# Vegeta2020/SE-SSD

Hardware: NVIDIA H100
Metric: frames_per_sec (higher is better)
Workload: dtype f32

## Files before the change

### include/sessd_b200.h

```cpp
#ifndef SESSD_B200_H
#define SESSD_B200_H

#include <stddef.h>
#include <stdint.h>

#ifdef __cplusplus
extern "C" {
#endif

#define SESSD_OK 0
#define SESSD_EINVAL (-1)
#define SESSD_ECAPACITY (-2)
#define SESSD_EWORKSPACE (-3)

const char *sessd_version(void);
long long sessd_launch_count(void);

typedef struct {
    float voxel_size[3];
    float range_min[3];
    float range_max[3];
    int grid[3];
    int max_points;
    int max_voxels;
    int num_feat;
} sessd_voxel_cfg;

size_t sessd_voxelize_workspace_bytes(int max_total_points, int batch, const sessd_voxel_cfg *cfg);

int sessd_voxelize(const float *d_points, const int *d_frame_off, int batch, int max_total_points,
                   const sessd_voxel_cfg *cfg, float *d_voxels, int *d_coors, int *d_num_points, float *d_mean,
                   int *d_num_voxels, void *workspace, size_t workspace_bytes, void *stream);

int sessd_voxelize_host(const float *h_points, int num_points, const sessd_voxel_cfg *cfg, float *h_voxels,
                        int *h_coors_zyx , int *h_num_points);

typedef struct {
    int batch;
    int shape[3];
} sessd_grid;

size_t sessd_hash_bytes(int max_rows, int *capacity_out);
int sessd_hash_build(const int *d_coors , const int *d_n, int max_rows, sessd_grid grid,
                     uint64_t *d_table, int capacity, void *stream);

size_t sessd_bitmap_words(sessd_grid grid);
size_t sessd_scan_scratch_bytes(size_t n_items);

int sessd_subm_rulebook(const int *d_coors, const int *d_n, int max_rows, sessd_grid grid, const int ksize[3],
                        int index_kind , const void *d_index, int hash_capacity,
                        int *d_nbr, void *stream);

int sessd_strided_rulebook(const int *d_in_coors, const int *d_n_in, int max_in, sessd_grid in_grid,
                           int in_index_kind, const void *d_in_index, int in_hash_capacity,
                           const int ksize[3], const int stride[3], const int padding[3],
                           sessd_grid out_grid, void *d_out_bitmap , void *d_scan_scratch,
                           int *d_out_coors, int *d_n_out, int max_out, int *d_nbr, int *d_status, void *stream);

int sessd_tile_list_stride(int kvol);
int sessd_rulebook_tile_lists(const int *d_nbr, int kvol, const int *d_n_out, int max_out, void *d_tiles, void *stream);

int sessd_spconv_forward(const float *d_in_feat, int cin, const int *d_nbr, int kvol, const int *d_n_out,
                         int max_out, const float *d_weight, int cout, const float *d_scale, const float *d_shift,
                         int relu, float *d_out_feat, void *stream);

int sessd_sparse_to_dense(const float *d_feat, const int *d_coors, const int *d_n, int max_rows, int channels,
                          sessd_grid grid, float *d_out, void *stream);
int sessd_sparse_to_dense_indexed(const float *d_feat, int max_rows, const void *d_bitmap_index, int channels, sessd_grid grid,
                                  float *d_out, void *stream);

int sessd_spconv_forward_rows(const float *d_in_feat, int cin, const int *d_nbr, int kvol, const int *d_n_out, int max_out,
                              const float *d_weight, int cout, const float *d_scale, const float *d_shift, int relu,
                              float *d_out_feat, float *d_amax_out, void *stream);
int sessd_spconv_forward_rows_planes(const float *d_in_feat, int cin, const int *d_nbr, int kvol, const int *d_n_out, int max_out,
                                     const float *d_weight, int cout, const float *d_scale, const float *d_shift, int relu,
                                     const float *d_amax_in, float gain, float shift_max, float *d_out_feat, void *d_out_planes, int cpo,
                                     float *d_out_info, void *stream);
int sessd_spconv_forward_cg(const void *d_in_planes, int cp, int plane_rows, const float *d_in_info, const void *d_tiles, int kvol,
                            const int *d_n_out, int max_out, const void *d_weight_h2, int cout, const float *d_scale, const float *d_shift,
                            int relu, float gain, float shift_max, float *d_out_f32, void *d_out_planes, float *d_out_info, void *stream);
void sessd_set_sp_cg_deep(int on);
int sessd_spconv_cg_blocks_per_sm(int cp, int cout, int deep);
int sessd_absmax_rows(const float *d_feat, const int *d_n, int max_rows, int channels, float *d_amax, void *stream);

int sessd_rulebook_transpose(const int *d_nbr, int kvol, const int *d_n_out, int max_out, int max_in, int *d_nbr_t, void *stream);
int sessd_sparse_split_planes(const float *d_x, const int *d_n, int max_rows, int channels, float *d_info, void *d_planes, int cp, void *stream);
int sessd_dense_grad_gather(const float *d_grad, const int *d_coors, const int *d_n, int max_rows, int channels, sessd_grid grid,
                            float *d_out, void *stream);
int sessd_spconv_wgrad_items(int max_out, int kvol);
size_t sessd_spconv_wgrad_workspace_bytes(int max_out, int kvol, int cin, int cout);
int sessd_spconv_wgrad_rows(const float *d_in_feat, int cin, const float *d_gout, int cout, const void *d_tiles, int kvol,
                            const int *d_n_out, int max_out, float *d_gw, void *d_ws, size_t ws_bytes, void *stream);
int sessd_spconv_wgrad_cg(const void *d_in_planes, int cp, const float *d_in_info, const void *d_g_planes, int cout, const float *d_g_info,
                          const void *d_tiles, int kvol, const int *d_n_out, int max_out, float *d_gw, void *d_ws, size_t ws_bytes,
                          void *stream);

typedef struct {
    int batch, in_h, in_w, cin;
    int out_h, out_w, cout;
    int grid_h, grid_w;
    int in_stride;
    int out_stride, out_off_y, out_off_x;
    int ntaps;
    int tap_dy[16], tap_dx[16];
    int relu;
} sessd_conv_desc;

int sessd_bev_conv_p2(const void *d_in_planes, const float *d_in_info, const void *d_weight_h2, int cout_pad, const float *d_scale,
                      const float *d_shift, const float *d_residual, const float *d_resid_info, float gain, float shift_max,
                      float *d_out_f32, void *d_out_planes, float *d_out_info, const sessd_conv_desc *desc, const int *d_items,
                      void *stream);
int sessd_bev_deconv_p2(const void *d_in_planes, const float *d_in_info, const void *d_weight_h2, int cout_pad, const float *d_scale,
                        const float *d_shift, const float *d_residual, const float *d_resid_info, float gain, float shift_max,
                        float *d_out_f32, void *d_out_planes, float *d_out_info, int batch, int in_h, int in_w, int cin, int cout,
                        int relu, const int *d_items, void *stream);
long long sessd_bev_skip_plan_words(int batch, int h, int w, int *offsets);
int sessd_bev_skip_plan(const void *d_bitmap_index, sessd_grid grid, int *d_plan, void *stream);
int sessd_bev_skip_fill(const int *d_record, float *d_out_f32, void *d_out_planes, int cout, void *stream);
int sessd_bev_wgrad_items(const sessd_conv_desc *desc);
size_t sessd_bev_wgrad_workspace_bytes(const sessd_conv_desc *desc);
int sessd_bev_wgrad(const void *d_in_planes, const float *d_in_info, const void *d_g_planes, const float *d_g_info,
                    const sessd_conv_desc *desc, float *d_gw, void *d_ws, size_t ws_bytes, void *stream);
int sessd_bev_split_planes(const float *d_x, long long n, float *d_info, void *d_planes, void *stream);
int sessd_sparse_to_dense_planes(const float *d_feat, int max_rows, const void *d_bitmap_index, int channels, sessd_grid grid,
                                 const float *d_amax, float *d_info, void *d_planes, void *stream);
int sessd_ssfa_fuse_planes(const float *d_x0, const float *d_x1, const float *d_w0, const float *d_w1, float s0, float t0, float s1,
                           float t1, int num_pixels, int channels, float *d_out, const float *d_info0, const float *d_info1,
                           float *d_out_info, void *d_planes, void *stream);

int sessd_absmax(const float *d_x, long long n, float *d_amax, void *stream);


typedef struct {
    float cnt_thresh;
    float dist_edge[4];
    float sigma2[3];
    float suppressed_thresh;
    float centerness_pow;
    int centerness;
} sessd_dinms_cfg;

#define SESSD_DINMS_MAX_PRE 4096

typedef struct {
    int batch;
    int num_anchors;
    int anchors_per_loc;
    int head_stride;
    float score_thresh;
    int nms_pre_max;
    int nms_post_max;
    float nms_iou_thresh;
    int nms_ge;
    float post_range[6];
    float direction_offset;
    int use_frustum;
    int nms_mode;
    sessd_dinms_cfg dinms;
} sessd_post_cfg;

size_t sessd_postprocess_workspace_bytes(const sessd_post_cfg *cfg);

int sessd_postprocess(const float *d_head, const float *d_anchors, const float *d_frustum,
                      const sessd_post_cfg *cfg, float *d_boxes, float *d_scores, int *d_labels, int *d_count,
                      int *d_aux, int *d_sel_anchor, void *workspace, size_t workspace_bytes, void *stream);

int sessd_postprocess_packed(const float *d_head, const float *d_anchors, const float *d_frustum,
                             const sessd_post_cfg *cfg, float *d_boxes, float *d_scores, int *d_labels, int *d_count,
                             int *d_aux, int *d_sel_anchor, float *d_packed, int *d_meta, const int *d_num_voxels,
                             const int *d_status, void *workspace, size_t workspace_bytes, void *stream);

size_t sessd_rotate_nms_workspace_bytes(int max_boxes, int pre_max);
int sessd_rotate_nms(const float *d_boxes5, const float *d_scores, const int *d_n, int max_boxes, int pre_max,
                     int post_max, float iou_thresh, int ge, int *d_keep, int *d_num_keep, void *workspace,
                     size_t workspace_bytes, void *stream);

size_t sessd_rotate_weighted_nms_workspace_bytes(int max_boxes, int pre_max);
int sessd_rotate_weighted_nms(const float *d_boxes7, const float *d_boxes5, const float *d_scores, const float *d_iou_preds,
                              const int *d_labels, const int *d_dirs, const float *d_anchors, const int *d_n, int max_boxes,
                              int pre_max, const sessd_dinms_cfg *cfg, float *d_out_boxes, float *d_out_scores, int *d_out_labels,
                              int *d_out_dirs, int *d_keep, int *d_selected, int *d_count, void *workspace, size_t workspace_bytes,
                              void *stream);

int sessd_boxes_overlap_bev(const float *d_a, int n, const float *d_b, int m, float *d_out, void *stream);
int sessd_boxes_aligned_overlap_bev(const float *d_a, const float *d_b, int n, float *d_out, void *stream);
int sessd_boxes_iou_bev(const float *d_a, int n, const float *d_b, int m, float *d_out, void *stream);
int sessd_boxes_iou3d(const float *d_a, int n, const float *d_b, int m, float *d_out, void *stream);
size_t sessd_nms_workspace_bytes(int n);
int sessd_nms_sorted(const float *d_boxes, int n, float thresh, int mode, long long *d_keep, int *d_num_keep,
                     void *workspace, size_t workspace_bytes, void *stream);

size_t sessd_assign_workspace_bytes(int num_anchors, int batch, int max_gt);
int sessd_assign_targets(const float *d_anchors, int num_anchors, const float *d_gt_boxes, const int *d_num_gt, int batch,
                         int max_gt, float matched_thr, float unmatched_thr, int *d_labels, float *d_bbox_targets,
                         float *d_bbox_outside_weights, int *d_pos_anchor, int *d_pos_gt_id, int *d_num_pos,
                         void *workspace, size_t workspace_bytes, void *stream);

#define SESSD_AUGMENT_MAX_GT 256
#define SESSD_AUGMENT_MAX_TRY 128
int sessd_box_collision(const double *d_boxes, int n, const double *d_qboxes, int k, uint8_t *d_out, void *stream);
int sessd_noise_per_box(const float *d_gt_boxes, const int *d_num_gt, const uint8_t *d_valid, int batch, int max_gt,
                        const double *d_loc_noise, const double *d_rot_noise, int num_try, double context, int *d_selected,
                        void *stream);
int sessd_points_in_boxes(const float *d_points, int n, int point_stride, const float *d_boxes, int m, double context, uint8_t *d_mask,
                          void *stream);
int sessd_augment_points(const float *d_points, const int *d_frame_off, int batch, int max_frame_points, const float *d_gt_boxes,
                         const int *d_num_gt, const uint8_t *d_valid, int max_gt, const double *d_loc_noise, const double *d_rot_noise,
                         int num_try, const int *d_selected, double context, const float *d_global, const int *d_perm,
                         const uint8_t *d_labeled, float *d_points_raw, float *d_points_out, void *stream);
int sessd_augment_boxes(const float *d_gt_boxes, const int *d_num_gt, const uint8_t *d_valid, const uint8_t *d_target, int batch,
                        int max_gt, const double *d_loc_noise, const double *d_rot_noise, int num_try, const int *d_selected,
                        const float *d_global, const float *range_bev, float *d_boxes_raw, int *d_num_raw, float *d_boxes_out,
                        int *d_num_out, float *d_boxes_global, int *d_num_global, void *stream);

int sessd_gtaug_select_host(const double *h_corners, int num_boxes, int num_cand, uint8_t *h_accepted);
size_t sessd_gtaug_paste_workspace_bytes(int batch, int num_points, int num_objects);
int sessd_gtaug_paste(const float *d_points, const int *d_frame_off, int batch, int num_points, const int *d_obj_off, const int *d_obj_ids,
                      int num_objects, int max_paste_points, const float *d_db_points, const int *d_db_off, const int *d_db_count,
                      const double *d_db_boxes, int db_size, void *d_workspace, size_t workspace_bytes, float *d_points_out, int capacity,
                      int *d_frame_off_out, void *stream);

#define SESSD_SADA_MAX_IDS (6 * SESSD_AUGMENT_MAX_GT)
int sessd_sada_pyramids(const float *d_boxes, int num_boxes, float *d_pyramids, float *d_planes, void *stream);
int sessd_sada_membership(const float *d_points, int n, const int *d_n, const float *d_planes, int num_pyramids, const int *d_ids, int num_ids,
                          uint32_t *d_bits, int *d_counts, void *stream);
size_t sessd_sada_compact_workspace_bytes(int n);
int sessd_sada_compact(const float *d_points, int n, const int *d_n, const uint32_t *d_bits, int num_ids, const int *d_counts, int min_count,
                       void *d_workspace, size_t workspace_bytes, float *d_out, int capacity, int *d_num_out, void *stream);
size_t sessd_sada_fps_workspace_bytes(int n, int num_ids);
int sessd_sada_fps(const float *d_points, int n, const int *d_n, const uint32_t *d_bits, int num_ids, const int *d_counts, int min_count, int k,
                   void *d_workspace, size_t workspace_bytes, float *d_out, int capacity, int *d_num, void *stream);
int sessd_sada_swap(const float *d_points, int n, const int *d_n, const uint32_t *d_bits, int num_pairs, const int *d_counts, const float *d_pyramids,
                    int num_pyramids, const int *d_ids, int max_swap_points, float *d_out, int capacity, const int *d_num_in,
                    int *d_num_out, void *stream);
int sessd_sada_shuffle(const float *d_points, const int *d_frame_off, int batch, int max_frame_points, const int *d_perm, float *d_out,
                       void *stream);

size_t sessd_prep_frustum_compact_workspace_bytes(int num_points);
int sessd_prep_frustum_compact(const float *d_points, const int *d_frame_off, int batch, int num_points, const double *d_planes,
                               void *d_workspace, size_t workspace_bytes, float *d_points_out, int capacity, int *d_frame_off_out, void *stream);
int sessd_prep_box_count(const float *d_points, const int *d_frame_off, int batch, int num_points, const double *d_box_planes,
                         const int *d_box_off, int num_boxes, int *d_counts, void *stream);
size_t sessd_prep_box_gather_workspace_bytes(int num_boxes);
int sessd_prep_box_gather(const float *d_points, const int *d_frame_off, int batch, int num_points, const double *d_box_planes,
                          const double *d_centres, const int *d_box_off, int num_boxes, const int *d_counts, int num_rows, void *d_workspace,
                          size_t workspace_bytes, float *d_rows_out, int capacity, int *d_obj_off, void *stream);

size_t sessd_head_loss_workspace_bytes(int batch);
size_t sessd_odiou_loss_workspace_bytes(int batch);
int sessd_odiou_loss(const float *d_head, const float *d_anchors, const int *d_labels, const float *d_reg_targets, int batch,
                     int num_anchors, int anchors_per_loc, int head_stride, float w_odiou, const float *d_losses, float *d_odiou_sum,
                     float *d_grad_head, void *workspace, size_t workspace_bytes, void *stream);
int sessd_odiou_pairs_host(const float *h_gboxes, const float *h_qboxes, int n, float *h_odiou, float *h_grad_q);
size_t sessd_iou_pred_loss_workspace_bytes(int batch);
int sessd_iou_pred_loss(const float *d_head, const float *d_anchors, const int *d_labels, const float *d_reg_targets, int batch,
                        int num_anchors, int anchors_per_loc, int head_stride, float sigma, float w_iou, float *d_losses,
                        float *d_grad_head, void *workspace, size_t workspace_bytes, void *stream);
int sessd_head_loss(const float *d_head, const float *d_anchors, const int *d_labels, const float *d_reg_targets, int batch,
                    int num_anchors, int anchors_per_loc, int head_stride, float alpha, float sigma, float dir_offset,
                    float pos_cls_weight, float neg_cls_weight, float w_cls, float w_loc, float w_dir, float *d_losses,
                    float *d_grad_head, void *workspace, size_t workspace_bytes, void *stream);

int sessd_axpby(float *d_y, const float *d_x, float a, float b, long long n, void *stream);
int sessd_adamw_step(float *d_param, const float *d_grad, float *d_exp_avg, float *d_exp_avg_sq, long long n, float lr, float beta1,
                     float beta2, float eps, float weight_decay, int step, void *stream);
size_t sessd_grad_sqnorm_workspace_bytes(long long n);
int sessd_grad_sqnorm(const float *d_x, long long n, float max_norm, float *d_out, void *d_workspace, void *stream);
int sessd_adamw_clip_ema_step(float *d_param, float *d_grad, float *d_exp_avg, float *d_exp_avg_sq, long long n, float lr, float beta1,
                              float beta2, float eps, float weight_decay, int step, const float *d_clip_coef, float *d_ema, double ema_alpha,
                              void *stream);

#define SESSD_KITTI_REC 13
#define SESSD_KITTI_PERSON_SITTING 11
#define SESSD_KITTI_VAN 12
typedef struct {
    int num_frames;
    const int *gt_off;
    const double *gt;
    const int *gt_code;
    const int *gt_occluded;
    const int *dc_off;
    const double *dc;
    const int *dt_off;
    const int *dt_cnt;
    const double *dt;
    const int *dt_code;
    const long long *ov_off;
} SessdKittiFrames;
size_t sessd_kitti_convert_workspace_bytes(long long capacity);
int sessd_kitti_convert_detections(const float *d_boxes7, const float *d_scores, const int *d_labels, const int *d_off, int num_frames,
                                   long long capacity, const double *d_calib, const int *d_image_hw, const int *d_label_code,
                                   int num_labels, double *d_rec, int *d_label, int *d_code, int *d_cnt, void *workspace,
                                   size_t workspace_bytes, void *stream);
int sessd_kitti_overlaps(const SessdKittiFrames *frames, int metric, int z_axis, double z_center, double *d_overlaps, void *stream);
size_t sessd_kitti_eval_workspace_bytes(int num_frames, long long total_gt, long long overlap_elems, int num_configs, int compute_aos);
int sessd_kitti_eval(const SessdKittiFrames *frames, int max_frame_dt, int metric, int z_axis, double z_center, int num_configs,
                     const int *d_cfg, const double *d_min_overlap, int compute_aos, long long total_gt, long long overlap_elems,
                     double *d_thresholds, int *d_num_thresholds, double *d_precision, double *d_aos, double *d_map, void *workspace,
                     size_t workspace_bytes, void *stream);

#ifdef __cplusplus
}
#endif
#endif
```

### include/sessd_b200_lab.h

```cpp
#ifndef SESSD_B200_LAB_H
#define SESSD_B200_LAB_H

#include "sessd_b200.h"

#ifdef __cplusplus
extern "C" {
#endif

int sessd_bev_conv_h2(const float *d_in, const void *d_weight_h2, int cout_pad, const float *d_scale,
                      const float *d_shift, const float *d_residual, float *d_out, const sessd_conv_desc *desc,
                      const float *d_amax_in, float *d_amax_out, void *stream);
int sessd_bev_deconv_h2(const float *d_in, const void *d_weight_h2, int cout_pad, const float *d_scale,
                        const float *d_shift, const float *d_residual, float *d_out, int batch, int in_h, int in_w,
                        int cin, int cout, int relu, const float *d_amax_in, float *d_amax_out, void *stream);

int sessd_bev_conv_p2_profile(const void *d_in_planes, const float *d_in_info, const void *d_weight_h2, int cout_pad,
                              const float *d_scale, const float *d_shift, const float *d_residual, const float *d_resid_info,
                              float gain, float shift_max, float *d_out_f32, void *d_out_planes, float *d_out_info,
                              const sessd_conv_desc *desc, const int *d_items, long long *d_prof, void *stream);
int sessd_bev_deconv_p2_profile(const void *d_in_planes, const float *d_in_info, const void *d_weight_h2, int cout_pad,
                                const float *d_scale, const float *d_shift, const float *d_residual, const float *d_resid_info,
                                float gain, float shift_max, float *d_out_f32, void *d_out_planes, float *d_out_info, int batch,
                                int in_h, int in_w, int cin, int cout, int relu, const int *d_items, long long *d_prof,
                                void *stream);

int sessd_bev_conv_p2_loads(const void *d_in_planes, const float *d_in_info, const void *d_weight_h2, int cout_pad,
                            const float *d_scale, const float *d_shift, const float *d_residual, const float *d_resid_info,
                            float gain, float shift_max, float *d_out_f32, void *d_out_planes, float *d_out_info,
                            const sessd_conv_desc *desc, const int *d_items, int smem_a, long long *d_prof, void *stream);

int sessd_bev_p2_plan(const sessd_conv_desc *desc, int deconv, int cout_pad, int split, int smem_a, int *plan);

#ifdef __cplusplus
}
#endif
#endif
```

### se-ssd_b200/csrc/bevconv_p2.cu

```cuda
#include "bevconv_p2.cuh"

namespace sessd {

__global__ void __launch_bounds__(256) bev_split_planes_kernel(const float4 *__restrict__ x, long long n4, float *__restrict__ info,
                                                               __half *__restrict__ planes, long long plane_stride) {
    const float s = pow2_scale_for_bound(__ldg(info));
    if (blockIdx.x == 0 && threadIdx.x == 0) info[1] = s;
    for (long long i = blockIdx.x * (long long)blockDim.x + threadIdx.x; i < n4; i += (long long)gridDim.x * blockDim.x) {
        const float4 v = __ldg(x + i);
        const float a[4] = {v.x * s, v.y * s, v.z * s, v.w * s};
        __align__(8) __half hi[4], lo[4];
#pragma unroll
        for (int t = 0; t < 4; ++t) {
            hi[t] = __float2half_rn(a[t]);
            lo[t] = __float2half_rn(a[t] - __half2float(hi[t]));
        }
        *reinterpret_cast<uint2 *>(planes + 4 * i) = *reinterpret_cast<const uint2 *>(hi);
        *reinterpret_cast<uint2 *>(planes + plane_stride + 4 * i) = *reinterpret_cast<const uint2 *>(lo);
    }
}

}

using namespace sessd;

extern "C" int sessd_bev_conv_p2(const void *d_in_planes, const float *d_in_info, const void *d_weight_h2, int cout_pad, const float *d_scale,
                                 const float *d_shift, const float *d_residual, const float *d_resid_info, float gain, float shift_max,
                                 float *d_out_f32, void *d_out_planes, float *d_out_info, const sessd_conv_desc *desc, const int *d_items,
                                 void *stream) {
    return p2_conv<kP2Planes>(d_in_planes, d_in_info, d_weight_h2, cout_pad, d_scale, d_shift, d_residual, d_resid_info, gain, shift_max,
                              d_out_f32, d_out_planes, d_out_info, desc, stream, d_items);
}

extern "C" int sessd_bev_deconv_p2(const void *d_in_planes, const float *d_in_info, const void *d_weight_h2, int cout_pad, const float *d_scale,
                                   const float *d_shift, const float *d_residual, const float *d_resid_info, float gain, float shift_max,
                                   float *d_out_f32, void *d_out_planes, float *d_out_info, int batch, int in_h, int in_w, int cin, int cout,
                                   int relu, const int *d_items, void *stream) {
    return p2_deconv<kP2Planes>(d_in_planes, d_in_info, d_weight_h2, cout_pad, d_scale, d_shift, d_residual, d_resid_info, gain, shift_max,
                                d_out_f32, d_out_planes, d_out_info, batch, in_h, in_w, cin, cout, relu, stream, d_items);
}

extern "C" int sessd_bev_split_planes(const float *d_x, long long n, float *d_info, void *d_planes, void *stream) {
    if (!d_x || !d_info || !d_planes || n < 4 || (n & 3) || ((uintptr_t)d_x & 15)) return SESSD_EINVAL;
    SESSD_LAUNCH(bev_split_planes_kernel, persistent_grid(n / 4, 256), 256, 0, stream, reinterpret_cast<const float4 *>(d_x), n / 4, d_info,
                 (__half *)d_planes, n);
    return last_error();
}
```

### se-ssd_b200/csrc/bevconv_p2.cuh

```cuda
#pragma once
#include <cuda_fp16.h>

#include "tc_common.cuh"

namespace sessd {

constexpr int kP2TileU = 8, kP2TileV = 16;
constexpr int kP2MaxCopies = 6, kP2MaxRowsV = 18;
constexpr int kP2BStages = 6, kP2MaxBStages = 12;
constexpr int kP2MmaWarps = 8;
constexpr int kP2PatchWarp = 8, kP2WeightWarp = 9;
constexpr int kP2Threads = 320;
constexpr int kP2ThreadsRegA = 384, kP2RegsConsumer = 232, kP2RegsProducer = 40;
static_assert(2 * (kP2RegsConsumer - 168) <= 168 - kP2RegsProducer, "the consumers take what the producers release");
constexpr int kP2MaxSmem = 227 * 1024;
constexpr int kP2Chunk = 32;
constexpr int kP2ItemsHeader = 32;
enum { kP2Planes = 0, kP2SplitF16 = 1 };
enum { kP2NoProbe = 0, kP2ProbeClocks = 1, kP2ProbeLoads = 2 };

struct P2Params {
    int batch, cin, cout;
    int in_stride;
    int out_h, out_w;
    int grid_u, grid_v;
    int u_is_x;
    int out_stride, nclass;
    int cls_ntaps[4], cls_off_u[4], cls_off_v[4];
    int tap_copy[4][9], tap_row[4][9], tap_w[4][9];
    int ncopies, rows_v, pitch_u;
    int copy_u[kP2MaxCopies], copy_v[kP2MaxCopies];
    int copy_bytes, patch_bytes, npatch;
    int load_bytes, staging_bytes;
    int bring_bytes;
    int out_info_scale;
    const float *in_amax;
    int relu, n_tile, nblocks;
    int bstages, bstage_bytes;
    int tiles_u, tiles_v, tiles, total;
    int cls_order[4];
    const float *in_info;
    const float *resid_info;
    float gain, shift_max;
    float *out_info;
    long long out_plane_stride;
    const int *items;
    long long *prof;
};

enum P2Prof {
    kProfCta,
    kProfItems,
    kProfSteps,
    kProfItemClk,
    kProfBFull,
    kProfPatchFull,
    kProfMmaWait,
    kProfEpilogue,
    kProfPatchEmpty,
    kProfPatchTotal,
    kProfBEmpty,
    kProfBTotal,
    kP2ProfWords = 16
};

__device__ __forceinline__ int p2_item_count(const P2Params &p) { return p.items ? __ldg(p.items) : p.total; }
__device__ __forceinline__ int p2_item(const P2Params &p, int k) { return p.items ? __ldg(p.items + kP2ItemsHeader + k) : k; }

struct P2ItemIndex { int rank, nb, t; };
__host__ __device__ __forceinline__ P2ItemIndex p2_item_index(int g, int nblocks, int tiles) {
    const int rank = g / (nblocks * tiles), rem = g - rank * (nblocks * tiles), nb = rem / tiles;
    return {rank, nb, rem - nb * tiles};
}

struct P2Item { int cls, n0, b, u0, v0, ntaps; };

__device__ __forceinline__ P2Item p2_decode(const P2Params &p, int g) {
    P2Item it;
    const P2ItemIndex ix = p2_item_index(g, p.nblocks, p.tiles);
    int t = ix.t;
    it.cls = p.cls_order[ix.rank];
    it.n0 = ix.nb * p.n_tile;
    const int tu = t % p.tiles_u; t /= p.tiles_u;
    const int tv = t % p.tiles_v;
    it.b = t / p.tiles_v;
    it.u0 = tu * kP2TileU; it.v0 = tv * kP2TileV;
    it.ntaps = p.cls_ntaps[it.cls];
    return it;
}

template <int N>
__device__ __forceinline__ void p2_wgmma(float *d, uint64_t da, uint64_t db, uint32_t accumulate) {
    if constexpr (N == 32) wgmma_f16_n32(d, da, db, accumulate);
    else if constexpr (N == 64) wgmma_f16_n64(d, da, db, accumulate);
    else if constexpr (N == 128) wgmma_f16_n128(d, da, db, accumulate);
    else wgmma_f16_n256(d, da, db, accumulate);
}

template <int N>
__device__ __forceinline__ void p2_wgmma_ra(float *d, const uint32_t *a, uint64_t db, uint32_t accumulate) {
    if constexpr (N == 32) wgmma_f16_ra_n32(d, a, db, accumulate);
    else if constexpr (N == 64) wgmma_f16_ra_n64(d, a, db, accumulate);
    else if constexpr (N == 128) wgmma_f16_ra_n128(d, a, db, accumulate);
    else wgmma_f16_ra_n256(d, a, db, accumulate);
}

template <bool PROFILE>
__device__ __forceinline__ long long p2_tick() {
    if constexpr (PROFILE) return clock64();
    return 0;
}
template <bool PROFILE>
__device__ __forceinline__ void p2_tock(long long &clk, long long t0) {
    if constexpr (PROFILE) clk += clock64() - t0;
}

__device__ __forceinline__ void p2_split_patch(const P2Params &p, const unsigned char *staging, unsigned char *planes, float s_in, int ctid) {
    const int rows = p.rows_v * kP2TileU;
    const int copy_in = p.staging_bytes / p.ncopies;
    const int items = p.ncopies * rows * 4;
    for (int i = ctid; i < items; i += kP2MmaWarps * 32) {
        const int j = i & 3, r = (i >> 2) % rows, c = (i >> 2) / rows;
        unsigned char *hi = planes + 2 * c * p.copy_bytes + r * 64 + ((j ^ ((r >> 1) & 3)) << 4);
        const float4 *src = reinterpret_cast<const float4 *>(staging + c * copy_in + r * 128 + j * 32);
        const float4 a = src[0], b = src[1];
        const float x[8] = {a.x * s_in, a.y * s_in, a.z * s_in, a.w * s_in, b.x * s_in, b.y * s_in, b.z * s_in, b.w * s_in};
        __align__(16) __half h[8], l[8];
#pragma unroll
        for (int t = 0; t < 8; ++t) { h[t] = __float2half_rn(x[t]); l[t] = __float2half_rn(x[t] - __half2float(h[t])); }
        *reinterpret_cast<uint4 *>(hi) = *reinterpret_cast<const uint4 *>(h);
        *reinterpret_cast<uint4 *>(hi + p.copy_bytes) = *reinterpret_cast<const uint4 *>(l);
    }
    asm volatile("fence.proxy.async.shared::cta;\n" ::: "memory");
    asm volatile("bar.sync 1, %0;\n" ::"n"(kP2MmaWarps * 32) : "memory");
}

template <int NT, int MODE, bool REGA = false, int PROBE = kP2NoProbe>
__global__ void __launch_bounds__(REGA ? kP2ThreadsRegA : kP2Threads, 1) bev_conv_p2_kernel(const __grid_constant__ CUtensorMap map_a,
                                                                   const __grid_constant__ CUtensorMap map_b,
                                                                   const float *__restrict__ scale, const float *__restrict__ shift,
                                                                   const float *__restrict__ resid, float *__restrict__ out_f32,
                                                                   __half *__restrict__ out_planes, P2Params p) {
    static_assert(!REGA || MODE == kP2Planes, "register-fed A reads the TMA-written planes");
    constexpr bool PROFILE = PROBE != kP2NoProbe, LOADS_ONLY = PROBE == kP2ProbeLoads;
    extern __shared__ unsigned char smem_raw[];
    unsigned char *tiles = (unsigned char *)(((uintptr_t)smem_raw + 1023) & ~(uintptr_t)1023);
    unsigned char *patches = tiles + p.bring_bytes;
    unsigned char *staging = patches + p.npatch * p.patch_bytes;
    uint64_t *bars = (uint64_t *)(staging + p.npatch * p.staging_bytes);
    uint64_t *patch_full = bars, *patch_empty = bars + 2, *b_full = bars + 4, *b_empty = bars + 4 + kP2MaxBStages;
    uint32_t *s_aoff = (uint32_t *)(b_empty + kP2MaxBStages);
    float *s_scale = (float *)(((uintptr_t)(s_aoff + 4 * 9) + 15) & ~(uintptr_t)15), *s_shift = s_scale + p.cout;

    const int warp = threadIdx.x >> 5, lane = threadIdx.x & 31;
    if (threadIdx.x == kP2PatchWarp * 32) prefetch_tensormap(&map_a);
    if (threadIdx.x == kP2WeightWarp * 32) prefetch_tensormap(&map_b);
    const int nchunks = p.cin / kP2Chunk;
    const int nitems = p2_item_count(p);
    const uint32_t b_plane_bytes = (uint32_t)p.n_tile * 64u;

    if (threadIdx.x == 0) {
        for (int s = 0; s < 2; ++s) { mbar_init(&patch_full[s], 1); mbar_init(&patch_empty[s], kP2MmaWarps); }
        for (int s = 0; s < p.bstages; ++s) { mbar_init(&b_full[s], 1); mbar_init(&b_empty[s], kP2MmaWarps); }
        asm volatile("fence.mbarrier_init.release.cluster;\n" ::: "memory");
    }
    for (int idx = threadIdx.x; idx < p.nclass * 9; idx += blockDim.x) {
        const int c = idx / 9, t = idx - c * 9;
        s_aoff[idx] = REGA ? (uint32_t)p.tap_row[c][t] : (uint32_t)((2 * p.tap_copy[c][t] * p.copy_bytes + p.tap_row[c][t] * 512) >> 4);
    }
    for (int n = threadIdx.x; n < p.cout; n += blockDim.x) {
        s_scale[n] = scale ? __ldg(scale + n) : 1.f;
        s_shift[n] = shift ? __ldg(shift + n) : 0.f;
    }
    __syncthreads();
    long long clk[kP2ProfWords] = {};
    const long long t_start = p2_tick<PROFILE>();
    long long *prof_rec = PROFILE ? p.prof + (size_t)blockIdx.x * kP2ProfWords : nullptr;

    if (warp >= kP2MmaWarps) {
        if constexpr (REGA) setmaxnreg_dec<kP2RegsProducer>();
        if (warp == kP2PatchWarp) {
            int pb = 0;
            uint32_t pph = 0;
            const uint32_t patches_u32 = smem_u32(patches);
            for (int k = blockIdx.x; k < nitems; k += gridDim.x) {
                const P2Item it = p2_decode(p, p2_item(p, k));
                const int bu = it.u0 * p.in_stride, bv = it.v0 * p.in_stride;
                for (int cc = 0; cc < nchunks; ++cc) {
                    { const long long t0 = p2_tick<PROFILE>(); mbar_wait<REGA>(&patch_empty[pb], pph ^ 1u); p2_tock<PROFILE>(clk[kProfPatchEmpty], t0); }
                    if (elect_one()) {
                        mbar_expect_tx(&patch_full[pb], (uint32_t)p.load_bytes);
                        if constexpr (MODE == kP2Planes) {
                            uint32_t dst = patches_u32 + (uint32_t)(pb * p.patch_bytes);
                            for (int c = 0; c < p.ncopies; ++c, dst += 2u * (uint32_t)p.copy_bytes) {
                                const int cu = bu + p.copy_u[c], cv = bv + p.copy_v[c];
                                tma_load_5d(dst, &map_a, &patch_full[pb], cc * kP2Chunk, cu, cv, it.b, 0);
                                tma_load_5d(dst + (uint32_t)p.copy_bytes, &map_a, &patch_full[pb], cc * kP2Chunk, cu, cv, it.b, 1);
                            }
                        } else {
                            const uint32_t copy_in = (uint32_t)(p.staging_bytes / p.ncopies);
                            uint32_t dst = smem_u32(staging) + (uint32_t)(pb * p.staging_bytes);
                            for (int c = 0; c < p.ncopies; ++c, dst += copy_in)
                                tma_load_5d(dst, &map_a, &patch_full[pb], cc * kP2Chunk, bu + p.copy_u[c], bv + p.copy_v[c], it.b, 0);
                        }
                    }
                    __syncwarp();
                    if (++pb == p.npatch) { pb = 0; pph ^= 1u; }
                }
            }
            if constexpr (PROFILE)
                if (lane == 0) {
                    prof_rec[kProfPatchEmpty] = clk[kProfPatchEmpty];
                    prof_rec[kProfPatchTotal] = clock64() - t_start;
                }
        } else if (warp == kP2WeightWarp) {
            int S = 0;
            uint32_t bph = 0;
            for (int k = blockIdx.x; k < nitems; k += gridDim.x) {
                const P2Item it = p2_decode(p, p2_item(p, k));
                for (int cc = 0; cc < nchunks; ++cc)
                    for (int tap = 0; tap < it.ntaps; ++tap) {
                        { const long long t0 = p2_tick<PROFILE>(); mbar_wait<REGA>(&b_empty[S], bph ^ 1u); p2_tock<PROFILE>(clk[kProfBEmpty], t0); }
                        if (elect_one()) {
                            unsigned char *st = tiles + S * p.bstage_bytes;
                            const int wtap = p.tap_w[it.cls][tap];
                            mbar_expect_tx(&b_full[S], 2 * b_plane_bytes);
                            tma_load_4d(st + b_plane_bytes, &map_b, &b_full[S], cc * kP2Chunk, it.n0, wtap, 0);
                            tma_load_4d(st, &map_b, &b_full[S], cc * kP2Chunk, it.n0, wtap, 1);
                        }
                        __syncwarp();
                        if (++S == p.bstages) { S = 0; bph ^= 1u; }
                    }
            }
            if constexpr (PROFILE)
                if (lane == 0) {
                    prof_rec[kProfBEmpty] = clk[kProfBEmpty];
                    prof_rec[kProfBTotal] = clock64() - t_start;
                }
        }
    } else {
        if constexpr (REGA) setmaxnreg_inc<kP2RegsConsumer>();
        const int wg = warp >> 2, wq = warp & 3;
        constexpr int kAcc = NT / 2;
        const uint32_t a_rows = (uint32_t)(wg * 64 * 64) >> 4;
        const uint32_t tiles_lo = desc_lo(smem_u32(tiles));
        const uint32_t patch_lo = desc_lo(smem_u32(patches)) + a_rows;
        const uint32_t plane_lo = b_plane_bytes >> 4;
        const uint32_t copy_lo = (uint32_t)(p.copy_bytes >> 4), patch_sz = (uint32_t)(p.patch_bytes >> 4);
        const uint32_t a_row = (uint32_t)((wg * 8 + wq * 2 + ((lane >> 3) & 1)) * p.pitch_u + (lane & 7)), a_chunk = (uint32_t)(lane >> 4);
        const uint32_t patches_u32 = smem_u32(patches);
        float amax_in = 0.f, s_in = 1.f;
        if constexpr (MODE == kP2Planes) { amax_in = __ldg(p.in_info); s_in = __ldg(p.in_info + 1); }
        if constexpr (MODE == kP2SplitF16) if (p.in_amax) { amax_in = __ldg(p.in_amax); s_in = pow2_scale_for_bound(amax_in); }
        const float inv_sa = 1.f / s_in;
        float bound = amax_in * p.gain + p.shift_max;
        if (p.resid_info) bound += __ldg(p.resid_info);
        const float s_out = pow2_scale_for_bound(bound);
        if (blockIdx.x == 0 && threadIdx.x == 0 && p.out_info && p.out_info_scale) p.out_info[1] = s_out;
        float vmax = 0.f;
        const int per_cls = p.nblocks * p.tiles;
        int S = 0, pb = 0;
        uint32_t bph = 0, pph = 0;
        for (int k = blockIdx.x; k < nitems; k += gridDim.x) {
            const long long t_item = p2_tick<PROFILE>();
            const int g = p2_item(p, k);
            const int cls = p.cls_order[g / per_cls];
            const int ntaps = p.cls_ntaps[cls];
            const uint32_t *aoff = s_aoff + cls * 9;
            float acc[NT];
#pragma unroll
            for (int i = 0; i < NT; ++i) acc[i] = 0.f;
            int prevS = -1, prev_pb = -1;
            bool first = true;
            if constexpr (REGA) {
                uint32_t frag[2][16];
                int tap = 0;
                uint32_t pbase = 0;
                auto load_frags = [&](uint32_t *fa) {
                    if (tap == 0) {
                        { const long long t0 = p2_tick<PROFILE>(); mbar_wait<REGA>(&patch_full[pb], pph); p2_tock<PROFILE>(clk[kProfPatchFull], t0); }
                        pbase = patches_u32 + (uint32_t)(pb * p.patch_bytes);
                    }
                    if constexpr (!LOADS_ONLY) {
                        const uint32_t r = a_row + aoff[tap];
                        const uint32_t a_hi = pbase + r * 64u + ((a_chunk ^ ((r >> 1) & 3u)) << 4), a_lo = a_hi + (uint32_t)p.copy_bytes;
                        ldsm_x4(fa, a_hi);
                        ldsm_x4(fa + 4, a_hi ^ 32u);
                        ldsm_x4(fa + 8, a_lo);
                        ldsm_x4(fa + 12, a_lo ^ 32u);
                    }
                };
                auto step_ra = [&](const uint32_t *fa, uint32_t *fn, bool more) {
                    { const long long t0 = p2_tick<PROFILE>(); mbar_wait<REGA>(&b_full[S], bph); p2_tock<PROFILE>(clk[kProfBFull], t0); }
                    const uint64_t db_lo = kDescSw64Hi | (uint64_t)(tiles_lo + (uint32_t)(S * (p.bstage_bytes >> 4)));
                    const uint64_t db_hi = db_lo + (uint64_t)plane_lo;
                    if constexpr (!LOADS_ONLY) {
                        wgmma_fence();
                        p2_wgmma_ra<2 * NT>(acc, fa, db_lo, first ? 0u : 1u);
                        p2_wgmma_ra<2 * NT>(acc, fa + 4, db_lo + 2, 1u);
                        wgmma_commit();
                    }
                    first = false;
                    if constexpr (PROFILE) ++clk[kProfSteps];
                    { const long long t0 = p2_tick<PROFILE>(); wgmma_wait<1>(); p2_tock<PROFILE>(clk[kProfMmaWait], t0); }
                    if (lane == 0 && prevS >= 0) mbar_arrive(&b_empty[prevS]);
                    prevS = S;
                    if (++S == p.bstages) { S = 0; bph ^= 1u; }
                    if (++tap == ntaps) {
                        tap = 0;
                        if (lane == 0) mbar_arrive(&patch_empty[pb]);
                        if (++pb == p.npatch) { pb = 0; pph ^= 1u; }
                    }
                    if (more) load_frags(fn);
                    if constexpr (!LOADS_ONLY) {
                        wgmma_fence();
                        p2_wgmma_ra<NT>(acc, fa + 8, db_hi, 1u);
                        p2_wgmma_ra<NT>(acc, fa + 12, db_hi + 2, 1u);
                        wgmma_commit();
                    }
                };
                const int nsteps = nchunks * ntaps;
                load_frags(frag[0]);
#pragma unroll 1
                for (int st = 0; st + 1 < nsteps; st += 2) { step_ra(frag[0], frag[1], true); step_ra(frag[1], frag[0], st + 2 < nsteps); }
                if (nsteps & 1) step_ra(frag[0], frag[1], false);
            } else {
                for (int cc = 0; cc < nchunks; ++cc) {
                    { const long long t0 = p2_tick<PROFILE>(); mbar_wait(&patch_full[pb], pph); p2_tock<PROFILE>(clk[kProfPatchFull], t0); }
                    if constexpr (MODE == kP2SplitF16)
                        p2_split_patch(p, staging + pb * p.staging_bytes, patches + pb * p.patch_bytes, s_in, threadIdx.x);
                    const uint32_t pbase = patch_lo + (uint32_t)pb * patch_sz;
#pragma unroll 1
                    for (int tap = 0; tap < ntaps; ++tap) {
                        { const long long t0 = p2_tick<PROFILE>(); mbar_wait(&b_full[S], bph); p2_tock<PROFILE>(clk[kProfBFull], t0); }
                        if constexpr (!LOADS_ONLY) {
                            const uint64_t da_hi = kDescSw64Hi | (uint64_t)(pbase + aoff[tap]);
                            const uint64_t da_lo = da_hi + (uint64_t)copy_lo;
                            const uint64_t db_lo = kDescSw64Hi | (uint64_t)(tiles_lo + (uint32_t)(S * (p.bstage_bytes >> 4)));
                            const uint64_t db_hi = db_lo + (uint64_t)plane_lo;
                            const uint32_t accum = first ? 0u : 1u;
                            wgmma_fence();
                            if constexpr (MODE == kP2Planes) {
                                p2_wgmma<2 * NT>(acc, da_hi, db_lo, accum);
                                p2_wgmma<2 * NT>(acc, da_hi + 2, db_lo + 2, 1u);
                            } else {
                                p2_wgmma<NT>(acc + kAcc, da_hi, db_hi, accum);
                                p2_wgmma<NT>(acc + kAcc, da_hi + 2, db_hi + 2, 1u);
                                p2_wgmma<NT>(acc, da_hi, db_lo, accum);
                                p2_wgmma<NT>(acc, da_hi + 2, db_lo + 2, 1u);
                            }
                            p2_wgmma<NT>(acc, da_lo, db_hi, 1u);
                            p2_wgmma<NT>(acc, da_lo + 2, db_hi + 2, 1u);
                            wgmma_commit();
                        }
                        first = false;
                        if constexpr (PROFILE) ++clk[kProfSteps];
                        { const long long t0 = p2_tick<PROFILE>(); wgmma_wait<1>(); p2_tock<PROFILE>(clk[kProfMmaWait], t0); }
                        if (lane == 0) {
                            if (prevS >= 0) mbar_arrive(&b_empty[prevS]);
                            if (prev_pb >= 0) mbar_arrive(&patch_empty[prev_pb]);
                        }
                        prevS = S;
                        prev_pb = (tap == ntaps - 1) ? pb : -1;
                        if (++S == p.bstages) { S = 0; bph ^= 1u; }
                    }
                    if (p.npatch == 1) {
                        { const long long t0 = p2_tick<PROFILE>(); wgmma_wait<0>(); p2_tock<PROFILE>(clk[kProfMmaWait], t0); }
                        if (lane == 0) {
                            mbar_arrive(&b_empty[prevS]);
                            mbar_arrive(&patch_empty[pb]);
                        }
                        prevS = prev_pb = -1;
                    }
                    if (++pb == p.npatch) { pb = 0; pph ^= 1u; }
                }
            }
            { const long long t0 = p2_tick<PROFILE>(); wgmma_wait<0>(); p2_tock<PROFILE>(clk[kProfMmaWait], t0); }
            const long long t_epi = p2_tick<PROFILE>();
            wgmma_fence_regs<NT>(acc);
            if (lane == 0) {
                if (prevS >= 0) mbar_arrive(&b_empty[prevS]);
                if (prev_pb >= 0) mbar_arrive(&patch_empty[prev_pb]);
            }
#pragma unroll
            for (int i = 0; i < kAcc; ++i) acc[i] = acc[kAcc + i] + acc[i];
            const P2Item it = p2_decode(p, g);
            const int q = lane & 3;
            const int r0 = wg * 64 + wq * 16 + (lane >> 2);
            bool rows_ok[2];
            size_t opixs[2];
#pragma unroll
            for (int h = 0; h < 2; ++h) {
                const int r = r0 + 8 * h;
                const int lv = r / kP2TileU, lu = r % kP2TileU;
                const int gu = it.u0 + lu, gv = it.v0 + lv;
                rows_ok[h] = it.b < p.batch && gu < p.grid_u && gv < p.grid_v;
                const int ou = gu * p.out_stride + p.cls_off_u[it.cls], ov = gv * p.out_stride + p.cls_off_v[it.cls];
                const int oy = p.u_is_x ? ov : ou, ox = p.u_is_x ? ou : ov;
                opixs[h] = ((size_t)it.b * p.out_h + (size_t)oy) * p.out_w + (size_t)ox;
            }
#pragma unroll
            for (int j = 0; j < (LOADS_ONLY ? 0 : NT / 32); ++j)
#pragma unroll
                for (int h = 0; h < 2; ++h) {
                    const bool row_ok = rows_ok[h];
                    const size_t opix = opixs[h];
                    float v[8], o[8] = {};
                    quad_transpose8(acc + 16 * j + 2 * h, q, v);
                    const int n = it.n0 + 32 * j + 8 * q;
                    const size_t off = opix * p.cout + n;
                    if (row_ok && n < p.cout) {
                        float sc[8], sh[8];
#pragma unroll
                        for (int t = 0; t < 8; t += 4) {
                            const float4 a = *reinterpret_cast<const float4 *>(s_scale + n + t);
                            const float4 b = *reinterpret_cast<const float4 *>(s_shift + n + t);
                            sc[t] = a.x; sc[t + 1] = a.y; sc[t + 2] = a.z; sc[t + 3] = a.w;
                            sh[t] = b.x; sh[t + 1] = b.y; sh[t + 2] = b.z; sh[t + 3] = b.w;
                        }
#pragma unroll
                        for (int t = 0; t < 8; ++t) {
                            o[t] = fmaf(v[t] * inv_sa, sc[t], sh[t]);
                            if (p.relu) o[t] = fmaxf(o[t], 0.f);
                        }
                        if (resid) {
#pragma unroll
                            for (int t = 0; t < 8; t += 4) {
                                const float4 rr = __ldg(reinterpret_cast<const float4 *>(resid + off + t));
                                o[t] += rr.x; o[t + 1] += rr.y; o[t + 2] += rr.z; o[t + 3] += rr.w;
                            }
                        }
#pragma unroll
                        for (int t = 0; t < 8; ++t) vmax = fmaxf(vmax, fabsf(o[t]));
                        if (out_planes) {
                            __align__(16) __half2 hi[4], lo[4];
#pragma unroll
                            for (int t = 0; t < 4; ++t) {
                                const float x0 = o[2 * t] * s_out, x1 = o[2 * t + 1] * s_out;
                                hi[t] = __floats2half2_rn(x0, x1);
                                const float2 f = __half22float2(hi[t]);
                                lo[t] = __floats2half2_rn(x0 - f.x, x1 - f.y);
                            }
                            *reinterpret_cast<uint4 *>(out_planes + off) = *reinterpret_cast<const uint4 *>(hi);
                            *reinterpret_cast<uint4 *>(out_planes + p.out_plane_stride + off) = *reinterpret_cast<const uint4 *>(lo);
                        }
                    }
                    if (out_f32) {
                        const bool up = q & 2;
                        float keep[4], recv[4];
#pragma unroll
                        for (int t = 0; t < 4; ++t) {
                            keep[t] = up ? o[4 + t] : o[t];
                            recv[t] = __shfl_xor_sync(0xFFFFFFFFu, up ? o[t] : o[4 + t], 2);
                        }
                        const int n_lo = it.n0 + 32 * j + 8 * (q & 1), c_lo = n_lo + 4 * (q >> 1);
                        const float4 w_lo = up ? make_float4(recv[0], recv[1], recv[2], recv[3]) : make_float4(keep[0], keep[1], keep[2], keep[3]);
                        const float4 w_hi = up ? make_float4(keep[0], keep[1], keep[2], keep[3]) : make_float4(recv[0], recv[1], recv[2], recv[3]);
                        if (row_ok && n_lo < p.cout) *reinterpret_cast<float4 *>(out_f32 + opix * p.cout + c_lo) = w_lo;
                        if (row_ok && n_lo + 16 < p.cout) *reinterpret_cast<float4 *>(out_f32 + opix * p.cout + c_lo + 16) = w_hi;
                    }
                }
            if constexpr (PROFILE) {
                const long long t_end = clock64();
                clk[kProfEpilogue] += t_end - t_epi;
                clk[kProfItemClk] += t_end - t_item;
                ++clk[kProfItems];
            }
        }
        if constexpr (PROFILE)
            if (threadIdx.x == 0) {
                clk[kProfCta] = clock64() - t_start;
                for (int w = kProfCta; w <= kProfEpilogue; ++w) prof_rec[w] = clk[w];
            }
        if (p.out_info) {
            const unsigned m = __reduce_max_sync(0xFFFFFFFFu, __float_as_uint(vmax));
            if (lane == 0 && m != 0u) atomicMax(reinterpret_cast<unsigned *>(p.out_info), m);
        }
    }
}

static int encode_map_nd(CUtensorMap *m, const void *base, int rank, const cuuint64_t *dims, const cuuint64_t *strides_bytes ,
                         const cuuint32_t *box, const cuuint32_t *estr, CUtensorMapSwizzle swz,
                         CUtensorMapDataType dtype = CU_TENSOR_MAP_DATA_TYPE_FLOAT16) {
    EncodeTiledFn enc = get_tensor_map_encoder();
    if (!enc) return SESSD_EINVAL;
    CUresult r = enc(m, dtype, (cuuint32_t)rank, const_cast<void *>(base), dims, strides_bytes, box, estr,
                     CU_TENSOR_MAP_INTERLEAVE_NONE, swz, CU_TENSOR_MAP_L2_PROMOTION_L2_256B, CU_TENSOR_MAP_FLOAT_OOB_FILL_NONE);
    return r == CUDA_SUCCESS ? 0 : 700 + (int)r;
}

struct P2Taps { int n, dy[9], dx[9], w[9], off_y, off_x; };

static void p2_deconv_classes(P2Taps cls[4]) {
    for (int c = 0; c < 4; ++c) {
        P2Taps &k = cls[c];
        k = {};
        k.off_y = c >> 1; k.off_x = c & 1;
        for (int dy = k.off_y; dy >= 0; --dy)
            for (int dx = k.off_x; dx >= 0; --dx, ++k.n) {
                k.dy[k.n] = dy; k.dx[k.n] = dx; k.w[k.n] = (k.off_y + 1 - 2 * dy) * 3 + (k.off_x + 1 - 2 * dx);
            }
    }
}

constexpr int p2_n_tile(int cout) { return cout <= 32 ? 32 : 128; }

struct P2Geometry {
    int u_is_x, grid_u, grid_v, tiles_u, tiles_v, tiles;
    int n_tile, nblocks, nclass, total;
    int ntaps[4], off_u[4], off_v[4], order[4];
};

static int p2_geometry(P2Geometry &g, int batch, int grid_h, int grid_w, int cout, int cout_pad, const P2Taps *cls, int nclass) {
    g = {};
    if (batch < 1 || grid_h < 1 || grid_w < 1 || cout < 8 || cout % 8) return SESSD_EINVAL;
    g.n_tile = p2_n_tile(cout);
    if (cout_pad % g.n_tile || cout_pad < cout) return SESSD_EINVAL;
    g.u_is_x = div_up(grid_w, kP2TileU) * div_up(grid_h, kP2TileV) <= div_up(grid_h, kP2TileU) * div_up(grid_w, kP2TileV);
    g.grid_u = g.u_is_x ? grid_w : grid_h; g.grid_v = g.u_is_x ? grid_h : grid_w;
    g.tiles_u = div_up(g.grid_u, kP2TileU); g.tiles_v = div_up(g.grid_v, kP2TileV);
    g.tiles = g.tiles_u * g.tiles_v * batch;
    g.nblocks = cout_pad / g.n_tile;
    g.nclass = nclass; g.total = nclass * g.nblocks * g.tiles;
    for (int c = 0; c < nclass; ++c) {
        g.ntaps[c] = cls[c].n;
        g.off_u[c] = g.u_is_x ? cls[c].off_x : cls[c].off_y;
        g.off_v[c] = g.u_is_x ? cls[c].off_y : cls[c].off_x;
        g.order[c] = c;
    }
    for (int i = 1; i < nclass; ++i)
        for (int k = i; k > 0 && g.ntaps[g.order[k]] > g.ntaps[g.order[k - 1]]; --k) {
            const int tmp = g.order[k]; g.order[k] = g.order[k - 1]; g.order[k - 1] = tmp;
        }
    return 0;
}

static int p2_plan(P2Params &p, const P2Taps *cls, int nclass, int grid_h, int grid_w, int cout_pad, int mode, bool reg_a, int *smem) {
    if (reg_a && (mode != kP2Planes || p.in_stride != 1)) return SESSD_EINVAL;
    if (p.cin < 64 || p.cin % 64) return SESSD_EINVAL;
    P2Geometry g;
    if (p2_geometry(g, p.batch, grid_h, grid_w, p.cout, cout_pad, cls, nclass)) return SESSD_EINVAL;
    p.u_is_x = g.u_is_x; p.grid_u = g.grid_u; p.grid_v = g.grid_v;
    p.tiles_u = g.tiles_u; p.tiles_v = g.tiles_v; p.tiles = g.tiles;
    p.n_tile = g.n_tile; p.nblocks = g.nblocks; p.nclass = g.nclass; p.total = g.total;
    for (int c = 0; c < 4; ++c) {
        p.cls_ntaps[c] = g.ntaps[c]; p.cls_off_u[c] = g.off_u[c]; p.cls_off_v[c] = g.off_v[c]; p.cls_order[c] = g.order[c];
    }
    const int s = p.in_stride;
    p.ncopies = 0;
    int key_u[kP2MaxCopies], key_vm[kP2MaxCopies], vmin[kP2MaxCopies], vmax[kP2MaxCopies];
    for (int c = 0; c < p.nclass; ++c)
        for (int t = 0; t < cls[c].n; ++t) {
            const int tu = p.u_is_x ? cls[c].dx[t] : cls[c].dy[t], tv = p.u_is_x ? cls[c].dy[t] : cls[c].dx[t];
            const int vm = ((tv % s) + s) % s;
            int k = 0;
            for (; k < p.ncopies; ++k)
                if (key_u[k] == tu && key_vm[k] == vm) break;
            if (k == p.ncopies) {
                if (p.ncopies == kP2MaxCopies) return SESSD_EINVAL;
                key_u[k] = tu; key_vm[k] = vm; vmin[k] = tv; vmax[k] = tv;
                ++p.ncopies;
            }
            vmin[k] = min(vmin[k], tv); vmax[k] = max(vmax[k], tv);
        }
    p.rows_v = 0;
    p.pitch_u = kP2TileU;
    for (int k = 0; k < p.ncopies; ++k) p.rows_v = max(p.rows_v, kP2TileV + (vmax[k] - vmin[k]) / s);
    if (p.rows_v > kP2MaxRowsV) return SESSD_EINVAL;
    for (int k = 0; k < p.ncopies; ++k) { p.copy_u[k] = key_u[k]; p.copy_v[k] = vmin[k]; }
    if (reg_a) {
        int umin = key_u[0], umax = key_u[0];
        for (int k = 1; k < p.ncopies; ++k) {
            umin = min(umin, key_u[k]); umax = max(umax, key_u[k]);
            vmin[0] = min(vmin[0], vmin[k]); vmax[0] = max(vmax[0], vmax[k]);
        }
        p.ncopies = 1;
        p.copy_u[0] = umin; p.copy_v[0] = vmin[0];
        p.pitch_u = kP2TileU + umax - umin; p.rows_v = kP2TileV + vmax[0] - vmin[0];
        if (p.pitch_u > 256 || p.rows_v > 256) return SESSD_EINVAL;
    }
    for (int c = 0; c < p.nclass; ++c) {
        for (int t = 0; t < cls[c].n; ++t) {
            const int tu = p.u_is_x ? cls[c].dx[t] : cls[c].dy[t], tv = p.u_is_x ? cls[c].dy[t] : cls[c].dx[t];
            const int vm = ((tv % s) + s) % s;
            int k = 0;
            for (; k < p.ncopies; ++k)
                if (key_u[k] == tu && key_vm[k] == vm) break;
            p.tap_copy[c][t] = reg_a ? 0 : k;
            p.tap_row[c][t] = reg_a ? (tv - p.copy_v[0]) * p.pitch_u + (tu - p.copy_u[0]) : (tv - vmin[k]) / s;
            p.tap_w[c][t] = cls[c].w[t];
        }
    }
    p.copy_bytes = (p.rows_v * p.pitch_u * 64 + 511) & ~511;
    p.patch_bytes = p.ncopies * 2 * p.copy_bytes;
    p.staging_bytes = mode == kP2Planes ? 0 : p.ncopies * p.rows_v * kP2TileU * kP2Chunk * 4;
    p.load_bytes = mode == kP2Planes ? p.ncopies * 2 * p.rows_v * p.pitch_u * 64 : p.staging_bytes;
    const int per_buf = p.patch_bytes + p.staging_bytes, bstage = 2 * p.n_tile * 64;
    const int tail = 1536 + 16 + 2 * 4 * p.cout;
    p.npatch = (kP2BStages * bstage + tail + 2 * per_buf <= kP2MaxSmem) ? 2 : 1;
    p.bstage_bytes = bstage;
    p.bstages = min((kP2MaxSmem - tail - p.npatch * per_buf) / bstage, kP2MaxBStages);
    if (p.bstages < 2) return SESSD_EINVAL;
    p.bring_bytes = p.bstages * bstage;
    *smem = p.bring_bytes + tail + p.npatch * per_buf;
    return 0;
}

template <int MODE, int PROBE = kP2NoProbe>
static int launch_p2(const void *d_in_planes, int in_h, int in_w, const float *d_in_info, const void *d_w, int w_taps, int cout_pad,
                     const float *d_scale, const float *d_shift, const float *d_residual, const float *d_resid_info, float gain,
                     float shift_max, float *d_out_f32, void *d_out_planes, float *d_out_info, P2Params &p, const P2Taps *cls, int nclass,
                     int grid_h, int grid_w, bool reg_a, void *stream) {
    if (!d_in_planes || !d_w || (!d_out_f32 && !d_out_planes)) return SESSD_EINVAL;
    if (MODE == kP2Planes && (!d_in_info || !d_scale)) return SESSD_EINVAL;
    if (MODE != kP2Planes && d_out_planes) return SESSD_EINVAL;
    if (((uintptr_t)d_scale | (uintptr_t)d_shift | (uintptr_t)d_residual | (uintptr_t)d_out_f32 | (uintptr_t)d_out_planes) & 15)
        return SESSD_EINVAL;
    int smem = 0;
    if (p2_plan(p, cls, nclass, grid_h, grid_w, cout_pad, MODE, reg_a, &smem)) return SESSD_EINVAL;
    if (p.items && cout_pad != div_up(p.cout, p.n_tile) * p.n_tile) return SESSD_EINVAL;
    const int s = p.in_stride;
    CUtensorMap map_a, map_b;
    if (MODE != kP2Planes) {
        const cuuint64_t row_w = (cuuint64_t)p.cin * 4, row_h = (cuuint64_t)in_w * p.cin * 4;
        const cuuint64_t dims[5] = {(cuuint64_t)p.cin, (cuuint64_t)(p.u_is_x ? in_w : in_h), (cuuint64_t)(p.u_is_x ? in_h : in_w),
                                    (cuuint64_t)p.batch, 1};
        const cuuint64_t strides[4] = {p.u_is_x ? row_w : row_h, p.u_is_x ? row_h : row_w, (cuuint64_t)in_h * in_w * p.cin * 4,
                                       (cuuint64_t)p.batch * in_h * in_w * p.cin * 4};
        const cuuint32_t box[5] = {(cuuint32_t)kP2Chunk, (cuuint32_t)(kP2TileU * s), (cuuint32_t)(p.rows_v * s), 1, 1};
        const cuuint32_t estr[5] = {1, (cuuint32_t)s, (cuuint32_t)s, 1, 1};
        int rc = encode_map_nd(&map_a, d_in_planes, 5, dims, strides, box, estr, CU_TENSOR_MAP_SWIZZLE_NONE, CU_TENSOR_MAP_DATA_TYPE_FLOAT32);
        if (rc) return rc;
    } else {
        const cuuint64_t row_w = (cuuint64_t)p.cin * 2, row_h = (cuuint64_t)in_w * p.cin * 2;
        const cuuint64_t dims[5] = {(cuuint64_t)p.cin, (cuuint64_t)(p.u_is_x ? in_w : in_h), (cuuint64_t)(p.u_is_x ? in_h : in_w),
                                    (cuuint64_t)p.batch, 2};
        const cuuint64_t strides[4] = {p.u_is_x ? row_w : row_h, p.u_is_x ? row_h : row_w, (cuuint64_t)in_h * in_w * p.cin * 2,
                                       (cuuint64_t)p.batch * in_h * in_w * p.cin * 2};
        const cuuint32_t box[5] = {(cuuint32_t)kP2Chunk, (cuuint32_t)(p.pitch_u * s), (cuuint32_t)(p.rows_v * s), 1, 1};
        const cuuint32_t estr[5] = {1, (cuuint32_t)s, (cuuint32_t)s, 1, 1};
        int rc = encode_map_nd(&map_a, d_in_planes, 5, dims, strides, box, estr, CU_TENSOR_MAP_SWIZZLE_64B);
        if (rc) return rc;
    }
    {
        const cuuint64_t dims[4] = {(cuuint64_t)p.cin, (cuuint64_t)cout_pad, (cuuint64_t)w_taps, 2};
        const cuuint64_t strides[3] = {(cuuint64_t)p.cin * 2, (cuuint64_t)cout_pad * p.cin * 2, (cuuint64_t)w_taps * cout_pad * p.cin * 2};
        const cuuint32_t box[4] = {(cuuint32_t)kP2Chunk, (cuuint32_t)p.n_tile, 1, 1};
        const cuuint32_t estr[4] = {1, 1, 1, 1};
        int rc = encode_map_nd(&map_b, d_w, 4, dims, strides, box, estr, CU_TENSOR_MAP_SWIZZLE_64B);
        if (rc) return rc;
    }
    constexpr bool kRegA = MODE == kP2Planes;
    auto kernel = bev_conv_p2_kernel<128, MODE, false, PROBE>;
    if (p.n_tile == 32) kernel = reg_a ? bev_conv_p2_kernel<32, MODE, kRegA, PROBE> : bev_conv_p2_kernel<32, MODE, false, PROBE>;
    else if (reg_a) kernel = bev_conv_p2_kernel<128, MODE, kRegA, PROBE>;
    static bool attr_done[2][2] = {};
    if (!attr_done[p.n_tile == 32][reg_a]) {
        SESSD_CUDA_TRY(cudaFuncSetAttribute(kernel, cudaFuncAttributeMaxDynamicSharedMemorySize, kP2MaxSmem));
        attr_done[p.n_tile == 32][reg_a] = true;
    }
    p.in_info = MODE == kP2Planes ? d_in_info : nullptr;
    p.in_amax = MODE == kP2SplitF16 ? d_in_info : nullptr;
    p.resid_info = d_residual ? d_resid_info : nullptr;
    if (d_residual && d_out_planes && !d_resid_info) return SESSD_EINVAL;
    p.gain = gain; p.shift_max = shift_max; p.out_info = d_out_info;
    p.out_info_scale = MODE == kP2Planes ? 1 : 0;
    if (d_out_planes && !d_out_info) return SESSD_EINVAL;
    p.out_plane_stride = (long long)p.batch * p.out_h * p.out_w * p.cout;
    static int num_sms = 0;
    if (!num_sms) {
        int dev = 0;
        SESSD_CUDA_TRY(cudaGetDevice(&dev));
        SESSD_CUDA_TRY(cudaDeviceGetAttribute(&num_sms, cudaDevAttrMultiProcessorCount, dev));
    }
    const int grid = p.total < num_sms ? p.total : num_sms;
    SESSD_LAUNCH(kernel, grid, reg_a ? kP2ThreadsRegA : kP2Threads, smem, (cudaStream_t)stream, map_a, map_b, d_scale, d_shift, d_residual, d_out_f32,
                 (__half *)d_out_planes, p);
    return last_error();
}


static int p2_conv_params(const sessd_conv_desc &d, P2Params &p, P2Taps &t) {
    if (d.ntaps < 1 || d.ntaps > 9 || (d.in_stride != 1 && d.in_stride != 2) || d.out_stride < 1) return SESSD_EINVAL;
    if ((d.grid_h - 1) * d.out_stride + d.out_off_y >= d.out_h || (d.grid_w - 1) * d.out_stride + d.out_off_x >= d.out_w) return SESSD_EINVAL;
    p = {};
    p.batch = d.batch; p.cin = d.cin; p.cout = d.cout; p.in_stride = d.in_stride;
    p.out_h = d.out_h; p.out_w = d.out_w; p.out_stride = d.out_stride; p.relu = d.relu;
    t = {};
    t.n = d.ntaps; t.off_y = d.out_off_y; t.off_x = d.out_off_x;
    for (int i = 0; i < d.ntaps; ++i) { t.dy[i] = d.tap_dy[i]; t.dx[i] = d.tap_dx[i]; t.w[i] = i; }
    return 0;
}

static void p2_deconv_params(int batch, int in_h, int in_w, int cin, int cout, int relu, P2Params &p, P2Taps cls[4]) {
    p = {};
    p.batch = batch; p.cin = cin; p.cout = cout; p.in_stride = 1;
    p.out_h = 2 * in_h; p.out_w = 2 * in_w; p.out_stride = 2; p.relu = relu;
    p2_deconv_classes(cls);
}

template <int MODE, int PROBE = kP2NoProbe>
static int p2_conv(const void *d_in_planes, const float *d_in_info, const void *d_weight_h2, int cout_pad, const float *d_scale,
                   const float *d_shift, const float *d_residual, const float *d_resid_info, float gain, float shift_max,
                   float *d_out_f32, void *d_out_planes, float *d_out_info, const sessd_conv_desc *desc, void *stream,
                   const int *d_items = nullptr, long long *d_prof = nullptr, bool smem_a = false) {
    if (!desc || (PROBE != kP2NoProbe && !d_prof)) return SESSD_EINVAL;
    const sessd_conv_desc &d = *desc;
    P2Params p;
    P2Taps t;
    if (p2_conv_params(d, p, t)) return SESSD_EINVAL;
    p.items = d_items;
    p.prof = d_prof;
    return launch_p2<MODE, PROBE>(d_in_planes, d.in_h, d.in_w, d_in_info, d_weight_h2, d.ntaps, cout_pad, d_scale, d_shift, d_residual, d_resid_info, gain,
                     shift_max, d_out_f32, d_out_planes, d_out_info, p, &t, 1, d.grid_h, d.grid_w, MODE == kP2Planes && d.in_stride == 1 && !smem_a,
                     stream);
}

template <int MODE, int PROBE = kP2NoProbe>
static int p2_deconv(const void *d_in_planes, const float *d_in_info, const void *d_weight_h2, int cout_pad, const float *d_scale,
                     const float *d_shift, const float *d_residual, const float *d_resid_info, float gain, float shift_max,
                     float *d_out_f32, void *d_out_planes, float *d_out_info, int batch, int in_h, int in_w, int cin, int cout,
                     int relu, void *stream, const int *d_items = nullptr, long long *d_prof = nullptr) {
    if (PROBE != kP2NoProbe && !d_prof) return SESSD_EINVAL;
    P2Params p;
    P2Taps cls[4];
    p2_deconv_params(batch, in_h, in_w, cin, cout, relu, p, cls);
    p.items = d_items;
    p.prof = d_prof;
    return launch_p2<MODE, PROBE>(d_in_planes, in_h, in_w, d_in_info, d_weight_h2, 9, cout_pad, d_scale, d_shift, d_residual, d_resid_info, gain, shift_max,
                     d_out_f32, d_out_planes, d_out_info, p, cls, 4, in_h, in_w, MODE == kP2Planes, stream);
}

}
```

### se-ssd_b200/csrc/bevconv_split.cu

```cuda
#include "bevconv_p2.cuh"

#include "../../include/sessd_b200_lab.h"

using namespace sessd;

extern "C" int sessd_bev_conv_h2(const float *d_in, const void *d_weight_h2, int cout_pad, const float *d_scale, const float *d_shift,
                                 const float *d_residual, float *d_out, const sessd_conv_desc *desc, const float *d_amax_in,
                                 float *d_amax_out, void *stream) {
    if (!d_in || !d_out || !d_scale) return SESSD_EINVAL;
    return p2_conv<kP2SplitF16>(d_in, d_amax_in, d_weight_h2, cout_pad, d_scale, d_shift, d_residual, nullptr, 0.f, 0.f, d_out, nullptr,
                                d_amax_out, desc, stream);
}

extern "C" int sessd_bev_deconv_h2(const float *d_in, const void *d_weight_h2, int cout_pad, const float *d_scale, const float *d_shift,
                                   const float *d_residual, float *d_out, int batch, int in_h, int in_w, int cin, int cout, int relu,
                                   const float *d_amax_in, float *d_amax_out, void *stream) {
    if (!d_in || !d_out || !d_scale) return SESSD_EINVAL;
    return p2_deconv<kP2SplitF16>(d_in, d_amax_in, d_weight_h2, cout_pad, d_scale, d_shift, d_residual, nullptr, 0.f, 0.f, d_out, nullptr,
                                  d_amax_out, batch, in_h, in_w, cin, cout, relu, stream);
}

extern "C" int sessd_bev_conv_p2_profile(const void *d_in_planes, const float *d_in_info, const void *d_weight_h2, int cout_pad,
                                         const float *d_scale, const float *d_shift, const float *d_residual, const float *d_resid_info,
                                         float gain, float shift_max, float *d_out_f32, void *d_out_planes, float *d_out_info,
                                         const sessd_conv_desc *desc, const int *d_items, long long *d_prof, void *stream) {
    return p2_conv<kP2Planes, kP2ProbeClocks>(d_in_planes, d_in_info, d_weight_h2, cout_pad, d_scale, d_shift, d_residual, d_resid_info, gain,
                                              shift_max, d_out_f32, d_out_planes, d_out_info, desc, stream, d_items, d_prof);
}

extern "C" int sessd_bev_deconv_p2_profile(const void *d_in_planes, const float *d_in_info, const void *d_weight_h2, int cout_pad,
                                           const float *d_scale, const float *d_shift, const float *d_residual, const float *d_resid_info,
                                           float gain, float shift_max, float *d_out_f32, void *d_out_planes, float *d_out_info, int batch,
                                           int in_h, int in_w, int cin, int cout, int relu, const int *d_items, long long *d_prof,
                                           void *stream) {
    return p2_deconv<kP2Planes, kP2ProbeClocks>(d_in_planes, d_in_info, d_weight_h2, cout_pad, d_scale, d_shift, d_residual, d_resid_info, gain,
                                                shift_max, d_out_f32, d_out_planes, d_out_info, batch, in_h, in_w, cin, cout, relu, stream,
                                                d_items, d_prof);
}

extern "C" int sessd_bev_conv_p2_loads(const void *d_in_planes, const float *d_in_info, const void *d_weight_h2, int cout_pad,
                                       const float *d_scale, const float *d_shift, const float *d_residual, const float *d_resid_info,
                                       float gain, float shift_max, float *d_out_f32, void *d_out_planes, float *d_out_info,
                                       const sessd_conv_desc *desc, const int *d_items, int smem_a, long long *d_prof, void *stream) {
    return p2_conv<kP2Planes, kP2ProbeLoads>(d_in_planes, d_in_info, d_weight_h2, cout_pad, d_scale, d_shift, d_residual, d_resid_info, gain,
                                             shift_max, d_out_f32, d_out_planes, d_out_info, desc, stream, d_items, d_prof, smem_a != 0);
}

extern "C" int sessd_bev_p2_plan(const sessd_conv_desc *desc, int deconv, int cout_pad, int split, int smem_a, int *plan) {
    if (!desc || !plan) return SESSD_EINVAL;
    const sessd_conv_desc &d = *desc;
    P2Params p;
    P2Taps cls[4];
    if (deconv) p2_deconv_params(d.batch, d.in_h, d.in_w, d.cin, d.cout, d.relu, p, cls);
    else if (p2_conv_params(d, p, cls[0])) return SESSD_EINVAL;
    const int mode = split ? kP2SplitF16 : kP2Planes;
    const bool reg_a = mode == kP2Planes && (deconv || (d.in_stride == 1 && !smem_a));
    int smem = 0;
    if (p2_plan(p, cls, deconv ? 4 : 1, deconv ? d.in_h : d.grid_h, deconv ? d.in_w : d.grid_w, cout_pad, mode, reg_a, &smem))
        return SESSD_EINVAL;
    const int rec[11] = {p.u_is_x, p.n_tile, p.nblocks, p.tiles, p.total, p.ncopies, p.rows_v, p.pitch_u, p.npatch, p.bstages, smem};
    for (int i = 0; i < 11; ++i) plan[i] = rec[i];
    for (int c = 0; c < 4; ++c) { plan[11 + c] = p.cls_ntaps[c]; plan[15 + c] = p.cls_order[c]; }
    return 0;
}
```

### se-ssd_b200/csrc/bevskip.cu

```cuda
#include "bevconv_p2.cuh"

namespace sessd {

enum {
    kRecCount = 0, kRecSkipped = 1, kRecNclass = 2, kRecTiles = 3, kRecTilesU = 4, kRecTilesV = 5, kRecUisX = 6, kRecOutStride = 7,
    kRecOutH = 8, kRecOutW = 9, kRecBatch = 10, kRecOffY = 11, kRecOffX = 15, kRecRep = 19, kRecSkipOff = 23, kRecFlagOff = 24
};

enum { kMX, kMB0a, kMB0b, kMX0, kMM0, kMM1, kMO0, kMO1, kMOut, kMTmp, kMB1a, kMB1b, kMX1, kMTmpH, kNumMaps };
constexpr int kNumFullMaps = kMTmp + 1;
constexpr int kSkipLaunches = 13;
constexpr int kSkipThreads = 1024;

struct SkipLaunch : P2Geometry {
    int map;
    int out_stride, out_h, out_w;
    int rec;
};

struct SkipPlan {
    int batch, depth, h, w, h2, w2, nwf, nwh;
    SkipLaunch l[kSkipLaunches];
};

static int skip_launch(SkipLaunch &L, int map, int batch, int grid_h, int grid_w, int out_h, int out_w, int cout, bool deconv) {
    P2Taps cls[4] = {};
    if (deconv) p2_deconv_classes(cls);
    else cls[0].n = 1;
    L.map = map;
    L.out_stride = deconv ? 2 : 1;
    L.out_h = out_h; L.out_w = out_w;
    return p2_geometry(L, batch, grid_h, grid_w, cout, div_up(cout, p2_n_tile(cout)) * p2_n_tile(cout), cls, deconv ? 4 : 1);
}

static long long skip_plan(SkipPlan &P, int batch, int h, int w) {
    if (batch < 1 || h < 4 || w < 4 || (h & 1) || (w & 1)) return 0;
    P.batch = batch; P.h = h; P.w = w; P.h2 = h / 2; P.w2 = w / 2;
    P.nwf = div_up(w, 32); P.nwh = div_up(P.w2, 32);
    const int h2 = P.h2, w2 = P.w2;
    SkipLaunch *L = P.l;
    const int rc = skip_launch(L[0], kMB0a, batch, h, w, h, w, 128, false)
                 | skip_launch(L[1], kMB0b, batch, h, w, h, w, 128, false)
                 | skip_launch(L[2], kMX0, batch, h, w, h, w, 128, false)
                 | skip_launch(L[3], kMB1a, batch, h2, w2, h2, w2, 256, false)
                 | skip_launch(L[4], kMB1b, batch, h2, w2, h2, w2, 256, false)
                 | skip_launch(L[5], kMX1, batch, h2, w2, h2, w2, 256, false)
                 | skip_launch(L[6], kMX0, batch, h, w, h, w, 128, false)
                 | skip_launch(L[7], kMX1, batch, h2, w2, h2, w2, 256, false)
                 | skip_launch(L[8], kMM0, batch, h2, w2, h, w, 128, true)
                 | skip_launch(L[9], kMM1, batch, h2, w2, h, w, 128, true)
                 | skip_launch(L[10], kMO0, batch, h, w, h, w, 128, false)
                 | skip_launch(L[11], kMO1, batch, h, w, h, w, 128, false)
                 | skip_launch(L[12], kMOut, batch, h, w, h, w, 24, false);
    long long words = 0;
    for (int i = 0; i < kSkipLaunches; ++i) {
        L[i].rec = (int)words;
        words += kP2ItemsHeader + L[i].total + 2LL * L[i].nclass * L[i].tiles;
    }
    return rc ? 0 : words;
}

struct BitMap {
    uint32_t *w;
    int h, wd, nw;
    __device__ __forceinline__ bool get(int y, int x) const { return (w[y * nw + (x >> 5)] >> (x & 31)) & 1u; }
    __device__ __forceinline__ uint32_t valid(int i) const {
        const int rem = wd - 32 * i;
        return rem >= 32 ? ~0u : ((1u << rem) - 1u);
    }
};

__device__ void skip_dilate3(const BitMap &in, const BitMap &tmp, const BitMap &out) {
    const int n = in.h * in.nw, last = (in.wd - 1) >> 5;
    for (int idx = threadIdx.x; idx < n; idx += blockDim.x) {
        const int y = idx / in.nw, i = idx - y * in.nw;
        const uint32_t *r = in.w + y * in.nw;
        const uint32_t c = r[i], l = i > 0 ? r[i - 1] : 0u, rr = i + 1 < in.nw ? r[i + 1] : 0u;
        uint32_t hv = c | (c << 1) | (l >> 31) | (c >> 1) | (rr << 31);
        if (i == 0) hv |= 1u;
        if (i == last) hv |= 1u << ((in.wd - 1) & 31);
        tmp.w[idx] = hv & in.valid(i);
    }
    __syncthreads();
    for (int idx = threadIdx.x; idx < n; idx += blockDim.x) {
        const int y = idx / in.nw, i = idx - y * in.nw;
        out.w[idx] = (y == 0 || y == in.h - 1) ? in.valid(i) : (tmp.w[idx - in.nw] | tmp.w[idx] | tmp.w[idx + in.nw]);
    }
    __syncthreads();
}

template <class F>
__device__ void skip_map_from(const BitMap &out, F f) {
    const int warp = threadIdx.x >> 5, lane = threadIdx.x & 31, nwarps = blockDim.x >> 5;
    for (int idx = warp; idx < out.h * out.nw; idx += nwarps) {
        const int y = idx / out.nw, x = (idx - y * out.nw) * 32 + lane;
        const unsigned bits = __ballot_sync(0xFFFFFFFFu, x < out.wd && f(y, x));
        if (lane == 0) out.w[idx] = bits;
    }
    __syncthreads();
}

template <class Pred>
__device__ int skip_compact(int n, Pred pred, int *out, int *s_scan) {
    const int warp = threadIdx.x >> 5, lane = threadIdx.x & 31, nwarps = blockDim.x >> 5;
    int base = 0;
    for (int start = 0; start < n; start += blockDim.x) {
        const int i = start + threadIdx.x;
        const bool v = i < n && pred(i);
        const unsigned bal = __ballot_sync(0xFFFFFFFFu, v);
        if (lane == 0) s_scan[warp] = __popc(bal);
        __syncthreads();
        if (warp == 0) {
            const int own = lane < nwarps ? s_scan[lane] : 0;
            int x = own;
#pragma unroll
            for (int o = 1; o < 32; o <<= 1) {
                const int y = __shfl_up_sync(0xFFFFFFFFu, x, o);
                if (lane >= o) x += y;
            }
            if (lane < nwarps) s_scan[lane] = x - own;
            if (lane == 31) s_scan[32] = x;
        }
        __syncthreads();
        if (v) out[base + s_scan[warp] + __popc(bal & ((1u << lane) - 1u))] = i;
        base += s_scan[32];
        __syncthreads();
    }
    return base;
}

__global__ void __launch_bounds__(kSkipThreads) bev_skip_plan_kernel(const uint2 *__restrict__ bitmap, int *__restrict__ plan, SkipPlan P) {
    extern __shared__ uint32_t s_bits[];
    __shared__ int s_scan[33], s_rep[4];
    BitMap m[kNumMaps];
    {
        uint32_t *p = s_bits;
        for (int i = 0; i < kNumMaps; ++i) {
            const bool full = i < kNumFullMaps;
            m[i].w = p; m[i].h = full ? P.h : P.h2; m[i].wd = full ? P.w : P.w2; m[i].nw = full ? P.nwf : P.nwh;
            p += m[i].h * m[i].nw;
        }
    }
    for (int b = 0; b < P.batch; ++b) {
        const BitMap X = m[kMX];
        for (int idx = threadIdx.x; idx < X.h * X.nw; idx += blockDim.x) {
            const int y = idx / X.nw, i = idx - y * X.nw;
            const int nbits = min(32, X.wd - 32 * i);
            uint32_t acc = 0u;
            for (int z = 0; z < P.depth; ++z) {
                const unsigned long long lin = (((unsigned long long)b * P.depth + z) * P.h + y) * P.w + 32 * i;
                const unsigned sh = (unsigned)(lin & 31);
                const uint32_t lo = __ldg(&bitmap[lin >> 5]).x, hi = sh + nbits > 32 ? __ldg(&bitmap[(lin >> 5) + 1]).x : 0u;
                acc |= __funnelshift_r(lo, hi, sh);
            }
            X.w[idx] = acc & X.valid(i);
        }
        __syncthreads();
        skip_dilate3(m[kMX], m[kMTmp], m[kMB0a]);
        skip_dilate3(m[kMB0a], m[kMTmp], m[kMB0b]);
        skip_dilate3(m[kMB0b], m[kMTmp], m[kMX0]);
        skip_dilate3(m[kMX0], m[kMTmp], m[kMX]);
        {
            const BitMap D = m[kMX];
            skip_map_from(m[kMB1a], [&](int y, int x) { return D.get(2 * y, 2 * x); });
        }
        skip_dilate3(m[kMB1a], m[kMTmpH], m[kMB1b]);
        skip_dilate3(m[kMB1b], m[kMTmpH], m[kMX1]);
        {
            const BitMap T = m[kMX1], R = m[kMX0];
            auto tget = [&](int gy, int gx) { return gy >= T.h || gx >= T.wd || T.get(gy, gx); };
            auto dc = [&](int oy, int ox) {
                const int py = oy & 1, px = ox & 1, gy = oy >> 1, gx = ox >> 1;
                return tget(gy, gx) || (py && tget(gy + 1, gx)) || (px && tget(gy, gx + 1)) || (py && px && tget(gy + 1, gx + 1));
            };
            skip_map_from(m[kMM0], [&](int y, int x) { return dc(y, x) || R.get(y, x); });
            skip_map_from(m[kMM1], dc);
        }
        skip_dilate3(m[kMM0], m[kMTmp], m[kMO0]);
        skip_dilate3(m[kMM1], m[kMTmp], m[kMO1]);
        for (int i = threadIdx.x; i < P.h * P.nwf; i += blockDim.x) m[kMOut].w[i] = m[kMO0].w[i] | m[kMO1].w[i];
        __syncthreads();
        for (int li = 0; li < kSkipLaunches; ++li) {
            const SkipLaunch &L = P.l[li];
            const BitMap &o = m[L.map];
            int *flags = plan + L.rec + kP2ItemsHeader + L.total + L.nclass * L.tiles;
            const int per_frame = L.tiles_u * L.tiles_v;
            for (int idx = threadIdx.x; idx < L.nclass * per_frame; idx += blockDim.x) {
                const int c = idx / per_frame, tf = idx - c * per_frame;
                const int tu = tf % L.tiles_u, tv = tf / L.tiles_u;
                const int u0 = tu * kP2TileU, v0 = tv * kP2TileV;
                bool run = u0 + kP2TileU > L.grid_u || v0 + kP2TileV > L.grid_v;
                if (!run && L.out_stride == 1) {
                    const int y0 = L.u_is_x ? v0 : u0, x0 = L.u_is_x ? u0 : v0;
                    const int ny = L.u_is_x ? kP2TileV : kP2TileU, nx = L.u_is_x ? kP2TileU : kP2TileV;
                    const uint32_t field = (1u << nx) - 1u;
                    for (int y = y0; y < y0 + ny && !run; ++y) run = (o.w[y * o.nw + (x0 >> 5)] >> (x0 & 31)) & field;
                } else if (!run) {
                    for (int r = 0; r < kP2TileU * kP2TileV && !run; ++r) {
                        const int ou = (u0 + (r & 7)) * L.out_stride + L.off_u[c], ov = (v0 + (r >> 3)) * L.out_stride + L.off_v[c];
                        run = L.u_is_x ? o.get(ov, ou) : o.get(ou, ov);
                    }
                }
                flags[c * L.tiles + b * per_frame + tf] = run ? 1 : 0;
            }
        }
        __syncthreads();
    }
    for (int li = 0; li < kSkipLaunches; ++li) {
        const SkipLaunch &L = P.l[li];
        int *rec = plan + L.rec;
        int *items = rec + kP2ItemsHeader, *skipped = items + L.total;
        const int *flags = skipped + L.nclass * L.tiles;
        if (threadIdx.x < 4) s_rep[threadIdx.x] = 0x7FFFFFFF;
        __syncthreads();
        for (int e = threadIdx.x; e < L.nclass * L.tiles; e += blockDim.x)
            if (!flags[e]) atomicMin(&s_rep[e / L.tiles], e % L.tiles);
        __syncthreads();
        const int count = skip_compact(L.total, [&](int g) {
            const P2ItemIndex ix = p2_item_index(g, L.nblocks, L.tiles);
            return flags[L.order[ix.rank] * L.tiles + ix.t] != 0 || ix.t == s_rep[L.order[ix.rank]];
        }, items, s_scan);
        const int nskip = skip_compact(L.nclass * L.tiles, [&](int e) {
            return flags[e] == 0 && e % L.tiles != s_rep[e / L.tiles];
        }, skipped, s_scan);
        if (threadIdx.x == 0) {
            rec[kRecCount] = count; rec[kRecSkipped] = nskip;
            rec[kRecNclass] = L.nclass; rec[kRecTiles] = L.tiles; rec[kRecTilesU] = L.tiles_u; rec[kRecTilesV] = L.tiles_v;
            rec[kRecUisX] = L.u_is_x; rec[kRecOutStride] = L.out_stride; rec[kRecOutH] = L.out_h; rec[kRecOutW] = L.out_w;
            rec[kRecBatch] = P.batch;
            for (int c = 0; c < 4; ++c) {
                rec[kRecOffY + c] = L.u_is_x ? L.off_v[c] : L.off_u[c]; rec[kRecOffX + c] = L.u_is_x ? L.off_u[c] : L.off_v[c];
                rec[kRecRep + c] = c < L.nclass && s_rep[c] != 0x7FFFFFFF ? s_rep[c] : -1;
            }
            rec[kRecSkipOff] = kP2ItemsHeader + L.total;
            rec[kRecFlagOff] = kP2ItemsHeader + L.total + L.nclass * L.tiles;
        }
        __syncthreads();
    }
}

__global__ void __launch_bounds__(256) bev_skip_fill_kernel(const int *__restrict__ rec, float *__restrict__ out_f32,
                                                            __half *__restrict__ out_planes, int cout) {
    const int nskip = __ldg(rec + kRecSkipped);
    if ((int)blockIdx.x >= nskip) return;
    const int tiles = __ldg(rec + kRecTiles), tiles_u = __ldg(rec + kRecTilesU), tiles_v = __ldg(rec + kRecTilesV);
    const int u_is_x = __ldg(rec + kRecUisX), os = __ldg(rec + kRecOutStride), out_h = __ldg(rec + kRecOutH), out_w = __ldg(rec + kRecOutW);
    const long long plane_stride = (long long)__ldg(rec + kRecBatch) * out_h * out_w * cout;
    const int *skipped = rec + __ldg(rec + kRecSkipOff);
    for (int e = blockIdx.x; e < nskip; e += gridDim.x) {
        const int ent = __ldg(skipped + e);
        const int c = ent / tiles, t = ent - c * tiles, r = __ldg(rec + kRecRep + c);
        const int oy0 = __ldg(rec + kRecOffY + c), ox0 = __ldg(rec + kRecOffX + c);
        auto pixel = [&](int tt, int lu, int lv) -> size_t {
            const int tu = tt % tiles_u, rest = tt / tiles_u, tv = rest % tiles_v, b = rest / tiles_v;
            const int gu = tu * kP2TileU + lu, gv = tv * kP2TileV + lv;
            const int gy = u_is_x ? gv : gu, gx = u_is_x ? gu : gv;
            return ((size_t)b * out_h + (size_t)(gy * os + oy0)) * out_w + (size_t)(gx * os + ox0);
        };
        if (out_f32) {
            const int q = cout / 4;
            for (int i = threadIdx.x; i < kP2TileU * kP2TileV * q; i += blockDim.x) {
                const int px = i / q, j = i - px * q;
                const float4 v = reinterpret_cast<const float4 *>(out_f32 + pixel(r, px & 7, px >> 3) * cout)[j];
                reinterpret_cast<float4 *>(out_f32 + pixel(t, px & 7, px >> 3) * cout)[j] = v;
            }
        }
        if (out_planes) {
            const int q = cout / 8, n = kP2TileU * kP2TileV * q;
            for (int i = threadIdx.x; i < 2 * n; i += blockDim.x) {
                const int pl = i / n, k = i - pl * n, px = k / q, j = k - px * q;
                const __half *src = out_planes + pl * plane_stride + pixel(r, px & 7, px >> 3) * cout;
                __half *dst = out_planes + pl * plane_stride + pixel(t, px & 7, px >> 3) * cout;
                reinterpret_cast<uint4 *>(dst)[j] = reinterpret_cast<const uint4 *>(src)[j];
            }
        }
    }
}

}

using namespace sessd;

extern "C" long long sessd_bev_skip_plan_words(int batch, int h, int w, int *offsets) {
    SkipPlan P;
    const long long words = skip_plan(P, batch, h, w);
    if (words && offsets)
        for (int i = 0; i < kSkipLaunches; ++i) offsets[i] = P.l[i].rec;
    return words;
}

extern "C" int sessd_bev_skip_plan(const void *d_bitmap_index, sessd_grid grid, int *d_plan, void *stream) {
    if (!d_bitmap_index || !d_plan || grid.shape[0] < 1) return SESSD_EINVAL;
    SkipPlan P;
    if (!skip_plan(P, grid.batch, grid.shape[1], grid.shape[2])) return SESSD_EINVAL;
    P.depth = grid.shape[0];
    const int smem = 4 * (kNumFullMaps * P.h * P.nwf + (kNumMaps - kNumFullMaps) * P.h2 * P.nwh);
    if (smem > 200 * 1024) return SESSD_EINVAL;
    static int attr_smem = 48 * 1024;
    if (smem > attr_smem) {
        SESSD_CUDA_TRY(cudaFuncSetAttribute(bev_skip_plan_kernel, cudaFuncAttributeMaxDynamicSharedMemorySize, smem));
        attr_smem = smem;
    }
    SESSD_LAUNCH(bev_skip_plan_kernel, 1, kSkipThreads, smem, (cudaStream_t)stream, (const uint2 *)d_bitmap_index, d_plan, P);
    return last_error();
}

extern "C" int sessd_bev_skip_fill(const int *d_record, float *d_out_f32, void *d_out_planes, int cout, void *stream) {
    if (!d_record || (!d_out_f32 && !d_out_planes) || cout < 8 || cout % 8) return SESSD_EINVAL;
    SESSD_LAUNCH(bev_skip_fill_kernel, 2 * kNumSMs, 256, 0, (cudaStream_t)stream, d_record, d_out_f32, (__half *)d_out_planes, cout);
    return last_error();
}
```

### se-ssd_b200/sessd_b200/_lib.py

```python
import ctypes as C
import os

_HERE = os.path.dirname(os.path.abspath(__file__))
LIB_PATH = os.path.join(os.path.dirname(_HERE), "libsessd_b200.so")
LAB_PATH = os.path.join(os.path.dirname(_HERE), "libsessd_b200_lab.so")


class SessdError(RuntimeError):
    pass


class VoxelCfg(C.Structure):
    _fields_ = [("voxel_size", C.c_float * 3), ("range_min", C.c_float * 3), ("range_max", C.c_float * 3),
                ("grid", C.c_int * 3), ("max_points", C.c_int), ("max_voxels", C.c_int), ("num_feat", C.c_int)]


class Grid(C.Structure):
    _fields_ = [("batch", C.c_int), ("shape", C.c_int * 3)]


class ConvDesc(C.Structure):
    _fields_ = [("batch", C.c_int), ("in_h", C.c_int), ("in_w", C.c_int), ("cin", C.c_int),
                ("out_h", C.c_int), ("out_w", C.c_int), ("cout", C.c_int),
                ("grid_h", C.c_int), ("grid_w", C.c_int), ("in_stride", C.c_int),
                ("out_stride", C.c_int), ("out_off_y", C.c_int), ("out_off_x", C.c_int),
                ("ntaps", C.c_int), ("tap_dy", C.c_int * 16), ("tap_dx", C.c_int * 16), ("relu", C.c_int)]


class DinmsCfg(C.Structure):
    _fields_ = [("cnt_thresh", C.c_float), ("dist_edge", C.c_float * 4), ("sigma2", C.c_float * 3), ("suppressed_thresh", C.c_float),
                ("centerness_pow", C.c_float), ("centerness", C.c_int)]


class PostCfg(C.Structure):
    _fields_ = [("batch", C.c_int), ("num_anchors", C.c_int), ("anchors_per_loc", C.c_int), ("head_stride", C.c_int),
                ("score_thresh", C.c_float), ("nms_pre_max", C.c_int), ("nms_post_max", C.c_int),
                ("nms_iou_thresh", C.c_float), ("nms_ge", C.c_int), ("post_range", C.c_float * 6),
                ("direction_offset", C.c_float), ("use_frustum", C.c_int), ("nms_mode", C.c_int), ("dinms", DinmsCfg)]


class KittiFrames(C.Structure):
    _fields_ = [("num_frames", C.c_int), ("gt_off", C.c_void_p), ("gt", C.c_void_p), ("gt_code", C.c_void_p),
                ("gt_occluded", C.c_void_p), ("dc_off", C.c_void_p), ("dc", C.c_void_p), ("dt_off", C.c_void_p),
                ("dt_cnt", C.c_void_p), ("dt", C.c_void_p), ("dt_code", C.c_void_p), ("ov_off", C.c_void_p)]


_vp, _i, _f, _sz, _ll = C.c_void_p, C.c_int, C.c_float, C.c_size_t, C.c_longlong
_I3 = C.POINTER(C.c_int)

SIGNATURES = {
    "sessd_version": (C.c_char_p, []),
    "sessd_launch_count": (_ll, []),
    "sessd_voxelize_workspace_bytes": (_sz, [_i, _i, C.POINTER(VoxelCfg)]),
    "sessd_voxelize": (_i, [_vp, _vp, _i, _i, C.POINTER(VoxelCfg), _vp, _vp, _vp, _vp, _vp, _vp, _sz, _vp]),
    "sessd_voxelize_host": (_i, [_vp, _i, C.POINTER(VoxelCfg), _vp, _vp, _vp]),
    "sessd_hash_bytes": (_sz, [_i, _I3]),
    "sessd_hash_build": (_i, [_vp, _vp, _i, Grid, _vp, _i, _vp]),
    "sessd_bitmap_words": (_sz, [Grid]),
    "sessd_scan_scratch_bytes": (_sz, [_sz]),
    "sessd_subm_rulebook": (_i, [_vp, _vp, _i, Grid, _I3, _i, _vp, _i, _vp, _vp]),
    "sessd_strided_rulebook": (_i, [_vp, _vp, _i, Grid, _i, _vp, _i, _I3, _I3, _I3, Grid, _vp, _vp, _vp, _vp, _i, _vp, _vp, _vp]),
    "sessd_tile_list_stride": (_i, [_i]),
    "sessd_rulebook_tile_lists": (_i, [_vp, _i, _vp, _i, _vp, _vp]),
    "sessd_spconv_forward": (_i, [_vp, _i, _vp, _i, _vp, _i, _vp, _i, _vp, _vp, _i, _vp, _vp]),
    "sessd_spconv_forward_rows": (_i, [_vp, _i, _vp, _i, _vp, _i, _vp, _i, _vp, _vp, _i, _vp, _vp, _vp]),
    "sessd_spconv_forward_rows_planes": (_i, [_vp, _i, _vp, _i, _vp, _i, _vp, _i, _vp, _vp, _i, _vp, _f, _f, _vp, _vp, _i, _vp, _vp]),
    "sessd_spconv_forward_cg": (_i, [_vp, _i, _i, _vp, _vp, _i, _vp, _i, _vp, _i, _vp, _vp, _i, _f, _f, _vp, _vp, _vp, _vp]),
    "sessd_set_sp_cg_deep": (None, [_i]),
    "sessd_spconv_cg_blocks_per_sm": (_i, [_i, _i, _i]),
    "sessd_absmax_rows": (_i, [_vp, _vp, _i, _i, _vp, _vp]),
    "sessd_rulebook_transpose": (_i, [_vp, _i, _vp, _i, _i, _vp, _vp]),
    "sessd_sparse_split_planes": (_i, [_vp, _vp, _i, _i, _vp, _vp, _i, _vp]),
    "sessd_dense_grad_gather": (_i, [_vp, _vp, _vp, _i, _i, Grid, _vp, _vp]),
    "sessd_spconv_wgrad_items": (_i, [_i, _i]),
    "sessd_spconv_wgrad_workspace_bytes": (_sz, [_i, _i, _i, _i]),
    "sessd_spconv_wgrad_rows": (_i, [_vp, _i, _vp, _i, _vp, _i, _vp, _i, _vp, _vp, _sz, _vp]),
    "sessd_spconv_wgrad_cg": (_i, [_vp, _i, _vp, _vp, _i, _vp, _vp, _i, _vp, _i, _vp, _vp, _sz, _vp]),
    "sessd_sparse_to_dense_indexed": (_i, [_vp, _i, _vp, _i, Grid, _vp, _vp]),
    "sessd_sparse_to_dense": (_i, [_vp, _vp, _vp, _i, _i, Grid, _vp, _vp]),
    "sessd_bev_conv_p2": (_i, [_vp, _vp, _vp, _i, _vp, _vp, _vp, _vp, _f, _f, _vp, _vp, _vp, C.POINTER(ConvDesc), _vp, _vp]),
    "sessd_bev_deconv_p2": (_i, [_vp, _vp, _vp, _i, _vp, _vp, _vp, _vp, _f, _f, _vp, _vp, _vp, _i, _i, _i, _i, _i, _i, _vp, _vp]),
    "sessd_bev_skip_plan_words": (_ll, [_i, _i, _i, _I3]),
    "sessd_bev_skip_plan": (_i, [_vp, Grid, _vp, _vp]),
    "sessd_bev_skip_fill": (_i, [_vp, _vp, _vp, _i, _vp]),
    "sessd_bev_wgrad_items": (_i, [C.POINTER(ConvDesc)]),
    "sessd_bev_wgrad_workspace_bytes": (_sz, [C.POINTER(ConvDesc)]),
    "sessd_bev_wgrad": (_i, [_vp, _vp, _vp, _vp, C.POINTER(ConvDesc), _vp, _vp, _sz, _vp]),
    "sessd_bev_split_planes": (_i, [_vp, _ll, _vp, _vp, _vp]),
    "sessd_sparse_to_dense_planes": (_i, [_vp, _i, _vp, _i, Grid, _vp, _vp, _vp, _vp]),
    "sessd_ssfa_fuse_planes": (_i, [_vp, _vp, _vp, _vp, _f, _f, _f, _f, _i, _i, _vp, _vp, _vp, _vp, _vp, _vp]),
    "sessd_absmax": (_i, [_vp, C.c_longlong, _vp, _vp]),
    "sessd_postprocess_workspace_bytes": (_sz, [C.POINTER(PostCfg)]),
    "sessd_postprocess": (_i, [_vp, _vp, _vp, C.POINTER(PostCfg), _vp, _vp, _vp, _vp, _vp, _vp, _vp, _sz, _vp]),
    "sessd_postprocess_packed": (_i, [_vp, _vp, _vp, C.POINTER(PostCfg), _vp, _vp, _vp, _vp, _vp, _vp, _vp, _vp, _vp, _vp, _vp, _sz, _vp]),
    "sessd_rotate_nms_workspace_bytes": (_sz, [_i, _i]),
    "sessd_rotate_nms": (_i, [_vp, _vp, _vp, _i, _i, _i, _f, _i, _vp, _vp, _vp, _sz, _vp]),
    "sessd_rotate_weighted_nms_workspace_bytes": (_sz, [_i, _i]),
    "sessd_rotate_weighted_nms": (_i, [_vp, _vp, _vp, _vp, _vp, _vp, _vp, _vp, _i, _i, C.POINTER(DinmsCfg), _vp, _vp, _vp, _vp, _vp, _vp, _vp,
                                       _vp, _sz, _vp]),
    "sessd_boxes_overlap_bev": (_i, [_vp, _i, _vp, _i, _vp, _vp]),
    "sessd_boxes_aligned_overlap_bev": (_i, [_vp, _vp, _i, _vp, _vp]),
    "sessd_boxes_iou_bev": (_i, [_vp, _i, _vp, _i, _vp, _vp]),
    "sessd_boxes_iou3d": (_i, [_vp, _i, _vp, _i, _vp, _vp]),
    "sessd_nms_workspace_bytes": (_sz, [_i]),
    "sessd_nms_sorted": (_i, [_vp, _i, _f, _i, _vp, _vp, _vp, _sz, _vp]),
    "sessd_head_loss_workspace_bytes": (_sz, [_i]),
    "sessd_head_loss": (_i, [_vp, _vp, _vp, _vp, _i, _i, _i, _i, _f, _f, _f, _f, _f, _f, _f, _f, _vp, _vp, _vp, _sz, _vp]),
    "sessd_odiou_loss_workspace_bytes": (_sz, [_i]),
    "sessd_odiou_loss": (_i, [_vp, _vp, _vp, _vp, _i, _i, _i, _i, _f, _vp, _vp, _vp, _vp, _sz, _vp]),
    "sessd_odiou_pairs_host": (_i, [_vp, _vp, _i, _vp, _vp]),
    "sessd_iou_pred_loss_workspace_bytes": (_sz, [_i]),
    "sessd_iou_pred_loss": (_i, [_vp, _vp, _vp, _vp, _i, _i, _i, _i, _f, _f, _vp, _vp, _vp, _sz, _vp]),
    "sessd_axpby": (_i, [_vp, _vp, _f, _f, _ll, _vp]),
    "sessd_adamw_step": (_i, [_vp, _vp, _vp, _vp, _ll, _f, _f, _f, _f, _f, _i, _vp]),
    "sessd_grad_sqnorm_workspace_bytes": (_sz, [_ll]),
    "sessd_grad_sqnorm": (_i, [_vp, _ll, _f, _vp, _vp, _vp]),
    "sessd_adamw_clip_ema_step": (_i, [_vp, _vp, _vp, _vp, _ll, _f, _f, _f, _f, _f, _i, _vp, _vp, C.c_double, _vp]),
    "sessd_assign_workspace_bytes": (_sz, [_i, _i, _i]),
    "sessd_assign_targets": (_i, [_vp, _i, _vp, _vp, _i, _i, _f, _f, _vp, _vp, _vp, _vp, _vp, _vp, _vp, _sz, _vp]),
    "sessd_box_collision": (_i, [_vp, _i, _vp, _i, _vp, _vp]),
    "sessd_noise_per_box": (_i, [_vp, _vp, _vp, _i, _i, _vp, _vp, _i, C.c_double, _vp, _vp]),
    "sessd_points_in_boxes": (_i, [_vp, _i, _i, _vp, _i, C.c_double, _vp, _vp]),
    "sessd_augment_points": (_i, [_vp, _vp, _i, _i, _vp, _vp, _vp, _i, _vp, _vp, _i, _vp, C.c_double, _vp, _vp, _vp, _vp, _vp, _vp]),
    "sessd_augment_boxes": (_i, [_vp, _vp, _vp, _vp, _i, _i, _vp, _vp, _i, _vp, _vp, C.POINTER(C.c_float), _vp, _vp, _vp, _vp, _vp, _vp, _vp]),
    "sessd_gtaug_select_host": (_i, [_vp, _i, _i, _vp]),
    "sessd_gtaug_paste_workspace_bytes": (_sz, [_i, _i, _i]),
    "sessd_gtaug_paste": (_i, [_vp, _vp, _i, _i, _vp, _vp, _i, _i, _vp, _vp, _vp, _vp, _i, _vp, _sz, _vp, _i, _vp, _vp]),
    "sessd_sada_pyramids": (_i, [_vp, _i, _vp, _vp, _vp]),
    "sessd_sada_membership": (_i, [_vp, _i, _vp, _vp, _i, _vp, _i, _vp, _vp, _vp]),
    "sessd_sada_compact_workspace_bytes": (_sz, [_i]),
    "sessd_sada_compact": (_i, [_vp, _i, _vp, _vp, _i, _vp, _i, _vp, _sz, _vp, _i, _vp, _vp]),
    "sessd_sada_fps_workspace_bytes": (_sz, [_i, _i]),
    "sessd_sada_fps": (_i, [_vp, _i, _vp, _vp, _i, _vp, _i, _i, _vp, _sz, _vp, _i, _vp, _vp]),
    "sessd_sada_swap": (_i, [_vp, _i, _vp, _vp, _i, _vp, _vp, _i, _vp, _i, _vp, _i, _vp, _vp, _vp]),
    "sessd_sada_shuffle": (_i, [_vp, _vp, _i, _i, _vp, _vp, _vp]),
    "sessd_prep_frustum_compact_workspace_bytes": (_sz, [_i]),
    "sessd_prep_frustum_compact": (_i, [_vp, _vp, _i, _i, _vp, _vp, _sz, _vp, _i, _vp, _vp]),
    "sessd_prep_box_count": (_i, [_vp, _vp, _i, _i, _vp, _vp, _i, _vp, _vp]),
    "sessd_prep_box_gather_workspace_bytes": (_sz, [_i]),
    "sessd_prep_box_gather": (_i, [_vp, _vp, _i, _i, _vp, _vp, _vp, _i, _vp, _i, _vp, _sz, _vp, _i, _vp, _vp]),
    "sessd_kitti_convert_workspace_bytes": (_sz, [_ll]),
    "sessd_kitti_convert_detections": (_i, [_vp, _vp, _vp, _vp, _i, _ll, _vp, _vp, _vp, _i, _vp, _vp, _vp, _vp, _vp, _sz, _vp]),
    "sessd_kitti_overlaps": (_i, [C.POINTER(KittiFrames), _i, _i, C.c_double, _vp, _vp]),
    "sessd_kitti_eval_workspace_bytes": (_sz, [_i, _ll, _ll, _i, _i]),
    "sessd_kitti_eval": (_i, [C.POINTER(KittiFrames), _i, _i, _i, C.c_double, _i, _vp, _vp, _i, _ll, _ll, _vp, _vp, _vp, _vp, _vp, _vp,
                              _sz, _vp]),
}


LAB_SIGNATURES = {
    "sessd_bev_conv_h2": (_i, [_vp, _vp, _i, _vp, _vp, _vp, _vp, C.POINTER(ConvDesc), _vp, _vp, _vp]),
    "sessd_bev_deconv_h2": (_i, [_vp, _vp, _i, _vp, _vp, _vp, _vp, _i, _i, _i, _i, _i, _i, _vp, _vp, _vp]),
    "sessd_bev_conv_p2_profile": (_i, [_vp, _vp, _vp, _i, _vp, _vp, _vp, _vp, _f, _f, _vp, _vp, _vp, C.POINTER(ConvDesc), _vp, _vp, _vp]),
    "sessd_bev_deconv_p2_profile": (_i, [_vp, _vp, _vp, _i, _vp, _vp, _vp, _vp, _f, _f, _vp, _vp, _vp, _i, _i, _i, _i, _i, _i, _vp, _vp,
                                         _vp]),
    "sessd_bev_conv_p2_loads": (_i, [_vp, _vp, _vp, _i, _vp, _vp, _vp, _vp, _f, _f, _vp, _vp, _vp, C.POINTER(ConvDesc), _vp, _i, _vp, _vp]),
    "sessd_bev_p2_plan": (_i, [C.POINTER(ConvDesc), _i, _i, _i, _i, _I3]),
}


def _load(path, signatures, mode=C.DEFAULT_MODE):
    if not os.path.exists(path):
        raise ImportError(
            "sessd_b200: %s is missing -- the CUDA library has not been built (run `python se-ssd_b200/build.py`). "
            "There is no CPU fallback." % path)
    lib = C.CDLL(path, mode=mode)
    for name, (res, args) in signatures.items():
        fn = getattr(lib, name)
        fn.restype = res
        fn.argtypes = args
    return lib


class _Libs:

    def __init__(self):
        self._prod = _load(LIB_PATH, SIGNATURES, C.RTLD_GLOBAL)
        self._lab = None

    def lab(self):
        if self._lab is None:
            self._lab = _load(LAB_PATH, LAB_SIGNATURES)
        return self._lab

    @property
    def lab_loaded(self):
        return self._lab is not None

    def __getattr__(self, name):
        if name in LAB_SIGNATURES:
            return getattr(self.lab(), name)
        return getattr(self._prod, name)


lib = _Libs()


def check(rc, what):
    if rc != 0:
        kind = {-1: "invalid argument", -2: "capacity exceeded", -3: "workspace too small"}.get(rc, "cudaError %d" % rc)
        raise SessdError("%s failed: %s" % (what, kind))


def version():
    return lib.sessd_version().decode()


def launch_count():
    return int(lib.sessd_launch_count())
```

### se-ssd_b200/sessd_b200/ops.py

```python
import ctypes as C

import numpy as np
import torch

from . import _lib
from ._lib import ConvDesc, DinmsCfg, Grid, PostCfg, VoxelCfg, check, lib


def _p(t):
    return C.c_void_p(t.data_ptr()) if t is not None else C.c_void_p(0)


def _st():
    return C.c_void_p(torch.cuda.current_stream().cuda_stream)


def _cuda(t, dtype, name):
    if not (isinstance(t, torch.Tensor) and t.is_cuda and t.dtype == dtype and t.is_contiguous()):
        raise ValueError("%s must be a contiguous CUDA %s tensor" % (name, dtype))
    return t


def _i3(v):
    return (C.c_int * 3)(*[int(x) for x in v])


def make_grid(batch, shape_dhw):
    g = Grid()
    g.batch = int(batch)
    g.shape[0], g.shape[1], g.shape[2] = [int(v) for v in shape_dhw]
    return g


def make_voxel_cfg(voxel_size, pc_range, max_points, max_voxels, num_feat=4):
    cfg = VoxelCfg()
    vs = np.asarray(voxel_size, np.float32)
    rg = np.asarray(pc_range, np.float32)
    grid = np.round((rg[3:] - rg[:3]) / vs).astype(np.int64)
    for j in range(3):
        cfg.voxel_size[j] = float(vs[j])
        cfg.range_min[j] = float(rg[j])
        cfg.range_max[j] = float(rg[3 + j])
        cfg.grid[j] = int(grid[j])
    cfg.max_points, cfg.max_voxels, cfg.num_feat = int(max_points), int(max_voxels), int(num_feat)
    return cfg


class VoxelBuffers:

    def __init__(self, cfg, batch, max_total_points, device, with_mean=True):
        self.cfg, self.batch, self.max_total_points = cfg, batch, max_total_points
        nv = batch * cfg.max_voxels
        self.voxels = torch.empty((nv, cfg.max_points, cfg.num_feat), dtype=torch.float32, device=device)
        self.coors = torch.empty((nv, 4), dtype=torch.int32, device=device)
        self.num_points = torch.empty((nv,), dtype=torch.int32, device=device)
        self.mean = torch.empty((nv, cfg.num_feat), dtype=torch.float32, device=device) if with_mean else None
        self.num_voxels = torch.zeros((batch + 1,), dtype=torch.int32, device=device)
        ws = lib.sessd_voxelize_workspace_bytes(max_total_points, batch, C.byref(cfg))
        self.ws = torch.empty((ws,), dtype=torch.uint8, device=device)


def voxelize(points, frame_off, buf):
    _cuda(points, torch.float32, "points")
    _cuda(frame_off, torch.int32, "frame_off")
    if points.shape[0] > buf.max_total_points or points.shape[1] != buf.cfg.num_feat or frame_off.numel() != buf.batch + 1:
        raise ValueError("voxelize: shape/capacity mismatch")
    rc = lib.sessd_voxelize(_p(points), _p(frame_off), buf.batch, buf.max_total_points, C.byref(buf.cfg), _p(buf.voxels),
                            _p(buf.coors), _p(buf.num_points), _p(buf.mean), _p(buf.num_voxels), _p(buf.ws), buf.ws.numel(), _st())
    check(rc, "sessd_voxelize")
    return buf


def voxelize_host(points_np, cfg):
    pts = np.ascontiguousarray(points_np, np.float32)
    if pts.ndim != 2 or pts.shape[1] != cfg.num_feat:
        raise ValueError("points must be [N,%d]" % cfg.num_feat)
    voxels = np.zeros((cfg.max_voxels, cfg.max_points, cfg.num_feat), np.float32)
    coors = np.zeros((cfg.max_voxels, 3), np.int32)
    num = np.zeros((cfg.max_voxels,), np.int32)
    m = lib.sessd_voxelize_host(pts.ctypes.data_as(C.c_void_p), pts.shape[0], C.byref(cfg), voxels.ctypes.data_as(C.c_void_p),
                                coors.ctypes.data_as(C.c_void_p), num.ctypes.data_as(C.c_void_p))
    if m < 0:
        raise _lib.SessdError("sessd_voxelize_host failed (%d)" % m)
    return voxels[:m].copy(), coors[:m].copy(), num[:m].copy()


def hash_capacity(max_rows):
    cap = C.c_int(0)
    lib.sessd_hash_bytes(int(max_rows), C.byref(cap))
    return cap.value


def hash_build(coors, n, max_rows, grid, table=None):
    cap = hash_capacity(max_rows)
    if table is None:
        table = torch.empty((cap,), dtype=torch.int64, device=coors.device)
    check(lib.sessd_hash_build(_p(coors), _p(n), int(max_rows), grid, _p(table), cap, _st()), "sessd_hash_build")
    return table


def bitmap_alloc(grid, device):
    words = lib.sessd_bitmap_words(grid)
    bitmap = torch.empty((words, 2), dtype=torch.int32, device=device)
    scratch = torch.empty((lib.sessd_scan_scratch_bytes(words),), dtype=torch.uint8, device=device)
    return bitmap, scratch


def subm_rulebook(coors, n, max_rows, grid, ksize, index_kind, index, nbr=None):
    kvol = int(ksize[0] * ksize[1] * ksize[2])
    if nbr is None:
        nbr = torch.empty((max_rows, kvol), dtype=torch.int32, device=coors.device)
    cap = index.numel() if index_kind == 0 else 0
    check(lib.sessd_subm_rulebook(_p(coors), _p(n), int(max_rows), grid, _i3(ksize), int(index_kind), _p(index), cap, _p(nbr), _st()),
          "sessd_subm_rulebook")
    return nbr


def strided_rulebook(in_coors, n_in, max_in, in_grid, in_index_kind, in_index, ksize, stride, padding, out_grid, bitmap,
                     scratch, out_coors, n_out, max_out, nbr, status):
    cap = in_index.numel() if in_index_kind == 0 else 0
    check(lib.sessd_strided_rulebook(_p(in_coors), _p(n_in), int(max_in), in_grid, int(in_index_kind), _p(in_index), cap, _i3(ksize),
                                     _i3(stride), _i3(padding), out_grid, _p(bitmap), _p(scratch), _p(out_coors), _p(n_out),
                                     int(max_out), _p(nbr), _p(status), _st()), "sessd_strided_rulebook")


def spconv_forward(in_feat, nbr, n_out, max_out, weight, scale, shift, relu, out=None):
    kvol, cin, cout = weight.shape
    if out is None:
        out = torch.empty((max_out, cout), dtype=torch.float32, device=in_feat.device)
    check(lib.sessd_spconv_forward(_p(in_feat), int(cin), _p(nbr), int(kvol), _p(n_out), int(max_out), _p(weight), int(cout),
                                   _p(scale), _p(shift), int(bool(relu)), _p(out), _st()), "sessd_spconv_forward")
    return out


def spconv_forward_rows(in_feat, nbr, n_out, max_out, weight, scale, shift, relu, out, amax_out=None):
    kvol, cin, cout = weight.shape
    check(lib.sessd_spconv_forward_rows(_p(in_feat), int(cin), _p(nbr), int(kvol), _p(n_out), int(max_out), _p(weight), int(cout),
                                        _p(scale), _p(shift), int(bool(relu)), _p(out), _p(amax_out), _st()), "sessd_spconv_forward_rows")
    return out


def _fp16_split(wt):
    amax = wt.abs().amax(dim=(0, 2))
    _, ex = torch.frexp(amax)
    e = torch.where(amax > 0, 11 - ex, torch.zeros_like(ex)).clamp(-100, 100).to(torch.float32)
    ws = wt * torch.exp2(e)[None, :, None]
    hi = ws.to(torch.float16)
    return hi, (ws - hi.to(torch.float32)).to(torch.float16), torch.exp2(-e).contiguous()


def pack_weight_sp_h2(wp, cp):
    kvol, cin, cout = wp.shape
    assert cp in (32, 64) and cin == cp
    hi, lo, inv = _fp16_split(wp.permute(0, 2, 1).contiguous().to(torch.float32))
    return torch.stack([hi, lo], 1).contiguous(), inv


def alloc_planes(max_rows, cp, device):
    return torch.zeros((max_rows + 1, 2 * cp), dtype=torch.float16, device=device)


def absmax_rows(feat, n, max_rows, amax):
    check(lib.sessd_absmax_rows(_p(feat), _p(n), int(max_rows), int(feat.shape[1]), _p(amax), _st()), "sessd_absmax_rows")
    return amax


def spconv_forward_rows_planes(in_feat, nbr, n_out, max_out, weight, scale, shift, relu, amax_in, gain, shift_max, out, out_planes, out_info):
    kvol, cin, cout = weight.shape
    check(lib.sessd_spconv_forward_rows_planes(_p(in_feat), int(cin), _p(nbr), int(kvol), _p(n_out), int(max_out), _p(weight), int(cout),
                                               _p(scale), _p(shift), int(bool(relu)), _p(amax_in), float(gain), float(shift_max), _p(out),
                                               _p(out_planes), int(out_planes.shape[1] // 2), _p(out_info), _st()),
          "sessd_spconv_forward_rows_planes")
    return out_planes


def alloc_tile_lists(max_out, kvol, device):
    return torch.zeros((-(-int(max_out) // 128), int(lib.sessd_tile_list_stride(int(kvol)))), dtype=torch.int32, device=device)


def rulebook_tile_lists(nbr, n_out, max_out, tiles):
    check(lib.sessd_rulebook_tile_lists(_p(nbr), int(nbr.shape[1]), _p(n_out), int(max_out), _p(tiles), _st()), "sessd_rulebook_tile_lists")
    return tiles


def spconv_forward_cg(in_planes, in_info, tiles, n_out, max_out, weight_h2, scale, shift, relu, gain, shift_max, out, out_planes, out_info):
    cp = in_planes.shape[1] // 2
    kvol = weight_h2.shape[0]
    cout = weight_h2.shape[2]
    check(lib.sessd_spconv_forward_cg(_p(in_planes), int(cp), int(in_planes.shape[0]), _p(in_info), _p(tiles), int(kvol), _p(n_out), int(max_out),
                                      _p(weight_h2), int(cout), _p(scale), _p(shift), int(bool(relu)), float(gain), float(shift_max), _p(out),
                                      _p(out_planes), _p(out_info), _st()), "sessd_spconv_forward_cg")
    return out if out is not None else out_planes


def set_sp_cg_deep(on):
    lib.sessd_set_sp_cg_deep(int(on))


def spconv_cg_blocks_per_sm(cp, cout, deep=0):
    n = int(lib.sessd_spconv_cg_blocks_per_sm(int(cp), int(cout), int(deep)))
    check(min(n, 0), "sessd_spconv_cg_blocks_per_sm")
    return n


def rulebook_transpose(nbr, n_out, max_out, max_in, nbr_t=None):
    kvol = int(nbr.shape[1])
    if nbr_t is None:
        nbr_t = torch.empty((int(max_in), kvol), dtype=torch.int32, device=nbr.device)
    check(lib.sessd_rulebook_transpose(_p(nbr), kvol, _p(n_out), int(max_out), int(max_in), _p(nbr_t), _st()), "sessd_rulebook_transpose")
    return nbr_t


def sparse_split_planes(x, n, max_rows, info, planes):
    check(lib.sessd_sparse_split_planes(_p(x), _p(n), int(max_rows), int(x.shape[1]), _p(info), _p(planes), int(planes.shape[1] // 2), _st()),
          "sessd_sparse_split_planes")
    return planes


def dense_grad_gather(grad, coors, n, max_rows, grid, channels, out=None):
    if out is None:
        out = torch.empty((int(max_rows), int(channels)), dtype=torch.float32, device=grad.device)
    check(lib.sessd_dense_grad_gather(_p(grad), _p(coors), _p(n), int(max_rows), int(channels), grid, _p(out), _st()), "sessd_dense_grad_gather")
    return out


def wgrad_items(max_out, kvol):
    return int(lib.sessd_spconv_wgrad_items(int(max_out), int(kvol)))


def wgrad_workspace(max_out, kvol, cin, cout, device):
    return torch.empty((int(lib.sessd_spconv_wgrad_workspace_bytes(int(max_out), int(kvol), int(cin), int(cout))),), dtype=torch.uint8,
                       device=device)


def spconv_wgrad_rows(in_feat, gout, tiles, n_out, max_out, kvol, gw=None, ws=None):
    cin, cout = int(in_feat.shape[1]), int(gout.shape[1])
    if gw is None:
        gw = torch.empty((int(kvol), cin, cout), dtype=torch.float32, device=gout.device)
    if ws is None:
        ws = wgrad_workspace(max_out, kvol, cin, cout, gout.device)
    check(lib.sessd_spconv_wgrad_rows(_p(in_feat), cin, _p(gout), cout, _p(tiles), int(kvol), _p(n_out), int(max_out), _p(gw), _p(ws), ws.numel(),
                                      _st()), "sessd_spconv_wgrad_rows")
    return gw


def spconv_wgrad_cg(in_planes, in_info, g_planes, g_info, tiles, n_out, max_out, kvol, gw=None, ws=None):
    cp, cout = int(in_planes.shape[1] // 2), int(g_planes.shape[1] // 2)
    if gw is None:
        gw = torch.empty((int(kvol), cp, cout), dtype=torch.float32, device=g_planes.device)
    if ws is None:
        ws = wgrad_workspace(max_out, kvol, cp, cout, g_planes.device)
    check(lib.sessd_spconv_wgrad_cg(_p(in_planes), cp, _p(in_info), _p(g_planes), cout, _p(g_info), _p(tiles), int(kvol), _p(n_out), int(max_out),
                                    _p(gw), _p(ws), ws.numel(), _st()), "sessd_spconv_wgrad_cg")
    return gw


def sparse_planes_to_float(planes, info, channels):
    cp = planes.shape[1] // 2
    return (planes[:, :channels].float() + planes[:, cp:cp + channels].float()) / info[1]


def sparse_to_dense(feat, coors, n, max_rows, grid, out=None):
    c = feat.shape[1]
    d, h, w = grid.shape[0], grid.shape[1], grid.shape[2]
    if out is None:
        out = torch.empty((grid.batch, h, w, c * d), dtype=torch.float32, device=feat.device)
    check(lib.sessd_sparse_to_dense(_p(feat), _p(coors), _p(n), int(max_rows), int(c), grid, _p(out), _st()), "sessd_sparse_to_dense")
    return out


def sparse_to_dense_indexed(feat, bitmap_index, grid, out):
    check(lib.sessd_sparse_to_dense_indexed(_p(feat), int(feat.shape[0]), _p(bitmap_index), int(feat.shape[1]), grid, _p(out), _st()),
          "sessd_sparse_to_dense_indexed")
    return out


def conv_desc(batch, in_hw, cin, out_hw, cout, grid_hw, taps, in_stride=1, out_stride=1, out_off=(0, 0), relu=True):
    d = ConvDesc()
    d.batch, d.in_h, d.in_w, d.cin = int(batch), int(in_hw[0]), int(in_hw[1]), int(cin)
    d.out_h, d.out_w, d.cout = int(out_hw[0]), int(out_hw[1]), int(cout)
    d.grid_h, d.grid_w = int(grid_hw[0]), int(grid_hw[1])
    d.in_stride, d.out_stride, d.out_off_y, d.out_off_x = int(in_stride), int(out_stride), int(out_off[0]), int(out_off[1])
    d.ntaps = len(taps)
    for t, (dy, dx) in enumerate(taps):
        d.tap_dy[t], d.tap_dx[t] = int(dy), int(dx)
    d.relu = int(bool(relu))
    return d


def pack_weight_h2(wp, cout_pad):
    taps, cin, cout = wp.shape
    wt = torch.zeros((taps, cout_pad, cin), dtype=torch.float32, device=wp.device)
    wt[:, :cout] = wp.permute(0, 2, 1)
    hi, lo, inv = _fp16_split(wt)
    return torch.stack([hi, lo], 0).contiguous(), inv


def bev_conv_h2(x, weight_h2, scale, shift, residual, out, desc, amax_in=None, amax_out=None):
    check(lib.sessd_bev_conv_h2(_p(x), _p(weight_h2), int(weight_h2.shape[2]), _p(scale), _p(shift), _p(residual), _p(out), C.byref(desc),
                                _p(amax_in), _p(amax_out), _st()), "sessd_bev_conv_h2")
    return out


def bev_deconv_h2(x, weight_h2, scale, shift, residual, out, relu=True, amax_in=None, amax_out=None):
    b, h, w, cin = x.shape
    check(lib.sessd_bev_deconv_h2(_p(x), _p(weight_h2), int(weight_h2.shape[2]), _p(scale), _p(shift), _p(residual), _p(out),
                                  int(b), int(h), int(w), int(cin), int(out.shape[-1]), int(bool(relu)), _p(amax_in), _p(amax_out), _st()),
          "sessd_bev_deconv_h2")
    return out


def alloc_bev_planes(batch, h, w, c, device):
    return torch.zeros((2, batch, h, w, c), dtype=torch.float16, device=device)


def conv_gain(wp, scale):
    g = wp.abs().sum(dim=(0, 1)) * scale.abs().to(wp.device)[: wp.shape[2]]
    return float(g.max()) * (1.0 + 1e-5)


def bev_conv_p2(in_planes, in_info, weight_h2, scale, shift, residual, resid_info, gain, shift_max, out_f32, out_planes, out_info, desc,
                items=None):
    check(lib.sessd_bev_conv_p2(_p(in_planes), _p(in_info), _p(weight_h2), int(weight_h2.shape[2]), _p(scale), _p(shift), _p(residual),
                                _p(resid_info), float(gain), float(shift_max), _p(out_f32), _p(out_planes), _p(out_info), C.byref(desc),
                                _p(items), _st()), "sessd_bev_conv_p2")


def bev_deconv_p2(in_planes, in_info, weight_h2, scale, shift, residual, resid_info, gain, shift_max, out_f32, out_planes, out_info, relu=True,
                  items=None):
    _two, b, h, w, cin = in_planes.shape
    cout = (out_f32 if out_f32 is not None else out_planes).shape[-1]
    check(lib.sessd_bev_deconv_p2(_p(in_planes), _p(in_info), _p(weight_h2), int(weight_h2.shape[2]), _p(scale), _p(shift), _p(residual),
                                  _p(resid_info), float(gain), float(shift_max), _p(out_f32), _p(out_planes), _p(out_info), int(b), int(h),
                                  int(w), int(cin), int(cout), int(bool(relu)), _p(items), _st()), "sessd_bev_deconv_p2")


class BevSkipPlan:

    LAUNCHES = 13

    def __init__(self, batch, h, w, device):
        offs = (C.c_int * self.LAUNCHES)()
        words = lib.sessd_bev_skip_plan_words(int(batch), int(h), int(w), offs)
        if words <= 0:
            raise ValueError("no skip plan for a [%d, %d, %d] neck" % (batch, h, w))
        self.offsets = list(offs)
        self.buf = torch.zeros((int(words),), dtype=torch.int32, device=device)

    def record(self, i):
        return self.buf[self.offsets[i]:]

    def build(self, bitmap_index, grid):
        check(lib.sessd_bev_skip_plan(_p(bitmap_index), grid, _p(self.buf), _st()), "sessd_bev_skip_plan")

    def fill(self, i, out_f32, out_planes, cout):
        check(lib.sessd_bev_skip_fill(_p(self.record(i)), _p(out_f32), _p(out_planes), int(cout), _st()), "sessd_bev_skip_fill")


def bev_split_planes(x, info, planes):
    check(lib.sessd_bev_split_planes(_p(x), int(x.numel()), _p(info), _p(planes), _st()), "sessd_bev_split_planes")
    return planes


def bev_wgrad_workspace(desc, device):
    n = int(lib.sessd_bev_wgrad_workspace_bytes(C.byref(desc)))
    if n == 0:
        raise ValueError("sessd_bev_wgrad: no weight gradient for this descriptor")
    return torch.empty((n,), dtype=torch.uint8, device=device)


def bev_wgrad(in_planes, in_info, g_planes, g_info, desc, gw=None, ws=None):
    if gw is None:
        gw = torch.empty((desc.ntaps, desc.cin, desc.cout), dtype=torch.float32, device=g_planes.device)
    if ws is None:
        ws = bev_wgrad_workspace(desc, g_planes.device)
    check(lib.sessd_bev_wgrad(_p(in_planes), _p(in_info), _p(g_planes), _p(g_info), C.byref(desc), _p(gw), _p(ws), ws.numel(), _st()),
          "sessd_bev_wgrad")
    return gw


def planes_to_float(planes, info):
    return (planes[0].float() + planes[1].float()) / info[1]


def sparse_to_dense_planes(feat, bitmap_index, grid, amax, info, planes):
    check(lib.sessd_sparse_to_dense_planes(_p(feat), int(feat.shape[0]), _p(bitmap_index), int(feat.shape[1]), grid, _p(amax), _p(info),
                                           _p(planes), _st()), "sessd_sparse_to_dense_planes")
    return planes


def ssfa_fuse_planes(x0, x1, w0, w1, s0, t0, s1, t1, out, info0, info1, out_info, planes):
    npix = x0.numel() // x0.shape[-1]
    check(lib.sessd_ssfa_fuse_planes(_p(x0), _p(x1), _p(w0), _p(w1), float(s0), float(t0), float(s1), float(t1), int(npix), int(x0.shape[-1]),
                                     _p(out), _p(info0), _p(info1), _p(out_info), _p(planes), _st()), "sessd_ssfa_fuse_planes")
    return out


def absmax(x, amax):
    check(lib.sessd_absmax(_p(x), int(x.numel()), _p(amax), _st()), "sessd_absmax")
    return amax


NMS_TYPES = ("rotate_nms", "rotate_weighted_nms")
DINMS_MAX_PRE = 4096


def make_dinms_cfg(nms_cnt_thresh=2.6, nms_sigma_dist_interval=(0, 20, 40, 60), nms_sigma_square=(0.0009, 0.009, 0.1, 1),
                   suppressed_thresh=0.3, centerness_pow=2, enable_centerness=True):
    if len(nms_sigma_dist_interval) != 4 or len(nms_sigma_square) < 3:
        raise ValueError("DI-NMS takes four distance edges (three bands) and their three sigma^2")
    d = DinmsCfg()
    d.cnt_thresh, d.suppressed_thresh, d.centerness_pow = float(nms_cnt_thresh), float(suppressed_thresh), float(centerness_pow)
    for j in range(4):
        d.dist_edge[j] = float(nms_sigma_dist_interval[j])
    for j in range(3):
        d.sigma2[j] = float(nms_sigma_square[j])
    d.centerness = int(bool(enable_centerness))
    return d


def make_post_cfg(batch, num_anchors=70400, anchors_per_loc=2, head_stride=24, score_thresh=0.3, nms_pre_max=1000, nms_post_max=100,
                  nms_iou_thresh=0.01, nms_ge=True, post_range=(0, -40.0, -5.0, 70.4, 40.0, 5.0), direction_offset=0.0,
                  use_frustum=False, nms_type="rotate_nms"):
    if nms_type not in NMS_TYPES:
        raise ValueError("nms_type must be one of %s, not %r" % (NMS_TYPES, nms_type))
    c = PostCfg()
    c.batch, c.num_anchors, c.anchors_per_loc, c.head_stride = int(batch), int(num_anchors), int(anchors_per_loc), int(head_stride)
    c.score_thresh, c.nms_pre_max, c.nms_post_max = float(score_thresh), int(nms_pre_max), int(nms_post_max)
    c.nms_iou_thresh, c.nms_ge = float(nms_iou_thresh), int(bool(nms_ge))
    for j in range(6):
        c.post_range[j] = float(post_range[j])
    c.direction_offset, c.use_frustum = float(direction_offset), int(bool(use_frustum))
    if nms_type == "rotate_weighted_nms":
        c.nms_mode, c.dinms = 1, make_dinms_cfg()
    return c


def post_capacity(cfg):
    return cfg.nms_pre_max if cfg.nms_mode == 1 else cfg.nms_post_max


class PostBuffers:
    def __init__(self, cfg, device):
        self.cfg = cfg
        b, p = cfg.batch, post_capacity(cfg)
        self.boxes = torch.zeros((b, p, 7), dtype=torch.float32, device=device)
        self.scores = torch.zeros((b, p), dtype=torch.float32, device=device)
        self.labels = torch.zeros((b, p), dtype=torch.int32, device=device)
        self.count = torch.zeros((b,), dtype=torch.int32, device=device)
        self.aux = torch.zeros((b, 4), dtype=torch.int32, device=device)
        self.sel_anchor = torch.zeros((b, p), dtype=torch.int32, device=device)
        self.ws = torch.empty((lib.sessd_postprocess_workspace_bytes(C.byref(cfg)),), dtype=torch.uint8, device=device)


def postprocess(head, anchors, frustum_planes, buf):
    check(lib.sessd_postprocess(_p(head), _p(anchors), _p(frustum_planes), C.byref(buf.cfg), _p(buf.boxes), _p(buf.scores), _p(buf.labels),
                                _p(buf.count), _p(buf.aux), _p(buf.sel_anchor), _p(buf.ws), buf.ws.numel(), _st()), "sessd_postprocess")
    return buf


def postprocess_packed(head, anchors, frustum_planes, buf, packed, meta, num_voxels=None, status=None):
    check(lib.sessd_postprocess_packed(_p(head), _p(anchors), _p(frustum_planes), C.byref(buf.cfg), _p(buf.boxes), _p(buf.scores),
                                       _p(buf.labels), _p(buf.count), _p(buf.aux), _p(buf.sel_anchor), _p(packed), _p(meta),
                                       _p(num_voxels), _p(status), _p(buf.ws), buf.ws.numel(), _st()), "sessd_postprocess_packed")
    return buf


def rotate_nms(boxes5, scores, n, max_boxes, pre_max, post_max, iou_thresh, ge=True):
    dev = boxes5.device
    keep = torch.empty((post_max,), dtype=torch.int32, device=dev)
    num = torch.zeros((1,), dtype=torch.int32, device=dev)
    ws = torch.empty((lib.sessd_rotate_nms_workspace_bytes(int(max_boxes), int(pre_max)),), dtype=torch.uint8, device=dev)
    check(lib.sessd_rotate_nms(_p(boxes5), _p(scores), _p(n), int(max_boxes), int(pre_max), int(post_max), float(iou_thresh),
                               int(bool(ge)), _p(keep), _p(num), _p(ws), ws.numel(), _st()), "sessd_rotate_nms")
    return keep, num


def rotate_weighted_nms(boxes7, boxes5, scores, iou_preds, labels, dirs, anchors, n, max_boxes, pre_max, dinms_cfg, ws=None):
    dev = scores.device
    for t, dt, name in ((boxes7, torch.float32, "boxes7"), (boxes5, torch.float32, "boxes5"), (scores, torch.float32, "scores"),
                        (iou_preds, torch.float32, "iou_preds"), (labels, torch.int32, "labels"), (dirs, torch.int32, "dirs"),
                        (n, torch.int32, "n")):
        _cuda(t, dt, name)
    if anchors is not None:
        _cuda(anchors, torch.float32, "anchors")
    p = int(pre_max)
    out = dict(boxes=torch.empty((p, 7), dtype=torch.float32, device=dev), scores=torch.empty((p,), dtype=torch.float32, device=dev),
               labels=torch.empty((p,), dtype=torch.int32, device=dev), dirs=torch.empty((p,), dtype=torch.int32, device=dev),
               keep=torch.empty((p,), dtype=torch.int32, device=dev), selected=torch.empty((p,), dtype=torch.int32, device=dev),
               count=torch.zeros((2,), dtype=torch.int32, device=dev))
    if ws is None:
        ws = torch.empty((max(lib.sessd_rotate_weighted_nms_workspace_bytes(int(max_boxes), p), 1),), dtype=torch.uint8, device=dev)
    check(lib.sessd_rotate_weighted_nms(_p(boxes7), _p(boxes5), _p(scores), _p(iou_preds), _p(labels), _p(dirs), _p(anchors), _p(n),
                                        int(max_boxes), p, C.byref(dinms_cfg), _p(out["boxes"]), _p(out["scores"]), _p(out["labels"]),
                                        _p(out["dirs"]), _p(out["keep"]), _p(out["selected"]), _p(out["count"]), _p(ws), ws.numel(),
                                        _st()), "sessd_rotate_weighted_nms")
    return out


def boxes_overlap_bev(a, b, out):
    check(lib.sessd_boxes_overlap_bev(_p(a), a.shape[0], _p(b), b.shape[0], _p(out), _st()), "sessd_boxes_overlap_bev")
    return out


def boxes_aligned_overlap_bev(a, b, out):
    check(lib.sessd_boxes_aligned_overlap_bev(_p(a), _p(b), a.shape[0], _p(out), _st()), "sessd_boxes_aligned_overlap_bev")
    return out


def boxes_iou_bev(a, b, out):
    check(lib.sessd_boxes_iou_bev(_p(a), a.shape[0], _p(b), b.shape[0], _p(out), _st()), "sessd_boxes_iou_bev")
    return out


def boxes_iou3d(a, b, out):
    check(lib.sessd_boxes_iou3d(_p(a), a.shape[0], _p(b), b.shape[0], _p(out), _st()), "sessd_boxes_iou3d")
    return out


def nms_sorted(boxes, thresh, mode):
    n = boxes.shape[0]
    dev = boxes.device
    keep = torch.empty((max(n, 1),), dtype=torch.int64, device=dev)
    num = torch.zeros((1,), dtype=torch.int32, device=dev)
    ws = torch.empty((lib.sessd_nms_workspace_bytes(n),), dtype=torch.uint8, device=dev)
    check(lib.sessd_nms_sorted(_p(boxes), n, float(thresh), int(mode), _p(keep), _p(num), _p(ws), ws.numel(), _st()), "sessd_nms_sorted")
    return keep, num


class AssignBuffers:

    def __init__(self, num_anchors, batch, max_gt, device):
        self.num_anchors, self.batch, self.max_gt = int(num_anchors), int(batch), int(max_gt)
        z = lambda shape, dt: torch.zeros(shape, dtype=dt, device=device)
        self.labels = z((batch, num_anchors), torch.int32)
        self.bbox_targets = z((batch, num_anchors, 7), torch.float32)
        self.bbox_outside_weights = z((batch, num_anchors), torch.float32)
        self.pos_anchor = z((batch, num_anchors), torch.int32)
        self.pos_gt_id = z((batch, num_anchors), torch.int32)
        self.num_pos = z((batch,), torch.int32)
        self.ws = torch.empty((lib.sessd_assign_workspace_bytes(self.num_anchors, self.batch, self.max_gt),), dtype=torch.uint8,
                              device=device)


def assign_targets(anchors, gt_boxes, num_gt, buf, matched_thr=0.6, unmatched_thr=0.45):
    _cuda(anchors, torch.float32, "anchors"); _cuda(gt_boxes, torch.float32, "gt_boxes"); _cuda(num_gt, torch.int32, "num_gt")
    assert anchors.shape == (buf.num_anchors, 7) and tuple(gt_boxes.shape) == (buf.batch, buf.max_gt, 7) and num_gt.numel() == buf.batch
    check(lib.sessd_assign_targets(_p(anchors), buf.num_anchors, _p(gt_boxes), _p(num_gt), buf.batch, buf.max_gt, float(matched_thr),
                                   float(unmatched_thr), _p(buf.labels), _p(buf.bbox_targets), _p(buf.bbox_outside_weights),
                                   _p(buf.pos_anchor), _p(buf.pos_gt_id), _p(buf.num_pos), _p(buf.ws), buf.ws.numel(), _st()),
          "sessd_assign_targets")
    return buf


def head_loss(head, anchors, labels, reg_targets, alpha=0.25, sigma=3.0, dir_offset=0.0, pos_cls_weight=1.0, neg_cls_weight=1.0,
              w_cls=1.0, w_loc=2.0, w_dir=0.2, w_iou=None, with_grad=True):
    _cuda(head, torch.float32, "head"); _cuda(anchors, torch.float32, "anchors"); _cuda(labels, torch.int32, "labels")
    _cuda(reg_targets, torch.float32, "reg_targets")
    B, A = labels.shape
    assert head.shape[0] == B and head.shape[1] * 2 == A and anchors.shape == (A, 7) and tuple(reg_targets.shape) == (B, A, 7)
    losses = torch.empty((B, 8), dtype=torch.float32, device=head.device)
    grad = torch.empty_like(head) if with_grad else None
    ws = torch.empty((lib.sessd_head_loss_workspace_bytes(int(B)),), dtype=torch.uint8, device=head.device)
    check(lib.sessd_head_loss(_p(head), _p(anchors), _p(labels), _p(reg_targets), int(B), int(A), 2, int(head.shape[2]), float(alpha), float(sigma),
                              float(dir_offset), float(pos_cls_weight), float(neg_cls_weight), float(w_cls), float(w_loc), float(w_dir),
                              _p(losses), _p(grad), _p(ws), ws.numel(), _st()), "sessd_head_loss")
    if w_iou is not None:
        ws2 = torch.empty((lib.sessd_iou_pred_loss_workspace_bytes(int(B)),), dtype=torch.uint8, device=head.device)
        check(lib.sessd_iou_pred_loss(_p(head), _p(anchors), _p(labels), _p(reg_targets), int(B), int(A), 2, int(head.shape[2]), float(sigma),
                                      float(w_iou), _p(losses), _p(grad), _p(ws2), ws2.numel(), _st()), "sessd_iou_pred_loss")
    return losses, grad


def odiou_pairs_host(gboxes, qboxes, with_grad=True):
    g = np.ascontiguousarray(gboxes, np.float32).reshape(-1, 7)
    q = np.ascontiguousarray(qboxes, np.float32).reshape(-1, 7)
    assert g.shape == q.shape
    out = np.zeros((g.shape[0],), np.float32)
    grad = np.zeros_like(q) if with_grad else None
    check(lib.sessd_odiou_pairs_host(g.ctypes.data_as(C.c_void_p), q.ctypes.data_as(C.c_void_p), int(g.shape[0]), out.ctypes.data_as(C.c_void_p),
                                     grad.ctypes.data_as(C.c_void_p) if with_grad else C.c_void_p(0)), "sessd_odiou_pairs_host")
    return out, grad


def odiou_loss(head, anchors, labels, reg_targets, losses, grad_head=None, w_odiou=2.0):
    B, A = labels.shape
    out = torch.empty((B,), dtype=torch.float32, device=head.device)
    ws = torch.empty((lib.sessd_odiou_loss_workspace_bytes(int(B)),), dtype=torch.uint8, device=head.device)
    check(lib.sessd_odiou_loss(_p(head), _p(anchors), _p(labels), _p(reg_targets), int(B), int(A), 2, int(head.shape[2]), float(w_odiou),
                               _p(losses), _p(out), _p(grad_head), _p(ws), ws.numel(), _st()), "sessd_odiou_loss")
    return out


def box_collision(boxes, qboxes, out=None):
    _cuda(boxes, torch.float64, "boxes"); _cuda(qboxes, torch.float64, "qboxes")
    n, k = boxes.shape[0], qboxes.shape[0]
    if out is None:
        out = torch.empty((n, k), dtype=torch.uint8, device=boxes.device)
    check(lib.sessd_box_collision(_p(boxes), int(n), _p(qboxes), int(k), _p(out), _st()), "sessd_box_collision")
    return out


def _aug_inputs(gt_boxes, num_gt, valid, loc_noise, rot_noise, selected=None):
    _cuda(gt_boxes, torch.float32, "gt_boxes"); _cuda(num_gt, torch.int32, "num_gt"); _cuda(valid, torch.uint8, "valid")
    _cuda(loc_noise, torch.float64, "loc_noise"); _cuda(rot_noise, torch.float64, "rot_noise")
    B, M = valid.shape
    T = rot_noise.shape[2]
    if (tuple(gt_boxes.shape) != (B, M, 7) or num_gt.numel() != B or tuple(loc_noise.shape) != (B, M, T, 3)
            or tuple(rot_noise.shape) != (B, M, T)):
        raise ValueError("augmentation inputs: shape mismatch")
    if selected is not None:
        _cuda(selected, torch.int32, "selected")
        if tuple(selected.shape) != (B, M):
            raise ValueError("selected must be [B, M]")
    return B, M, T


def points_in_boxes(points, boxes, context=-1.0, mask=None):
    _cuda(points, torch.float32, "points"); _cuda(boxes, torch.float32, "boxes")
    if points.dim() != 2 or points.shape[1] < 3 or boxes.dim() != 2 or boxes.shape[1] != 7:
        raise ValueError("points_in_boxes: points [N, >=3], boxes [M, 7]")
    n, m = points.shape[0], boxes.shape[0]
    if mask is None:
        mask = torch.empty((n, m), dtype=torch.uint8, device=points.device)
    check(lib.sessd_points_in_boxes(_p(points), int(n), int(points.shape[1]), _p(boxes), int(m), float(context), _p(mask), _st()),
          "sessd_points_in_boxes")
    return mask


def noise_per_box(gt_boxes, num_gt, valid, loc_noise, rot_noise, context=-1.0, selected=None):
    B, M, T = _aug_inputs(gt_boxes, num_gt, valid, loc_noise, rot_noise)
    if selected is None:
        selected = torch.empty((B, M), dtype=torch.int32, device=gt_boxes.device)
    _cuda(selected, torch.int32, "selected")
    check(lib.sessd_noise_per_box(_p(gt_boxes), _p(num_gt), _p(valid), int(B), int(M), _p(loc_noise), _p(rot_noise), int(T),
                                  float(context), _p(selected), _st()), "sessd_noise_per_box")
    return selected


def augment_points(points, frame_off, max_frame_points, gt_boxes, num_gt, valid, loc_noise, rot_noise, selected, glob, perm, labeled=None,
                   context=-1.0, points_raw=None, points_out=None, with_raw=True):
    B, M, T = _aug_inputs(gt_boxes, num_gt, valid, loc_noise, rot_noise, selected)
    _cuda(points, torch.float32, "points"); _cuda(frame_off, torch.int32, "frame_off"); _cuda(glob, torch.float32, "glob")
    _cuda(perm, torch.int32, "perm")
    if labeled is not None:
        _cuda(labeled, torch.uint8, "labeled")
        if labeled.numel() != B:
            raise ValueError("labeled must be [B]")
    if points.dim() != 2 or points.shape[1] != 4 or frame_off.numel() != B + 1 or perm.numel() != points.shape[0] or tuple(glob.shape) != (B, 5):
        raise ValueError("augment_points: shape mismatch")
    if not with_raw:
        points_raw = None
    elif points_raw is None:
        points_raw = torch.empty_like(points)
    if points_out is None:
        points_out = torch.empty_like(points)
    written = (("points_raw", points_raw), ("points_out", points_out)) if with_raw else (("points_out", points_out),)
    for name, t in written:
        _cuda(t, torch.float32, name)
# ... 253 lines not shown
```

### se-ssd_b200/sessd_b200/runners.py

```python
import itertools
import math

import torch
from sessd_data.layers import SPMIDDLE_LAYERS
from sessd_data.layers import SSFA_LAUNCHES, ssfa_extents

from . import ops

BN_EPS = 1e-3

def conv_out_shape(shape, ksize, stride, padding):
    return tuple((int(i) + 2 * p - k) // s + 1 for i, k, s, p in zip(shape, ksize, stride, padding))


def fold_bn(gamma, beta, mean, var, eps=BN_EPS):
    scale = gamma.float() / torch.sqrt(var.float() + eps)
    shift = beta.float() - mean.float() * scale
    return scale.contiguous(), shift.contiguous()


def sparse_impl(cin, use_tc=True):
    if not use_tc:
        return "simt"
    return "rows" if cin <= 16 else "cg"


def plane_width(channels):
    return 32 if channels <= 32 else 64


def spmiddle_plan(use_tc=True, keep_f32=False, cin0=4):
    plan, cin, lvl = [], cin0, 0
    for kind, cout, ks, st, pd, key in SPMIDDLE_LAYERS:
        lout = lvl if kind == "subm" else lvl + 1
        rb = key if kind == "subm" else "sp%d" % lout
        impl = sparse_impl(cin, use_tc)
        plan.append(dict(kind=kind, key=key, ks=ks, st=st, pd=pd, cin=cin, cout=cout, lin=lvl, lout=lout, rb=rb,
                         build_rb=all(p["rb"] != rb for p in plan), impl=impl, cp_in=plane_width(cin) if impl == "cg" else None))
        cin, lvl = cout, lout
    nxt = {}
    for p in reversed(plan):
        p["tile_lists"] = p["build_rb"] and any(q["impl"] == "cg" for q in plan if q["rb"] == p["rb"])
        p["cp_out"] = nxt.get("cp_in")
        p["out_f32"] = keep_f32 or p["cp_out"] is None
        p["out_info"] = p["impl"] == "cg" or p["cp_out"] is not None or (nxt.get("impl") == "rows" and nxt["cp_out"] is not None)
        nxt = p
    return plan


class SpMiddleRunner:

    GROWTH = (1.0, 4.0, 6.0, 5.0, 3.0)

    def __init__(self, batch, max_voxels_total, input_shape_xyz=(1408, 1600, 40), num_input_features=4, device="cuda",
                 growth=None, use_tc=True, keep_f32=False):
        self.batch, self.device = batch, torch.device(device)
        self.use_tc, self.keep_f32 = bool(use_tc), bool(keep_f32)
        shape = (int(input_shape_xyz[2]) + 1, int(input_shape_xyz[1]), int(input_shape_xyz[0]))
        growth = growth or self.GROWTH
        self.levels = []
        self._add_level(shape, int(max_voxels_total), hash_index=True)
        self.plan = spmiddle_plan(self.use_tc, self.keep_f32, num_input_features)
        rulebooks = {}
        for p in self.plan:
            if p["kind"] != "subm":
                oshape = conv_out_shape(self.levels[p["lin"]]["shape"], p["ks"], p["st"], p["pd"])
                cells = batch * oshape[0] * oshape[1] * oshape[2]
                self._add_level(oshape, min(cells, int(math.ceil(max_voxels_total * growth[p["lout"]]))), hash_index=False)
            if p["build_rb"]:
                cap, kvol = self.levels[p["lout"]]["cap"], p["ks"][0] * p["ks"][1] * p["ks"][2]
                rulebooks[p["rb"]] = (torch.empty((cap, kvol), dtype=torch.int32, device=self.device),
                                      ops.alloc_tile_lists(cap, kvol, self.device) if p["tile_lists"] else None)
            p["nbr"], p["tiles"] = rulebooks[p["rb"]]
        caps = [self.levels[p["lout"]]["cap"] for p in self.plan]
        self.feats = [torch.zeros((cap, p["cout"]), dtype=torch.float32, device=self.device) if p["out_f32"] else None
                      for p, cap in zip(self.plan, caps)]
        self.planes = [ops.alloc_planes(cap, p["cp_out"], self.device) if p["cp_out"] else None for p, cap in zip(self.plan, caps)]
        assert all(pl is None or pl.shape[0] <= (1 << 25) for pl in self.planes)
        last = self.levels[-1]
        self.out_channels = self.plan[-1]["cout"] * last["shape"][0]
        self.dense = torch.zeros((batch, last["shape"][1], last["shape"][2], self.out_channels), dtype=torch.float32,
                                 device=self.device)
        self.status = torch.zeros((1,), dtype=torch.int32, device=self.device)
        self.weights = None
        self.info = torch.zeros((len(self.plan), 2), dtype=torch.float32, device=self.device)

    def layer_output(self, li):
        p = self.plan[li]
        if p["out_f32"]:
            return self.feats[li]
        return ops.sparse_planes_to_float(self.planes[li][:-1], self.info[li], p["cout"])

    def _add_level(self, shape, cap, hash_index):
        grid = ops.make_grid(self.batch, shape)
        lv = dict(shape=shape, cap=cap, grid=grid, n=torch.zeros((1,), dtype=torch.int32, device=self.device))
        if hash_index:
            lv["index_kind"] = 0
            lv["index"] = torch.empty((ops.hash_capacity(cap),), dtype=torch.int64, device=self.device)
            lv["coors"] = None
        else:
            lv["index_kind"] = 1
            lv["index"], lv["scratch"] = ops.bitmap_alloc(grid, self.device)
            lv["coors"] = torch.zeros((cap, 4), dtype=torch.int32, device=self.device)
        self.levels.append(lv)

    def load_weights(self, layers):
        assert len(layers) == len(self.plan)
        self.weights = []
        for p, l in zip(self.plan, layers):
            w = torch.as_tensor(l["weight"], dtype=torch.float32, device=self.device)
            assert tuple(w.shape) == (*p["ks"], p["cin"], p["cout"]), (w.shape, p)
            sc, sh = fold_bn(*[torch.as_tensor(l[k], device=self.device) for k in ("gamma", "beta", "mean", "var")], eps=float(l.get("eps", BN_EPS)))
            wp = w.reshape(-1, p["cin"], p["cout"]).contiguous()
            p["gain"], p["shift_max"] = ops.conv_gain(wp, sc), float(sh.abs().max())
            if p["impl"] == "cg":
                tiles, inv = ops.pack_weight_sp_h2(wp, p["cp_in"])
                self.weights.append((tiles, (sc * inv).contiguous(), sh))
            else:
                self.weights.append((wp, sc, sh))

    def forward(self, feat0, coors0, n0, mark=None, dense_planes=None):
        mark = mark or (lambda label: None)
        assert self.weights is not None, "load_weights first"
        L0 = self.levels[0]
        cap0 = min(coors0.shape[0], L0["cap"])
        L0["coors"], L0["n_ext"] = coors0, n0
        ops.hash_build(coors0, n0, cap0, L0["grid"], L0["index"])
        mark("hash_build")
        if self.use_tc:
            self.info.zero_()
        x = feat0
        for li, p in enumerate(self.plan):
            lin, lout = self.levels[p["lin"]], self.levels[p["lout"]]
            n_in = lin["n_ext"] if p["lin"] == 0 else lin["n"]
            cap_in = cap0 if p["lin"] == 0 else lin["cap"]
            n_out, cap_out = (n_in, cap_in) if p["kind"] == "subm" else (lout["n"], lout["cap"])
            if p["build_rb"]:
                if p["kind"] == "subm":
                    ops.subm_rulebook(lin["coors"], n_in, cap_in, lin["grid"], p["ks"], lin["index_kind"], lin["index"], p["nbr"])
                else:
                    ops.strided_rulebook(lin["coors"], n_in, cap_in, lin["grid"], lin["index_kind"], lin["index"], p["ks"], p["st"],
                                         p["pd"], lout["grid"], lout["index"], lout["scratch"], lout["coors"], lout["n"], lout["cap"],
                                         p["nbr"], self.status)
                if p["tiles"] is not None:
                    ops.rulebook_tile_lists(p["nbr"], n_out, cap_out, p["tiles"])
                mark("rulebook:" + p["rb"])
            w, sc, sh = self.weights[li]
            out = self.feats[li]
            if p["impl"] == "rows" and p["cp_out"]:
                ops.spconv_forward_rows_planes(x, p["nbr"], n_out, cap_out, w, sc, sh, True, self.info[li - 1, 0:1], p["gain"], p["shift_max"],
                                               out, self.planes[li], self.info[li])
            elif p["impl"] == "rows":
                ops.spconv_forward_rows(x, p["nbr"], n_out, cap_out, w, sc, sh, True, out, self.info[li, 0:1] if p["out_info"] else None)
            elif p["impl"] == "cg":
                ops.spconv_forward_cg(self.planes[li - 1], self.info[li - 1], p["tiles"], n_out, cap_out, w, sc, sh, True, p["gain"],
                                      p["shift_max"], out, self.planes[li], self.info[li])
            else:
                ops.spconv_forward(x, p["nbr"], n_out, cap_out, w, sc, sh, True, out)
            mark("conv:%d" % li)
            x = out
        last = self.levels[-1]
        if dense_planes is not None:
            assert self.plan[-1]["out_info"], "the planes' scale needs the last layer's abs-max (use_tc)"
            out = ops.sparse_to_dense_planes(x, last["index"], last["grid"], self.info[-1, 0:1], dense_planes[1], dense_planes[0])
        else:
            out = ops.sparse_to_dense_indexed(x, last["index"], last["grid"], self.dense)
        mark("dense")
        return out


class RunnerCache:

    def __init__(self):
        self.runner = self.key = self.weights = None

    def get(self, module, key, build, load):
        if self.runner is None or key != self.key:
            self.runner, self.key, self.weights = build(), key, None
        weights = tuple((t.data_ptr(), t._version) for t in itertools.chain(module.parameters(), module.buffers()))
        if weights != self.weights:
            load(self.runner)
            self.weights = weights
        return self.runner


_SSFA = {L.name: L for L in SSFA_LAUNCHES}


def conv_taps(k):
    return [(dy - k // 2, dx - k // 2) for dy in range(k) for dx in range(k)]


def _pack_conv(w):
    cout, cin, kh, kw = w.shape
    packed = w.permute(2, 3, 1, 0).reshape(kh * kw, cin, cout).contiguous()
    return packed, [(ky, kx) for ky in range(kh) for kx in range(kw)]


def launch_weight(L, w):
    if L.kind == "deconv":
        return w.permute(2, 3, 0, 1).reshape(9, L.cin, L.cout).contiguous(), None
    return _pack_conv(w)[0], conv_taps(L.k)


def launch_desc(L, batch, in_hw, out_hw, taps, relu=None):
    return ops.conv_desc(batch, in_hw, L.cin, out_hw, L.cout, out_hw, taps, in_stride=L.stride, relu=L.relu if relu is None else relu)


def head_weight(param):
    w, b = (torch.cat([param(c + s) for c in ("conv_box", "conv_cls", "conv_dir", "conv_iou")], 0) for s in (".weight", ".bias"))
    pad = _SSFA["head"].cout - w.shape[0]
    return torch.cat([w, w.new_zeros((pad,) + tuple(w.shape[1:]))], 0), torch.cat([b, b.new_zeros((pad,))], 0)


def pack_head(head_sd, prefix, device):
    return head_weight(lambda name: head_sd[prefix + name].to(device, torch.float32))


def fold_ssfa_bn(sd, conv_name, device, eps=BN_EPS):
    blk, idx = conv_name.rsplit(".", 1)
    b = "%s.%d." % (blk, int(idx) + 1)
    return fold_bn(*(sd[b + k].to(device, torch.float32) for k in ("weight", "bias", "running_mean", "running_var")), eps=eps)


def pack_h2(wp, taps, scale, shift):
    planes, inv = ops.pack_weight_h2(wp, _cout_pad(wp.shape[2]))
    scale = torch.ones(wp.shape[2], device=wp.device) if scale is None else scale
    return dict(w=planes, scale=(scale * inv[:scale.numel()]).contiguous(), shift=shift.contiguous(), gain=ops.conv_gain(wp, scale),
                shift_max=float(shift.abs().max()), taps=taps)


def _cout_pad(cout):
    n_tile = 32 if cout <= 32 else 128
    return -(-cout // n_tile) * n_tile


def ssfa_weights(ssfa_sd, head_sd, head_prefix, device, bn_eps=BN_EPS):
    for L in SSFA_LAUNCHES:
        if L.name != "head":
            wp, taps = launch_weight(L, ssfa_sd[L.name + ".weight"].to(device, torch.float32))
            yield (L, wp, taps) + fold_ssfa_bn(ssfa_sd, L.name, device, bn_eps)
        elif head_sd is not None:
            w, bias = pack_head(head_sd, head_prefix, device)
            yield (L, *launch_weight(L, w), None, bias)


def ssfa_fuse_weights(ssfa_sd, device, bn_eps=BN_EPS):
    out = {}
    for name in ("w_0.0", "w_1.0"):
        sc, sh = fold_ssfa_bn(ssfa_sd, name, device, bn_eps)
        out[name] = (ssfa_sd[name + ".weight"].to(device, torch.float32).reshape(-1).contiguous(), float(sc[0]), float(sh[0]))
    return out


SSFA_SLOT = {n: i for i, n in enumerate(["x"] + [L.dst for L in SSFA_LAUNCHES if not L.f32] + ["out"] + [L.dst for L in SSFA_LAUNCHES if L.f32])}


class SSFAPlanesRunner:

    HEAD_STRIDE = 24
    SLOT = SSFA_SLOT
    SKIP_LAUNCHES = tuple(L.name for L in SSFA_LAUNCHES)

    def __init__(self, batch, hw=(200, 176), device="cuda", skip_constant=False):
        self.batch, self.h, self.w, self.device = batch, int(hw[0]), int(hw[1]), torch.device(device)
        pl = lambda hw_, c: ops.alloc_bev_planes(batch, hw_[0], hw_[1], c, self.device)
        z = lambda hw_, c: torch.zeros((batch,) + hw_ + (c,), dtype=torch.float32, device=self.device)
        H, ext = (self.h, self.w), lambda L: ssfa_extents(L, self.h, self.w)[1]
        self.planes = dict(x=pl(H, 128), **{L.dst: pl(ext(L), L.cout) for L in SSFA_LAUNCHES if not L.f32}, out=pl(H, 128))
        self.buf = dict(**{L.dst: z(ext(L), L.cout) for L in SSFA_LAUNCHES[:-1] if L.f32}, out=z(H, 128), head=z(H, self.HEAD_STRIDE))
        self.info = torch.zeros((16, 2), dtype=torch.float32, device=self.device)
        self.params = None
        self.skip_constant = bool(skip_constant)
        self.skip = ops.BevSkipPlan(batch, self.h, self.w, self.device) if self.skip_constant else None

    def _info(self, name):
        return self.info[self.SLOT[name]]

    def load_state(self, ssfa_sd, head_sd=None, head_prefix="tasks.0.", bn_eps=BN_EPS):
        P = ssfa_fuse_weights(ssfa_sd, self.device, bn_eps)
        for L, *weight in ssfa_weights(ssfa_sd, head_sd, head_prefix, self.device, bn_eps):
            P[L.name] = pack_h2(*weight)
        self.params = P

    def _split(self, x, name):
        self.info.zero_()
        ops.absmax(x, self._info(name)[0:1])
        ops.bev_split_planes(x, self._info(name), self.planes[name])

    def _launch(self, L, skip=False):
        q = self.params[L.name]
        out_f32, out_planes = (self.buf[L.dst], None) if L.f32 else (None, self.planes[L.dst])
        resid, resid_info = (self.buf[L.residual], self._info(L.residual)) if L.residual else (None, None)
        i = self.SKIP_LAUNCHES.index(L.name)
        rec = self.skip.record(i) if skip else None
        if L.kind == "conv":
            d = launch_desc(L, self.batch, *ssfa_extents(L, self.h, self.w), q["taps"])
            ops.bev_conv_p2(self.planes[L.src], self._info(L.src), q["w"], q["scale"], q["shift"], resid, resid_info, q["gain"],
                            q["shift_max"], out_f32, out_planes, self._info(L.dst), d, items=rec)
        else:
            ops.bev_deconv_p2(self.planes[L.src], self._info(L.src), q["w"], q["scale"], q["shift"], resid, resid_info, q["gain"],
                              q["shift_max"], out_f32, out_planes, self._info(L.dst), L.relu, items=rec)
        if skip:
            self.skip.fill(i, out_f32, out_planes, L.cout)

    def forward(self, x=None, mark=None, occupancy=None):
        assert self.params is not None, "load_state first"
        mark = mark or (lambda label: None)
        if x is not None:
            self._split(x, "x")
        skip = self.skip_constant and occupancy is not None
        if skip:
            index, grid = occupancy
            assert (grid.batch, grid.shape[1], grid.shape[2]) == (self.batch, self.h, self.w), "occupancy of another map"
            self.skip.build(index, grid)
            mark("neck:skip_plan")
        for L in SSFA_LAUNCHES[:-1]:
            self._launch(L, skip)
            mark("neck:" + L.name)
        w0, s0, t0 = self.params["w_0.0"]
        w1, s1, t1 = self.params["w_1.0"]
        ops.ssfa_fuse_planes(self.buf["o0"], self.buf["o1"], w0, w1, s0, t0, s1, t1, self.buf["out"], self._info("o0"), self._info("o1"),
                             self._info("out"), self.planes["out"])
        if "head" not in self.params:
            mark("neck:fuse+head")
            return self.buf["out"], None
        self.head(skip=skip)
        mark("neck:fuse+head")
        return self.buf["out"], self.buf["head"]

    def head(self, skip=False):
        self._launch(SSFA_LAUNCHES[-1], skip)
        return self.buf["head"]

    def activation(self, name):
        if name in self.buf:
            return self.buf[name]
        return ops.planes_to_float(self.planes[name], self._info(name))

    def bench_layer(self, name="bottom_up_block_0.4"):

        def launch():
            self._launch(_SSFA[name]._replace(src="x0", dst="b0b"))

        return launch, "bev_conv_p2_kernel (fp16 wgmma from pre-split fp16 planes, two-term split)"


class HeadRunner(SSFAPlanesRunner):

    def __init__(self, batch, hw, device="cuda"):
        self.batch, self.h, self.w, self.device = batch, int(hw[0]), int(hw[1]), torch.device(device)
        self.planes = dict(out=ops.alloc_bev_planes(batch, self.h, self.w, 128, self.device))
        self.buf = dict(head=torch.zeros((batch, self.h, self.w, self.HEAD_STRIDE), dtype=torch.float32, device=self.device))
        self.info = torch.zeros((len(self.SLOT), 2), dtype=torch.float32, device=self.device)
        self.params = None

    def load_state(self, head_sd, prefix=""):
        w, bias = pack_head(head_sd, prefix, self.device)
        self.params = {"head": pack_h2(*launch_weight(_SSFA["head"], w), None, bias)}

    def forward(self, x):
        self._split(x, "out")
        return self.head()
```

Before: 1546.

## Pack occupied BEV row segments into compacted tiles for skip-aware neck convs

Adds a segment-based skip plan that packs occupied row segments from different locations into one GEMM tile, each slot loaded by its own small TMA box. Tiles no longer need to be fully aligned to the spatial grid, so empty area inside partially occupied tiles is not computed. This needs a new plan kernel, a per-slot output coordinate decode in the epilogue, and a separate fill kernel for skipped outputs. The cost is more, smaller TMA loads per item and extra indexing. Layers that have a segment record use this path and the rest fall back to the previous item lists.

```diff
diff --git a/include/sessd_b200.h b/include/sessd_b200.h
--- a/include/sessd_b200.h
+++ b/include/sessd_b200.h
@@ -109,14 +109,16 @@
 int sessd_bev_conv_p2(const void *d_in_planes, const float *d_in_info, const void *d_weight_h2, int cout_pad, const float *d_scale,
                       const float *d_shift, const float *d_residual, const float *d_resid_info, float gain, float shift_max,
                       float *d_out_f32, void *d_out_planes, float *d_out_info, const sessd_conv_desc *desc, const int *d_items,
-                      void *stream);
+                      const int *d_segs, void *stream);
 int sessd_bev_deconv_p2(const void *d_in_planes, const float *d_in_info, const void *d_weight_h2, int cout_pad, const float *d_scale,
                         const float *d_shift, const float *d_residual, const float *d_resid_info, float gain, float shift_max,
                         float *d_out_f32, void *d_out_planes, float *d_out_info, int batch, int in_h, int in_w, int cin, int cout,
-                        int relu, const int *d_items, void *stream);
+                        int relu, const int *d_items, const int *d_segs, void *stream);
 long long sessd_bev_skip_plan_words(int batch, int h, int w, int *offsets);
-int sessd_bev_skip_plan(const void *d_bitmap_index, sessd_grid grid, int *d_plan, void *stream);
+long long sessd_bev_skip_seg_words(int batch, int h, int w, int *offsets);
+int sessd_bev_skip_plan(const void *d_bitmap_index, sessd_grid grid, int *d_plan, int *d_segs, void *stream);
 int sessd_bev_skip_fill(const int *d_record, float *d_out_f32, void *d_out_planes, int cout, void *stream);
+int sessd_bev_skip_fill_segs(const int *d_seg_record, float *d_out_f32, void *d_out_planes, int cout, void *stream);
 int sessd_bev_wgrad_items(const sessd_conv_desc *desc);
 size_t sessd_bev_wgrad_workspace_bytes(const sessd_conv_desc *desc);
 int sessd_bev_wgrad(const void *d_in_planes, const float *d_in_info, const void *d_g_planes, const float *d_g_info,
diff --git a/include/sessd_b200_lab.h b/include/sessd_b200_lab.h
--- a/include/sessd_b200_lab.h
+++ b/include/sessd_b200_lab.h
@@ -17,17 +17,21 @@
 int sessd_bev_conv_p2_profile(const void *d_in_planes, const float *d_in_info, const void *d_weight_h2, int cout_pad,
                               const float *d_scale, const float *d_shift, const float *d_residual, const float *d_resid_info,
                               float gain, float shift_max, float *d_out_f32, void *d_out_planes, float *d_out_info,
-                              const sessd_conv_desc *desc, const int *d_items, long long *d_prof, void *stream);
+                              const sessd_conv_desc *desc, const int *d_items, const int *d_segs, long long *d_prof, void *stream);
 int sessd_bev_deconv_p2_profile(const void *d_in_planes, const float *d_in_info, const void *d_weight_h2, int cout_pad,
                                 const float *d_scale, const float *d_shift, const float *d_residual, const float *d_resid_info,
                                 float gain, float shift_max, float *d_out_f32, void *d_out_planes, float *d_out_info, int batch,
-                                int in_h, int in_w, int cin, int cout, int relu, const int *d_items, long long *d_prof,
-                                void *stream);
+                                int in_h, int in_w, int cin, int cout, int relu, const int *d_items, const int *d_segs,
+                                long long *d_prof, void *stream);
 
 int sessd_bev_conv_p2_loads(const void *d_in_planes, const float *d_in_info, const void *d_weight_h2, int cout_pad,
                             const float *d_scale, const float *d_shift, const float *d_residual, const float *d_resid_info,
                             float gain, float shift_max, float *d_out_f32, void *d_out_planes, float *d_out_info,
                             const sessd_conv_desc *desc, const int *d_items, int smem_a, long long *d_prof, void *stream);
+int sessd_bev_conv_p2_seg_loads(const void *d_in_planes, const float *d_in_info, const void *d_weight_h2, int cout_pad,
+                                const float *d_scale, const float *d_shift, const float *d_residual, const float *d_resid_info,
+                                float gain, float shift_max, float *d_out_f32, void *d_out_planes, float *d_out_info,
+                                const sessd_conv_desc *desc, const int *d_segs, long long *d_prof, void *stream);
 
 int sessd_bev_p2_plan(const sessd_conv_desc *desc, int deconv, int cout_pad, int split, int smem_a, int *plan);
 
diff --git a/se-ssd_b200/csrc/bevconv_p2.cu b/se-ssd_b200/csrc/bevconv_p2.cu
--- a/se-ssd_b200/csrc/bevconv_p2.cu
+++ b/se-ssd_b200/csrc/bevconv_p2.cu
@@ -27,17 +27,17 @@
 extern "C" int sessd_bev_conv_p2(const void *d_in_planes, const float *d_in_info, const void *d_weight_h2, int cout_pad, const float *d_scale,
                                  const float *d_shift, const float *d_residual, const float *d_resid_info, float gain, float shift_max,
                                  float *d_out_f32, void *d_out_planes, float *d_out_info, const sessd_conv_desc *desc, const int *d_items,
-                                 void *stream) {
+                                 const int *d_segs, void *stream) {
     return p2_conv<kP2Planes>(d_in_planes, d_in_info, d_weight_h2, cout_pad, d_scale, d_shift, d_residual, d_resid_info, gain, shift_max,
-                              d_out_f32, d_out_planes, d_out_info, desc, stream, d_items);
+                              d_out_f32, d_out_planes, d_out_info, desc, stream, d_items, nullptr, false, d_segs);
 }
 
 extern "C" int sessd_bev_deconv_p2(const void *d_in_planes, const float *d_in_info, const void *d_weight_h2, int cout_pad, const float *d_scale,
                                    const float *d_shift, const float *d_residual, const float *d_resid_info, float gain, float shift_max,
                                    float *d_out_f32, void *d_out_planes, float *d_out_info, int batch, int in_h, int in_w, int cin, int cout,
-                                   int relu, const int *d_items, void *stream) {
+                                   int relu, const int *d_items, const int *d_segs, void *stream) {
     return p2_deconv<kP2Planes>(d_in_planes, d_in_info, d_weight_h2, cout_pad, d_scale, d_shift, d_residual, d_resid_info, gain, shift_max,
-                                d_out_f32, d_out_planes, d_out_info, batch, in_h, in_w, cin, cout, relu, stream, d_items);
+                                d_out_f32, d_out_planes, d_out_info, batch, in_h, in_w, cin, cout, relu, stream, d_items, nullptr, d_segs);
 }
 
 extern "C" int sessd_bev_split_planes(const float *d_x, long long n, float *d_info, void *d_planes, void *stream) {
diff --git a/se-ssd_b200/csrc/bevconv_p2.cuh b/se-ssd_b200/csrc/bevconv_p2.cuh
--- a/se-ssd_b200/csrc/bevconv_p2.cuh
+++ b/se-ssd_b200/csrc/bevconv_p2.cuh
@@ -16,6 +16,7 @@
 constexpr int kP2MaxSmem = 227 * 1024;
 constexpr int kP2Chunk = 32;
 constexpr int kP2ItemsHeader = 32;
+constexpr int kP2SegHeader = 32, kP2SegSlots = kP2TileV;
 enum { kP2Planes = 0, kP2SplitF16 = 1 };
 enum { kP2NoProbe = 0, kP2ProbeClocks = 1, kP2ProbeLoads = 2 };
 
@@ -45,6 +46,8 @@
     float *out_info;
     long long out_plane_stride;
     const int *items;
+    const int *segs;
+    int slot_rows;
     long long *prof;
 };
 
@@ -64,7 +67,7 @@
     kP2ProfWords = 16
 };
 
-__device__ __forceinline__ int p2_item_count(const P2Params &p) { return p.items ? __ldg(p.items) : p.total; }
+__device__ __forceinline__ int p2_item_count(const P2Params &p) { return p.segs ? __ldg(p.segs) : p.items ? __ldg(p.items) : p.total; }
 __device__ __forceinline__ int p2_item(const P2Params &p, int k) { return p.items ? __ldg(p.items + kP2ItemsHeader + k) : k; }
 
 struct P2ItemIndex { int rank, nb, t; };
@@ -87,6 +90,15 @@
     it.u0 = tu * kP2TileU; it.v0 = tv * kP2TileV;
     it.ntaps = p.cls_ntaps[it.cls];
     return it;
+}
+
+__device__ __forceinline__ const int *p2_seg_group(const P2Params &p, int k) {
+    return p.segs + kP2SegHeader + (k / p.nblocks) * kP2SegSlots;
+}
+struct P2Seg { int b, u0, v; };
+__device__ __forceinline__ P2Seg p2_seg(const P2Params &p, int e) {
+    const int s = e & 0xFFFFFF, rest = s / p.tiles_u;
+    return {rest / p.grid_v, (s - rest * p.tiles_u) * kP2TileU, rest % p.grid_v};
 }
 
 template <int N>
@@ -184,6 +196,23 @@
             uint32_t pph = 0;
             const uint32_t patches_u32 = smem_u32(patches);
             for (int k = blockIdx.x; k < nitems; k += gridDim.x) {
+                if (REGA && p.segs) {
+                    const int e = __ldg(p2_seg_group(p, k) + (lane >> 1));
+                    const P2Seg sg = p2_seg(p, e);
+                    const uint32_t bytes = (uint32_t)__popc(__ballot_sync(0xFFFFFFFFu, e >= 0)) * (uint32_t)p.load_bytes;
+                    const uint32_t dst0 = patches_u32 + (uint32_t)((lane & 1) * p.copy_bytes + (lane >> 1) * p.slot_rows * 64);
+                    for (int cc = 0; cc < nchunks; ++cc) {
+                        { const long long t0 = p2_tick<PROFILE>(); mbar_wait<REGA>(&patch_empty[pb], pph ^ 1u); p2_tock<PROFILE>(clk[kProfPatchEmpty], t0); }
+                        if (elect_one()) mbar_expect_tx(&patch_full[pb], bytes);
+                        __syncwarp();
+                        if (e >= 0)
+                            tma_load_5d(dst0 + (uint32_t)(pb * p.patch_bytes), &map_a, &patch_full[pb], cc * kP2Chunk, sg.u0 + p.copy_u[0],
+                                        sg.v + p.copy_v[0], sg.b, lane & 1);
+                        __syncwarp();
+                        if (++pb == p.npatch) { pb = 0; pph ^= 1u; }
+                    }
+                    continue;
+                }
                 const P2Item it = p2_decode(p, p2_item(p, k));
                 const int bu = it.u0 * p.in_stride, bv = it.v0 * p.in_stride;
                 for (int cc = 0; cc < nchunks; ++cc) {
@@ -217,7 +246,14 @@
             int S = 0;
             uint32_t bph = 0;
             for (int k = blockIdx.x; k < nitems; k += gridDim.x) {
-                const P2Item it = p2_decode(p, p2_item(p, k));
+                P2Item it;
+                if (REGA && p.segs) {
+                    it.cls = __ldg(p2_seg_group(p, k)) >> 24;
+                    it.n0 = (k % p.nblocks) * p.n_tile;
+                    it.ntaps = p.cls_ntaps[it.cls];
+                } else {
+                    it = p2_decode(p, p2_item(p, k));
+                }
                 for (int cc = 0; cc < nchunks; ++cc)
                     for (int tap = 0; tap < it.ntaps; ++tap) {
                         { const long long t0 = p2_tick<PROFILE>(); mbar_wait<REGA>(&b_empty[S], bph ^ 1u); p2_tock<PROFILE>(clk[kProfBEmpty], t0); }
@@ -247,7 +283,7 @@
         const uint32_t patch_lo = desc_lo(smem_u32(patches)) + a_rows;
         const uint32_t plane_lo = b_plane_bytes >> 4;
         const uint32_t copy_lo = (uint32_t)(p.copy_bytes >> 4), patch_sz = (uint32_t)(p.patch_bytes >> 4);
-        const uint32_t a_row = (uint32_t)((wg * 8 + wq * 2 + ((lane >> 3) & 1)) * p.pitch_u + (lane & 7)), a_chunk = (uint32_t)(lane >> 4);
+        const uint32_t a_row = (uint32_t)((wg * 8 + wq * 2 + ((lane >> 3) & 1)) * p.slot_rows + (lane & 7)), a_chunk = (uint32_t)(lane >> 4);
         const uint32_t patches_u32 = smem_u32(patches);
         float amax_in = 0.f, s_in = 1.f;
         if constexpr (MODE == kP2Planes) { amax_in = __ldg(p.in_info); s_in = __ldg(p.in_info + 1); }
@@ -264,7 +300,8 @@
         for (int k = blockIdx.x; k < nitems; k += gridDim.x) {
             const long long t_item = p2_tick<PROFILE>();
             const int g = p2_item(p, k);
-            const int cls = p.cls_order[g / per_cls];
+            const int *grp = REGA && p.segs ? p2_seg_group(p, k) : nullptr;
+            const int cls = grp ? __ldg(grp) >> 24 : p.cls_order[g / per_cls];
             const int ntaps = p.cls_ntaps[cls];
             const uint32_t *aoff = s_aoff + cls * 9;
             float acc[NT];
@@ -375,6 +412,8 @@
                     if (++pb == p.npatch) { pb = 0; pph ^= 1u; }
                 }
             }
+            int seg_e[2] = {-1, -1};
+            if (grp) { seg_e[0] = __ldg(grp + wg * 8 + wq * 2); seg_e[1] = __ldg(grp + wg * 8 + wq * 2 + 1); }
             { const long long t0 = p2_tick<PROFILE>(); wgmma_wait<0>(); p2_tock<PROFILE>(clk[kProfMmaWait], t0); }
             const long long t_epi = p2_tick<PROFILE>();
             wgmma_fence_regs<NT>(acc);
@@ -384,7 +423,7 @@
             }
 #pragma unroll
             for (int i = 0; i < kAcc; ++i) acc[i] = acc[kAcc + i] + acc[i];
-            const P2Item it = p2_decode(p, g);
+            P2Item it = grp ? P2Item{cls, (k % p.nblocks) * p.n_tile, 0, 0, 0, ntaps} : p2_decode(p, g);
             const int q = lane & 3;
             const int r0 = wg * 64 + wq * 16 + (lane >> 2);
             bool rows_ok[2];
@@ -393,6 +432,10 @@
             for (int h = 0; h < 2; ++h) {
                 const int r = r0 + 8 * h;
                 const int lv = r / kP2TileU, lu = r % kP2TileU;
+                if (grp) {
+                    const P2Seg sg = p2_seg(p, seg_e[h]);
+                    it.b = seg_e[h] >= 0 ? sg.b : p.batch; it.u0 = sg.u0; it.v0 = sg.v - lv;
+                }
                 const int gu = it.u0 + lu, gv = it.v0 + lv;
                 rows_ok[h] = it.b < p.batch && gu < p.grid_u && gv < p.grid_v;
                 const int ou = gu * p.out_stride + p.cls_off_u[it.cls], ov = gv * p.out_stride + p.cls_off_v[it.cls];
@@ -535,8 +578,10 @@
     return 0;
 }
 
-static int p2_plan(P2Params &p, const P2Taps *cls, int nclass, int grid_h, int grid_w, int cout_pad, int mode, bool reg_a, int *smem) {
+static int p2_plan(P2Params &p, const P2Taps *cls, int nclass, int grid_h, int grid_w, int cout_pad, int mode, bool reg_a, int *smem,
+                   bool segs = false) {
     if (reg_a && (mode != kP2Planes || p.in_stride != 1)) return SESSD_EINVAL;
+    if (segs && !reg_a) return SESSD_EINVAL;
     if (p.cin < 64 || p.cin % 64) return SESSD_EINVAL;
     P2Geometry g;
     if (p2_geometry(g, p.batch, grid_h, grid_w, p.cout, cout_pad, cls, nclass)) return SESSD_EINVAL;
@@ -592,12 +637,19 @@
         }
     }
     p.copy_bytes = (p.rows_v * p.pitch_u * 64 + 511) & ~511;
+    p.slot_rows = p.pitch_u;
+    if (segs) {
+        const int win = (p.rows_v - kP2TileV + 1) * p.pitch_u;
+        p.slot_rows = (win + 7) & ~7;
+        p.copy_bytes = kP2SegSlots * p.slot_rows * 64;
+    }
     p.patch_bytes = p.ncopies * 2 * p.copy_bytes;
     p.staging_bytes = mode == kP2Planes ? 0 : p.ncopies * p.rows_v * kP2TileU * kP2Chunk * 4;
     p.load_bytes = mode == kP2Planes ? p.ncopies * 2 * p.rows_v * p.pitch_u * 64 : p.staging_bytes;
+    if (segs) p.load_bytes = (p.rows_v - kP2TileV + 1) * p.pitch_u * 64;
     const int per_buf = p.patch_bytes + p.staging_bytes, bstage = 2 * p.n_tile * 64;
     const int tail = 1536 + 16 + 2 * 4 * p.cout;
-    p.npatch = (kP2BStages * bstage + tail + 2 * per_buf <= kP2MaxSmem) ? 2 : 1;
+    p.npatch = (segs || kP2BStages * bstage + tail + 2 * per_buf <= kP2MaxSmem) ? 2 : 1;
     p.bstage_bytes = bstage;
     p.bstages = min((kP2MaxSmem - tail - p.npatch * per_buf) / bstage, kP2MaxBStages);
     if (p.bstages < 2) return SESSD_EINVAL;
@@ -617,8 +669,10 @@
     if (((uintptr_t)d_scale | (uintptr_t)d_shift | (uintptr_t)d_residual | (uintptr_t)d_out_f32 | (uintptr_t)d_out_planes) & 15)
         return SESSD_EINVAL;
     int smem = 0;
-    if (p2_plan(p, cls, nclass, grid_h, grid_w, cout_pad, MODE, reg_a, &smem)) return SESSD_EINVAL;
-    if (p.items && cout_pad != div_up(p.cout, p.n_tile) * p.n_tile) return SESSD_EINVAL;
+    if (p.items && p.segs) return SESSD_EINVAL;
+    if (p2_plan(p, cls, nclass, grid_h, grid_w, cout_pad, MODE, reg_a, &smem, p.segs != nullptr)) return SESSD_EINVAL;
+    if ((p.items || p.segs) && cout_pad != div_up(p.cout, p.n_tile) * p.n_tile) return SESSD_EINVAL;
+    if (p.segs && (long long)p.batch * p.grid_v * p.tiles_u >= (1 << 24)) return SESSD_EINVAL;
     const int s = p.in_stride;
     CUtensorMap map_a, map_b;
     if (MODE != kP2Planes) {
@@ -637,7 +691,8 @@
                                     (cuuint64_t)p.batch, 2};
         const cuuint64_t strides[4] = {p.u_is_x ? row_w : row_h, p.u_is_x ? row_h : row_w, (cuuint64_t)in_h * in_w * p.cin * 2,
                                        (cuuint64_t)p.batch * in_h * in_w * p.cin * 2};
-        const cuuint32_t box[5] = {(cuuint32_t)kP2Chunk, (cuuint32_t)(p.pitch_u * s), (cuuint32_t)(p.rows_v * s), 1, 1};
+        const int box_v = p.segs ? p.rows_v - kP2TileV + 1 : p.rows_v;
+        const cuuint32_t box[5] = {(cuuint32_t)kP2Chunk, (cuuint32_t)(p.pitch_u * s), (cuuint32_t)(box_v * s), 1, 1};
         const cuuint32_t estr[5] = {1, (cuuint32_t)s, (cuuint32_t)s, 1, 1};
         int rc = encode_map_nd(&map_a, d_in_planes, 5, dims, strides, box, estr, CU_TENSOR_MAP_SWIZZLE_64B);
         if (rc) return rc;
@@ -703,13 +758,14 @@
 static int p2_conv(const void *d_in_planes, const float *d_in_info, const void *d_weight_h2, int cout_pad, const float *d_scale,
                    const float *d_shift, const float *d_residual, const float *d_resid_info, float gain, float shift_max,
                    float *d_out_f32, void *d_out_planes, float *d_out_info, const sessd_conv_desc *desc, void *stream,
-                   const int *d_items = nullptr, long long *d_prof = nullptr, bool smem_a = false) {
+                   const int *d_items = nullptr, long long *d_prof = nullptr, bool smem_a = false, const int *d_segs = nullptr) {
     if (!desc || (PROBE != kP2NoProbe && !d_prof)) return SESSD_EINVAL;
     const sessd_conv_desc &d = *desc;
     P2Params p;
     P2Taps t;
     if (p2_conv_params(d, p, t)) return SESSD_EINVAL;
     p.items = d_items;
+    p.segs = d_segs;
     p.prof = d_prof;
     return launch_p2<MODE, PROBE>(d_in_planes, d.in_h, d.in_w, d_in_info, d_weight_h2, d.ntaps, cout_pad, d_scale, d_shift, d_residual, d_resid_info, gain,
                      shift_max, d_out_f32, d_out_planes, d_out_info, p, &t, 1, d.grid_h, d.grid_w, MODE == kP2Planes && d.in_stride == 1 && !smem_a,
@@ -720,12 +776,13 @@
 static int p2_deconv(const void *d_in_planes, const float *d_in_info, const void *d_weight_h2, int cout_pad, const float *d_scale,
                      const float *d_shift, const float *d_residual, const float *d_resid_info, float gain, float shift_max,
                      float *d_out_f32, void *d_out_planes, float *d_out_info, int batch, int in_h, int in_w, int cin, int cout,
-                     int relu, void *stream, const int *d_items = nullptr, long long *d_prof = nullptr) {
+                     int relu, void *stream, const int *d_items = nullptr, long long *d_prof = nullptr, const int *d_segs = nullptr) {
     if (PROBE != kP2NoProbe && !d_prof) return SESSD_EINVAL;
     P2Params p;
     P2Taps cls[4];
     p2_deconv_params(batch, in_h, in_w, cin, cout, relu, p, cls);
     p.items = d_items;
+    p.segs = d_segs;
     p.prof = d_prof;
     return launch_p2<MODE, PROBE>(d_in_planes, in_h, in_w, d_in_info, d_weight_h2, 9, cout_pad, d_scale, d_shift, d_residual, d_resid_info, gain, shift_max,
                      d_out_f32, d_out_planes, d_out_info, p, cls, 4, in_h, in_w, MODE == kP2Planes, stream);
diff --git a/se-ssd_b200/csrc/bevconv_split.cu b/se-ssd_b200/csrc/bevconv_split.cu
--- a/se-ssd_b200/csrc/bevconv_split.cu
+++ b/se-ssd_b200/csrc/bevconv_split.cu
@@ -23,19 +23,20 @@
 extern "C" int sessd_bev_conv_p2_profile(const void *d_in_planes, const float *d_in_info, const void *d_weight_h2, int cout_pad,
                                          const float *d_scale, const float *d_shift, const float *d_residual, const float *d_resid_info,
                                          float gain, float shift_max, float *d_out_f32, void *d_out_planes, float *d_out_info,
-                                         const sessd_conv_desc *desc, const int *d_items, long long *d_prof, void *stream) {
+                                         const sessd_conv_desc *desc, const int *d_items, const int *d_segs, long long *d_prof,
+                                         void *stream) {
     return p2_conv<kP2Planes, kP2ProbeClocks>(d_in_planes, d_in_info, d_weight_h2, cout_pad, d_scale, d_shift, d_residual, d_resid_info, gain,
-                                              shift_max, d_out_f32, d_out_planes, d_out_info, desc, stream, d_items, d_prof);
+                                              shift_max, d_out_f32, d_out_planes, d_out_info, desc, stream, d_items, d_prof, false, d_segs);
 }
 
 extern "C" int sessd_bev_deconv_p2_profile(const void *d_in_planes, const float *d_in_info, const void *d_weight_h2, int cout_pad,
                                            const float *d_scale, const float *d_shift, const float *d_residual, const float *d_resid_info,
                                            float gain, float shift_max, float *d_out_f32, void *d_out_planes, float *d_out_info, int batch,
-                                           int in_h, int in_w, int cin, int cout, int relu, const int *d_items, long long *d_prof,
-                                           void *stream) {
+                                           int in_h, int in_w, int cin, int cout, int relu, const int *d_items, const int *d_segs,
+                                           long long *d_prof, void *stream) {
     return p2_deconv<kP2Planes, kP2ProbeClocks>(d_in_planes, d_in_info, d_weight_h2, cout_pad, d_scale, d_shift, d_residual, d_resid_info, gain,
                                                 shift_max, d_out_f32, d_out_planes, d_out_info, batch, in_h, in_w, cin, cout, relu, stream,
-                                                d_items, d_prof);
+                                                d_items, d_prof, d_segs);
 }
 
 extern "C" int sessd_bev_conv_p2_loads(const void *d_in_planes, const float *d_in_info, const void *d_weight_h2, int cout_pad,
@@ -44,6 +45,15 @@
                                        const sessd_conv_desc *desc, const int *d_items, int smem_a, long long *d_prof, void *stream) {
     return p2_conv<kP2Planes, kP2ProbeLoads>(d_in_planes, d_in_info, d_weight_h2, cout_pad, d_scale, d_shift, d_residual, d_resid_info, gain,
                                              shift_max, d_out_f32, d_out_planes, d_out_info, desc, stream, d_items, d_prof, smem_a != 0);
+}
+
+extern "C" int sessd_bev_conv_p2_seg_loads(const void *d_in_planes, const float *d_in_info, const void *d_weight_h2, int cout_pad,
+                                           const float *d_scale, const float *d_shift, const float *d_residual, const float *d_resid_info,
+                                           float gain, float shift_max, float *d_out_f32, void *d_out_planes, float *d_out_info,
+                                           const sessd_conv_desc *desc, const int *d_segs, long long *d_prof, void *stream) {
+    if (!d_segs) return SESSD_EINVAL;
+    return p2_conv<kP2Planes, kP2ProbeLoads>(d_in_planes, d_in_info, d_weight_h2, cout_pad, d_scale, d_shift, d_residual, d_resid_info, gain,
+                                             shift_max, d_out_f32, d_out_planes, d_out_info, desc, stream, nullptr, d_prof, false, d_segs);
 }
 
 extern "C" int sessd_bev_p2_plan(const sessd_conv_desc *desc, int deconv, int cout_pad, int split, int smem_a, int *plan) {
diff --git a/se-ssd_b200/csrc/bevskip.cu b/se-ssd_b200/csrc/bevskip.cu
--- a/se-ssd_b200/csrc/bevskip.cu
+++ b/se-ssd_b200/csrc/bevskip.cu
@@ -6,6 +6,11 @@
     kRecCount = 0, kRecSkipped = 1, kRecNclass = 2, kRecTiles = 3, kRecTilesU = 4, kRecTilesV = 5, kRecUisX = 6, kRecOutStride = 7,
     kRecOutH = 8, kRecOutW = 9, kRecBatch = 10, kRecOffY = 11, kRecOffX = 15, kRecRep = 19, kRecSkipOff = 23, kRecFlagOff = 24
 };
+enum {
+    kSegCount = 0, kSegSkipped = 1, kSegGroups = 2, kSegNclass = 3, kSegPerClass = 4, kSegTilesU = 5, kSegGridV = 6, kSegUisX = 7,
+    kSegOutStride = 8, kSegOutH = 9, kSegOutW = 10, kSegBatch = 11, kSegOffY = 12, kSegOffX = 16, kSegRep = 20, kSegSkipOff = 28,
+    kSegFlagOff = 29
+};
 
 enum { kMX, kMB0a, kMB0b, kMX0, kMM0, kMM1, kMO0, kMO1, kMOut, kMTmp, kMB1a, kMB1b, kMX1, kMTmpH, kNumMaps };
 constexpr int kNumFullMaps = kMTmp + 1;
@@ -16,10 +21,15 @@
     int map;
     int out_stride, out_h, out_w;
     int rec;
+    int seg;
+    int nseg, max_groups;
 };
 
 struct SkipPlan {
     int batch, depth, h, w, h2, w2, nwf, nwh;
+    long long seg_words;
+    long long map_off;
+    int frame_words;
     SkipLaunch l[kSkipLaunches];
 };
 
@@ -53,10 +63,19 @@
                  | skip_launch(L[11], kMO1, batch, h, w, h, w, 128, false)
                  | skip_launch(L[12], kMOut, batch, h, w, h, w, 24, false);
     long long words = 0;
+    P.seg_words = 0;
     for (int i = 0; i < kSkipLaunches; ++i) {
         L[i].rec = (int)words;
         words += kP2ItemsHeader + L[i].total + 2LL * L[i].nclass * L[i].tiles;
-    }
+        L[i].nseg = batch * L[i].grid_v * L[i].tiles_u;
+        L[i].max_groups = L[i].nclass * div_up(L[i].nseg, kP2SegSlots);
+        L[i].seg = i == 3 ? -1 : (int)P.seg_words;
+        if (L[i].seg >= 0) P.seg_words += kP2SegHeader + (long long)kP2SegSlots * L[i].max_groups + 2LL * L[i].nclass * L[i].nseg;
+    }
+    P.frame_words = kNumFullMaps * h * P.nwf + (kNumMaps - kNumFullMaps) * P.h2 * P.nwh;
+    P.map_off = P.seg_words;
+    P.seg_words += (long long)batch * P.frame_words;
+    if (P.seg_words >= (1LL << 31) || L[0].nseg >= (1 << 24)) return 0;
     return rc ? 0 : words;
 }
 
@@ -129,7 +148,8 @@
     return base;
 }
 
-__global__ void __launch_bounds__(kSkipThreads) bev_skip_plan_kernel(const uint2 *__restrict__ bitmap, int *__restrict__ plan, SkipPlan P) {
+__global__ void __launch_bounds__(kSkipThreads) bev_skip_plan_kernel(const uint2 *__restrict__ bitmap, int *__restrict__ plan,
+                                                                    int *__restrict__ segs, SkipPlan P) {
     extern __shared__ uint32_t s_bits[];
     __shared__ int s_scan[33], s_rep[4];
     BitMap m[kNumMaps];
@@ -204,6 +224,7 @@
                 flags[c * L.tiles + b * per_frame + tf] = run ? 1 : 0;
             }
         }
+        for (int i = threadIdx.x; i < P.frame_words; i += blockDim.x) segs[P.map_off + (long long)b * P.frame_words + i] = (int)s_bits[i];
         __syncthreads();
     }
     for (int li = 0; li < kSkipLaunches; ++li) {
@@ -236,6 +257,116 @@
             rec[kRecFlagOff] = kP2ItemsHeader + L.total + L.nclass * L.tiles;
         }
         __syncthreads();
+    }
+}
+
+__global__ void __launch_bounds__(kSkipThreads) bev_skip_seg_kernel(int *__restrict__ segs, SkipPlan P) {
+    __shared__ int s_scan[33], s_rep[8];
+    const SkipLaunch &L = P.l[blockIdx.x];
+    if (L.seg < 0) return;
+    int *rec = segs + L.seg;
+    int *groups = rec + kP2SegHeader, *skipped = groups + kP2SegSlots * L.max_groups;
+    int *flags = skipped + L.nclass * L.nseg;
+    const int nseg = L.nseg;
+    const bool full = L.map < kNumFullMaps;
+    const int map_word = full ? L.map * P.h * P.nwf : kNumFullMaps * P.h * P.nwf + (L.map - kNumFullMaps) * P.h2 * P.nwh;
+    const int seg_frame = L.grid_v * L.tiles_u;
+    for (int b = 0; b < P.batch; ++b) {
+        const BitMap o{reinterpret_cast<uint32_t *>(segs + P.map_off + (long long)b * P.frame_words + map_word), full ? P.h : P.h2,
+                       full ? P.w : P.w2, full ? P.nwf : P.nwh};
+        for (int idx = threadIdx.x; idx < L.nclass * seg_frame; idx += blockDim.x) {
+            const int c = idx / seg_frame, sf = idx - c * seg_frame;
+            const int v = sf / L.tiles_u, u0 = (sf - v * L.tiles_u) * kP2TileU;
+            bool live = u0 + kP2TileU > L.grid_u;
+            if (!live && L.out_stride == 1 && L.u_is_x) {
+                live = (o.w[v * o.nw + (u0 >> 5)] >> (u0 & 31)) & 0xFFu;
+            } else {
+                for (int i = 0; i < kP2TileU && !live; ++i) {
+                    const int ou = (u0 + i) * L.out_stride + L.off_u[c], ov = v * L.out_stride + L.off_v[c];
+                    live = L.u_is_x ? o.get(ov, ou) : o.get(ou, ov);
+                }
+            }
+            flags[c * nseg + b * seg_frame + sf] = live ? 1 : 0;
+        }
+    }
+    __syncthreads();
+    auto parity = [&](int s) { return (s / L.tiles_u) % L.grid_v & 1; };
+    if (threadIdx.x < 8) s_rep[threadIdx.x] = 0x7FFFFFFF;
+    __syncthreads();
+    for (int e = threadIdx.x; e < L.nclass * nseg; e += blockDim.x)
+        if (!flags[e]) {
+            const int c = e / nseg, s = e - c * nseg;
+            atomicMin(&s_rep[2 * c + parity(s)], s);
+        }
+    __syncthreads();
+    int ngroups = 0;
+    for (int rank = 0; rank < L.nclass; ++rank) {
+        const int c = L.order[rank];
+        int *g = groups + kP2SegSlots * ngroups;
+        const int n = skip_compact(nseg, [&](int s) {
+            return flags[c * nseg + s] != 0 || s == s_rep[2 * c] || s == s_rep[2 * c + 1];
+        }, g, s_scan);
+        const int ng = (n + kP2SegSlots - 1) / kP2SegSlots;
+        for (int j = threadIdx.x; j < ng * kP2SegSlots; j += blockDim.x) g[j] = j < n ? (c << 24) | g[j] : -1;
+        ngroups += ng;
+        __syncthreads();
+    }
+    const int nskip = skip_compact(L.nclass * nseg, [&](int e) {
+        const int c = e / nseg, s = e - c * nseg;
+        return flags[e] == 0 && s != s_rep[2 * c + parity(s)];
+    }, skipped, s_scan);
+    if (threadIdx.x == 0) {
+        rec[kSegCount] = ngroups * L.nblocks; rec[kSegSkipped] = nskip; rec[kSegGroups] = ngroups;
+        rec[kSegNclass] = L.nclass; rec[kSegPerClass] = nseg; rec[kSegTilesU] = L.tiles_u; rec[kSegGridV] = L.grid_v;
+        rec[kSegUisX] = L.u_is_x; rec[kSegOutStride] = L.out_stride; rec[kSegOutH] = L.out_h; rec[kSegOutW] = L.out_w;
+        rec[kSegBatch] = P.batch;
+        for (int c = 0; c < 4; ++c) {
+            rec[kSegOffY + c] = L.u_is_x ? L.off_v[c] : L.off_u[c]; rec[kSegOffX + c] = L.u_is_x ? L.off_u[c] : L.off_v[c];
+            for (int par = 0; par < 2; ++par)
+                rec[kSegRep + 2 * c + par] = c < L.nclass && s_rep[2 * c + par] != 0x7FFFFFFF ? s_rep[2 * c + par] : -1;
+        }
+        rec[kSegSkipOff] = kP2SegHeader + kP2SegSlots * L.max_groups;
+        rec[kSegFlagOff] = kP2SegHeader + kP2SegSlots * L.max_groups + L.nclass * nseg;
+    }
+}
+
+__global__ void __launch_bounds__(256) bev_skip_fill_segs_kernel(const int *__restrict__ rec, float *__restrict__ out_f32,
+                                                                 __half *__restrict__ out_planes, int cout) {
+    const int nskip = __ldg(rec + kSegSkipped);
+    const int nseg = __ldg(rec + kSegPerClass), tiles_u = __ldg(rec + kSegTilesU), grid_v = __ldg(rec + kSegGridV);
+    const int u_is_x = __ldg(rec + kSegUisX), os = __ldg(rec + kSegOutStride), out_h = __ldg(rec + kSegOutH), out_w = __ldg(rec + kSegOutW);
+    const long long plane_stride = (long long)__ldg(rec + kSegBatch) * out_h * out_w * cout;
+    const int *skipped = rec + __ldg(rec + kSegSkipOff);
+    auto pixels = [&](int e, int lu, size_t &dst, size_t &src) {
+        const int ent = __ldg(skipped + e), c = ent / nseg, s = ent - c * nseg;
+        const int oy0 = __ldg(rec + kSegOffY + c), ox0 = __ldg(rec + kSegOffX + c);
+        auto pixel = [&](int ss) -> size_t {
+            const int rest = ss / tiles_u, v = rest % grid_v, b = rest / grid_v, gu = (ss - rest * tiles_u) * kP2TileU + lu;
+            const int gy = u_is_x ? v : gu, gx = u_is_x ? gu : v;
+            return ((size_t)b * out_h + (size_t)(gy * os + oy0)) * out_w + (size_t)(gx * os + ox0);
+        };
+        dst = pixel(s);
+        src = pixel(__ldg(rec + kSegRep + 2 * c + ((s / tiles_u) % grid_v & 1)));
+    };
+    const int stride = gridDim.x * blockDim.x, tid = blockIdx.x * blockDim.x + threadIdx.x;
+    if (out_f32) {
+        const int q = cout / 4, n = nskip * kP2TileU * q;
+        for (int i = tid; i < n; i += stride) {
+            const int px = i / q, j = i - px * q;
+            size_t dst, src;
+            pixels(px / kP2TileU, px % kP2TileU, dst, src);
+            reinterpret_cast<float4 *>(out_f32 + dst * cout)[j] = reinterpret_cast<const float4 *>(out_f32 + src * cout)[j];
+        }
+    }
+    if (out_planes) {
+        const int q = cout / 8, n = nskip * kP2TileU * q;
+        for (int i = tid; i < 2 * n; i += stride) {
+            const int pl = i / n, k = i - pl * n, px = k / q, j = k - px * q;
+            size_t dst, src;
+            pixels(px / kP2TileU, px % kP2TileU, dst, src);
+            reinterpret_cast<uint4 *>(out_planes + pl * plane_stride + dst * cout)[j] =
+                reinterpret_cast<const uint4 *>(out_planes + pl * plane_stride + src * cout)[j];
+        }
     }
 }
 
@@ -289,19 +420,28 @@
     return words;
 }
 
-extern "C" int sessd_bev_skip_plan(const void *d_bitmap_index, sessd_grid grid, int *d_plan, void *stream) {
-    if (!d_bitmap_index || !d_plan || grid.shape[0] < 1) return SESSD_EINVAL;
+extern "C" long long sessd_bev_skip_seg_words(int batch, int h, int w, int *offsets) {
+    SkipPlan P;
+    if (!skip_plan(P, batch, h, w)) return 0;
+    if (offsets)
+        for (int i = 0; i < kSkipLaunches; ++i) offsets[i] = P.l[i].seg;
+    return P.seg_words;
+}
+
+extern "C" int sessd_bev_skip_plan(const void *d_bitmap_index, sessd_grid grid, int *d_plan, int *d_segs, void *stream) {
+    if (!d_bitmap_index || !d_plan || !d_segs || grid.shape[0] < 1) return SESSD_EINVAL;
     SkipPlan P;
     if (!skip_plan(P, grid.batch, grid.shape[1], grid.shape[2])) return SESSD_EINVAL;
     P.depth = grid.shape[0];
-    const int smem = 4 * (kNumFullMaps * P.h * P.nwf + (kNumMaps - kNumFullMaps) * P.h2 * P.nwh);
+    const int smem = 4 * P.frame_words;
     if (smem > 200 * 1024) return SESSD_EINVAL;
     static int attr_smem = 48 * 1024;
     if (smem > attr_smem) {
         SESSD_CUDA_TRY(cudaFuncSetAttribute(bev_skip_plan_kernel, cudaFuncAttributeMaxDynamicSharedMemorySize, smem));
         attr_smem = smem;
     }
-    SESSD_LAUNCH(bev_skip_plan_kernel, 1, kSkipThreads, smem, (cudaStream_t)stream, (const uint2 *)d_bitmap_index, d_plan, P);
+    SESSD_LAUNCH(bev_skip_plan_kernel, 1, kSkipThreads, smem, (cudaStream_t)stream, (const uint2 *)d_bitmap_index, d_plan, d_segs, P);
+    SESSD_LAUNCH(bev_skip_seg_kernel, kSkipLaunches, kSkipThreads, 0, (cudaStream_t)stream, d_segs, P);
     return last_error();
 }
 
@@ -310,3 +450,9 @@
     SESSD_LAUNCH(bev_skip_fill_kernel, 2 * kNumSMs, 256, 0, (cudaStream_t)stream, d_record, d_out_f32, (__half *)d_out_planes, cout);
     return last_error();
 }
+
+extern "C" int sessd_bev_skip_fill_segs(const int *d_seg_record, float *d_out_f32, void *d_out_planes, int cout, void *stream) {
+    if (!d_seg_record || (!d_out_f32 && !d_out_planes) || cout < 8 || cout % 8) return SESSD_EINVAL;
+    SESSD_LAUNCH(bev_skip_fill_segs_kernel, 2 * kNumSMs, 256, 0, (cudaStream_t)stream, d_seg_record, d_out_f32, (__half *)d_out_planes, cout);
+    return last_error();
+}
diff --git a/se-ssd_b200/sessd_b200/_lib.py b/se-ssd_b200/sessd_b200/_lib.py
--- a/se-ssd_b200/sessd_b200/_lib.py
+++ b/se-ssd_b200/sessd_b200/_lib.py
@@ -78,11 +78,13 @@
     "sessd_spconv_wgrad_cg": (_i, [_vp, _i, _vp, _vp, _i, _vp, _vp, _i, _vp, _i, _vp, _vp, _sz, _vp]),
     "sessd_sparse_to_dense_indexed": (_i, [_vp, _i, _vp, _i, Grid, _vp, _vp]),
     "sessd_sparse_to_dense": (_i, [_vp, _vp, _vp, _i, _i, Grid, _vp, _vp]),
-    "sessd_bev_conv_p2": (_i, [_vp, _vp, _vp, _i, _vp, _vp, _vp, _vp, _f, _f, _vp, _vp, _vp, C.POINTER(ConvDesc), _vp, _vp]),
-    "sessd_bev_deconv_p2": (_i, [_vp, _vp, _vp, _i, _vp, _vp, _vp, _vp, _f, _f, _vp, _vp, _vp, _i, _i, _i, _i, _i, _i, _vp, _vp]),
+    "sessd_bev_conv_p2": (_i, [_vp, _vp, _vp, _i, _vp, _vp, _vp, _vp, _f, _f, _vp, _vp, _vp, C.POINTER(ConvDesc), _vp, _vp, _vp]),
+    "sessd_bev_deconv_p2": (_i, [_vp, _vp, _vp, _i, _vp, _vp, _vp, _vp, _f, _f, _vp, _vp, _vp, _i, _i, _i, _i, _i, _i, _vp, _vp, _vp]),
     "sessd_bev_skip_plan_words": (_ll, [_i, _i, _i, _I3]),
-    "sessd_bev_skip_plan": (_i, [_vp, Grid, _vp, _vp]),
+    "sessd_bev_skip_seg_words": (_ll, [_i, _i, _i, _I3]),
+    "sessd_bev_skip_plan": (_i, [_vp, Grid, _vp, _vp, _vp]),
     "sessd_bev_skip_fill": (_i, [_vp, _vp, _vp, _i, _vp]),
+    "sessd_bev_skip_fill_segs": (_i, [_vp, _vp, _vp, _i, _vp]),
     "sessd_bev_wgrad_items": (_i, [C.POINTER(ConvDesc)]),
     "sessd_bev_wgrad_workspace_bytes": (_sz, [C.POINTER(ConvDesc)]),
     "sessd_bev_wgrad": (_i, [_vp, _vp, _vp, _vp, C.POINTER(ConvDesc), _vp, _vp, _sz, _vp]),
@@ -151,10 +153,13 @@
 LAB_SIGNATURES = {
     "sessd_bev_conv_h2": (_i, [_vp, _vp, _i, _vp, _vp, _vp, _vp, C.POINTER(ConvDesc), _vp, _vp, _vp]),
     "sessd_bev_deconv_h2": (_i, [_vp, _vp, _i, _vp, _vp, _vp, _vp, _i, _i, _i, _i, _i, _i, _vp, _vp, _vp]),
-    "sessd_bev_conv_p2_profile": (_i, [_vp, _vp, _vp, _i, _vp, _vp, _vp, _vp, _f, _f, _vp, _vp, _vp, C.POINTER(ConvDesc), _vp, _vp, _vp]),
+    "sessd_bev_conv_p2_profile": (_i, [_vp, _vp, _vp, _i, _vp, _vp, _vp, _vp, _f, _f, _vp, _vp, _vp, C.POINTER(ConvDesc), _vp, _vp, _vp,
+                                       _vp]),
     "sessd_bev_deconv_p2_profile": (_i, [_vp, _vp, _vp, _i, _vp, _vp, _vp, _vp, _f, _f, _vp, _vp, _vp, _i, _i, _i, _i, _i, _i, _vp, _vp,
+                                         _vp, _vp]),
+    "sessd_bev_conv_p2_loads": (_i, [_vp, _vp, _vp, _i, _vp, _vp, _vp, _vp, _f, _f, _vp, _vp, _vp, C.POINTER(ConvDesc), _vp, _i, _vp, _vp]),
+    "sessd_bev_conv_p2_seg_loads": (_i, [_vp, _vp, _vp, _i, _vp, _vp, _vp, _vp, _f, _f, _vp, _vp, _vp, C.POINTER(ConvDesc), _vp, _vp,
                                          _vp]),
-    "sessd_bev_conv_p2_loads": (_i, [_vp, _vp, _vp, _i, _vp, _vp, _vp, _vp, _f, _f, _vp, _vp, _vp, C.POINTER(ConvDesc), _vp, _i, _vp, _vp]),
     "sessd_bev_p2_plan": (_i, [C.POINTER(ConvDesc), _i, _i, _i, _i, _I3]),
 }
 
diff --git a/se-ssd_b200/sessd_b200/ops.py b/se-ssd_b200/sessd_b200/ops.py
--- a/se-ssd_b200/sessd_b200/ops.py
+++ b/se-ssd_b200/sessd_b200/ops.py
@@ -320,19 +320,19 @@
 
 
 def bev_conv_p2(in_planes, in_info, weight_h2, scale, shift, residual, resid_info, gain, shift_max, out_f32, out_planes, out_info, desc,
-                items=None):
+                items=None, segs=None):
     check(lib.sessd_bev_conv_p2(_p(in_planes), _p(in_info), _p(weight_h2), int(weight_h2.shape[2]), _p(scale), _p(shift), _p(residual),
                                 _p(resid_info), float(gain), float(shift_max), _p(out_f32), _p(out_planes), _p(out_info), C.byref(desc),
-                                _p(items), _st()), "sessd_bev_conv_p2")
+                                _p(items), _p(segs), _st()), "sessd_bev_conv_p2")
 
 
 def bev_deconv_p2(in_planes, in_info, weight_h2, scale, shift, residual, resid_info, gain, shift_max, out_f32, out_planes, out_info, relu=True,
-                  items=None):
+                  items=None, segs=None):
     _two, b, h, w, cin = in_planes.shape
     cout = (out_f32 if out_f32 is not None else out_planes).shape[-1]
     check(lib.sessd_bev_deconv_p2(_p(in_planes), _p(in_info), _p(weight_h2), int(weight_h2.shape[2]), _p(scale), _p(shift), _p(residual),
                                   _p(resid_info), float(gain), float(shift_max), _p(out_f32), _p(out_planes), _p(out_info), int(b), int(h),
-                                  int(w), int(cin), int(cout), int(bool(relu)), _p(items), _st()), "sessd_bev_deconv_p2")
+                                  int(w), int(cin), int(cout), int(bool(relu)), _p(items), _p(segs), _st()), "sessd_bev_deconv_p2")
 
 
 class BevSkipPlan:
@@ -340,21 +340,30 @@
     LAUNCHES = 13
 
     def __init__(self, batch, h, w, device):
-        offs = (C.c_int * self.LAUNCHES)()
+        offs, seg_offs = (C.c_int * self.LAUNCHES)(), (C.c_int * self.LAUNCHES)()
         words = lib.sessd_bev_skip_plan_words(int(batch), int(h), int(w), offs)
-        if words <= 0:
+        seg_words = lib.sessd_bev_skip_seg_words(int(batch), int(h), int(w), seg_offs)
+        if words <= 0 or seg_words <= 0:
             raise ValueError("no skip plan for a [%d, %d, %d] neck" % (batch, h, w))
-        self.offsets = list(offs)
+        self.offsets, self.seg_offsets = list(offs), list(seg_offs)
         self.buf = torch.zeros((int(words),), dtype=torch.int32, device=device)
+        self.seg_buf = torch.zeros((int(seg_words),), dtype=torch.int32, device=device)
 
     def record(self, i):
         return self.buf[self.offsets[i]:]
 
+    def seg_record(self, i):
+        return self.seg_buf[self.seg_offsets[i]:] if self.seg_offsets[i] >= 0 else None
+
     def build(self, bitmap_index, grid):
-        check(lib.sessd_bev_skip_plan(_p(bitmap_index), grid, _p(self.buf), _st()), "sessd_bev_skip_plan")
+        check(lib.sessd_bev_skip_plan(_p(bitmap_index), grid, _p(self.buf), _p(self.seg_buf), _st()), "sessd_bev_skip_plan")
 
     def fill(self, i, out_f32, out_planes, cout):
         check(lib.sessd_bev_skip_fill(_p(self.record(i)), _p(out_f32), _p(out_planes), int(cout), _st()), "sessd_bev_skip_fill")
+
+    def fill_segs(self, i, out_f32, out_planes, cout):
+        check(lib.sessd_bev_skip_fill_segs(_p(self.seg_record(i)), _p(out_f32), _p(out_planes), int(cout), _st()),
+              "sessd_bev_skip_fill_segs")
 
 
 def bev_split_planes(x, info, planes):
diff --git a/se-ssd_b200/sessd_b200/runners.py b/se-ssd_b200/sessd_b200/runners.py
--- a/se-ssd_b200/sessd_b200/runners.py
+++ b/se-ssd_b200/sessd_b200/runners.py
@@ -293,15 +293,18 @@
         out_f32, out_planes = (self.buf[L.dst], None) if L.f32 else (None, self.planes[L.dst])
         resid, resid_info = (self.buf[L.residual], self._info(L.residual)) if L.residual else (None, None)
         i = self.SKIP_LAUNCHES.index(L.name)
-        rec = self.skip.record(i) if skip else None
+        segs = self.skip.seg_record(i) if skip else None
+        rec = self.skip.record(i) if skip and segs is None else None
         if L.kind == "conv":
             d = launch_desc(L, self.batch, *ssfa_extents(L, self.h, self.w), q["taps"])
             ops.bev_conv_p2(self.planes[L.src], self._info(L.src), q["w"], q["scale"], q["shift"], resid, resid_info, q["gain"],
-                            q["shift_max"], out_f32, out_planes, self._info(L.dst), d, items=rec)
+                            q["shift_max"], out_f32, out_planes, self._info(L.dst), d, items=rec, segs=segs)
         else:
             ops.bev_deconv_p2(self.planes[L.src], self._info(L.src), q["w"], q["scale"], q["shift"], resid, resid_info, q["gain"],
-                              q["shift_max"], out_f32, out_planes, self._info(L.dst), L.relu, items=rec)
-        if skip:
+                              q["shift_max"], out_f32, out_planes, self._info(L.dst), L.relu, items=rec, segs=segs)
+        if segs is not None:
+            self.skip.fill_segs(i, out_f32, out_planes, L.cout)
+        elif skip:
             self.skip.fill(i, out_f32, out_planes, L.cout)
 
     def forward(self, x=None, mark=None, occupancy=None):
```

Result: faster. 1618 (median of 6 runs) (+4.6%).
